# ipc-sim/IPC

Measured on AMD Instinct MI355X. Metric: newton_iterations_per_sec, higher is better.
Workload: dtype f64

## Files before the change

include/ipcgpu.h:

```cpp
#ifndef IPCGPU_H
#define IPCGPU_H

#ifdef __cplusplus
extern "C" {
#endif

#define IPCGPU_OK 0
#define IPCGPU_NOT_PD 1
#define IPCGPU_ERR_ARG -1
#define IPCGPU_ERR_HIP -2
#define IPCGPU_ERR_STATE -3
#define IPCGPU_ERR_UNSUPPORTED -4

typedef struct ipcgpu_ctx ipcgpu_ctx;

enum { IPCGPU_NOT_DBC = 0, IPCGPU_DBC_ZERO = 1, IPCGPU_DBC_NONZERO = 2 };

enum { IPCGPU_SOLVER_MULTIFRONTAL = 0, IPCGPU_SOLVER_ROCSOLVER_CSRRF = 1, IPCGPU_SOLVER_PCG = 2 };
enum { IPCGPU_PRECOND_BLOCK_JACOBI = 0, IPCGPU_PRECOND_LAGGED_CHOLESKY = 1, IPCGPU_PRECOND_TWO_LEVEL = 2 };

const char* ipcgpu_last_error(void);
int ipcgpu_version(void);

int ipcgpu_ctx_create(int device_id, ipcgpu_ctx** out);
int ipcgpu_ctx_destroy(ipcgpu_ctx*);
int ipcgpu_ctx_set_solver(ipcgpu_ctx*, int solver_type);
int ipcgpu_ctx_set_shard(ipcgpu_ctx*, int rank, int world_size);

typedef struct ipcgpu_tetmesh ipcgpu_tetmesh;
int ipcgpu_read_tet_mesh(const char* path, ipcgpu_tetmesh** mesh, int* nV, int* nT, int* nSF);
int ipcgpu_tet_mesh_get(const ipcgpu_tetmesh*, double* V_colmajor, int* T_colmajor, int* SF_colmajor);
void ipcgpu_tet_mesh_free(ipcgpu_tetmesh*);
int ipcgpu_save_tet_mesh(const char* path, int nV, int nT, const double* V_colmajor, const int* T_colmajor);

int ipcgpu_set_mesh(ipcgpu_ctx*, int nV, int nT, const double* V_rest_colmajor,
    const int* F_colmajor, double youngs_modulus, double poisson_ratio, double density);
int ipcgpu_set_dbc(ipcgpu_ctx*, int n, const int* vert_ids, int dbc_type);
int ipcgpu_clear_dbc(ipcgpu_ctx*);
int ipcgpu_set_component_material(ipcgpu_ctx*, int nodeBegin, int nodeEnd, int tetBegin, int tetEnd, double rho, double YM, double PR);
int ipcgpu_set_energy_type(ipcgpu_ctx*, int energy_type);
int ipcgpu_set_positions(ipcgpu_ctx*, const double* V_colmajor);
int ipcgpu_get_positions(ipcgpu_ctx*, double* V_colmajor);
int ipcgpu_set_xtilde(ipcgpu_ctx*, const double* xTilta_colmajor);
int ipcgpu_get_features(ipcgpu_ctx*, double* restTriInv_9nT, double* triArea_nT, double* mass_nV,
    double* mu_nT, double* lambda_nT);
int ipcgpu_get_mesh_dims(ipcgpu_ctx*, int* nV, int* nT);
int ipcgpu_set_mesh_features(ipcgpu_ctx*, const double* restTriInv_9nT, const double* triArea_nT, const double* mass_nV,
    const double* mu_nT, const double* lambda_nT);
int ipcgpu_check_inversion(ipcgpu_ctx*, int* ok);

int ipcgpu_elastic_energy(ipcgpu_ctx*, double coef, double* energy);
int ipcgpu_elastic_energy_per_elem(ipcgpu_ctx*, double* perElem_nT);
int ipcgpu_elastic_stress(ipcgpu_ctx*, double* perElem_nTx8, double* perNode_nVx8, int* n_invalid);
int ipcgpu_elastic_gradient(ipcgpu_ctx*, double coef, int projectDBC, double* grad_3nV);
int ipcgpu_elastic_hessian_add(ipcgpu_ctx*, double coef, int projectDBC);
int ipcgpu_filter_step_size(ipcgpu_ctx*, const double* searchDir_3nV, double* stepSize_inout);

int ipcgpu_linsys_set_pattern(ipcgpu_ctx*, int n_extra, const int* extra_pairs_2n);
int ipcgpu_linsys_set_pattern_csr(ipcgpu_ctx*, int n_rows, const int* ia, const int* ja);
int ipcgpu_linsys_get_dims(ipcgpu_ctx*, int* n_rows, int* nnz);
int ipcgpu_linsys_get_pattern(ipcgpu_ctx*, int* ia, int* ja);
int ipcgpu_linsys_set_zero(ipcgpu_ctx*);
int ipcgpu_linsys_get_values(ipcgpu_ctx*, double* a);
int ipcgpu_linsys_set_values(ipcgpu_ctx*, const double* a);
int ipcgpu_linsys_apply_host_updates(ipcgpu_ctx*, const double* delta_nnz, const unsigned char* isSet_nnz, const double* setVal_nnz);
int ipcgpu_linsys_add_coeff(ipcgpu_ctx*, int row, int col, double v);
int ipcgpu_linsys_set_coeff(ipcgpu_ctx*, int row, int col, double v);
int ipcgpu_linsys_multiply(ipcgpu_ctx*, const double* x, double* Ax);
int ipcgpu_linsys_analyze_pattern(ipcgpu_ctx*);
int ipcgpu_linsys_factorize(ipcgpu_ctx*);
int ipcgpu_linsys_solve(ipcgpu_ctx*, const double* rhs, double* result);
int ipcgpu_linsys_precondition_diag(ipcgpu_ctx*, const double* in, double* out);
int ipcgpu_linsys_set_iterative(ipcgpu_ctx*, double rel_tol, int max_iter, int precond, int max_factor_age);
int ipcgpu_linsys_iter_stats(ipcgpu_ctx*, double* out6);
int ipcgpu_linsys_coarse_stats(ipcgpu_ctx*, double* out5);
int ipcgpu_linsys_coarse_dims(ipcgpu_ctx*, int* n_aggregates, int* n_rows, int* nnz);
int ipcgpu_linsys_coarse_get(ipcgpu_ctx*, int* agg_of_node, int* coarse_ia, int* coarse_ja, double* coarse_a);
int ipcgpu_linsys_multiply_sym(ipcgpu_ctx*, const double* x, double* Ax);
int ipcgpu_linsys_set_shard(ipcgpu_ctx*, int rank, int world_size);
int ipcgpu_linsys_shard_stats(ipcgpu_ctx*, double* out2);
int ipcgpu_linsys_exchange_stats(ipcgpu_ctx*, double* out4);
int ipcgpu_linsys_critical_path(ipcgpu_ctx*, double* out5);
int ipcgpu_opt_comm_stats(ipcgpu_ctx*, double* out6);
int ipcgpu_opt_complete_matrix(ipcgpu_ctx*);
int ipcgpu_linsys_entry_destinations(ipcgpu_ctx*, long long* dst_nnz);
int ipcgpu_linsys_set_tuning(ipcgpu_ctx*, double bulk_min_mb, int bulk_block);
int ipcgpu_linsys_stats(ipcgpu_ctx*, double* stats4);

int ipcgpu_assemble_newton(ipcgpu_ctx*, double dtSq, int projectDBC, double* grad_3nV );
int ipcgpu_incremental_potential(ipcgpu_ctx*, double dtSq, double* energy);
int ipcgpu_gradient(ipcgpu_ctx*, double dtSq, int projectDBC, double* grad_3nV);

int ipcgpu_set_surface(ipcgpu_ctx*, int nSF, const int* SF_colmajor);
int ipcgpu_set_surface_codim(ipcgpu_ctx*, int nSF, const int* SF_colmajor, int nCE, const int* CE_pairs);
int ipcgpu_set_exact_predicates(ipcgpu_ctx*, int on);
int ipcgpu_get_surface(ipcgpu_ctx*, int* counts3 , int* SVI , int* SFEdges_2n );
int ipcgpu_set_obstacle_nodes(ipcgpu_ctx*, int n, const int* vert_ids, int obstacle_only);
int ipcgpu_set_codim_nodes(ipcgpu_ctx*, int n, const int* node_ids, const double* node_mass);
int ipcgpu_contact_build(ipcgpu_ctx*, double dHat, int* counts3);
int ipcgpu_contact_counts(ipcgpu_ctx*, int* counts3);
int ipcgpu_contact_get(ipcgpu_ctx*, int* active_4n, int* paraEE_4n, int* paraEEeIeJ_2n, int* csPTEE_2n );
int ipcgpu_contact_set(ipcgpu_ctx*, int nActive, const int* active_4n, int nParaEE, const int* paraEE_4n, const int* paraEEeIeJ_2n);
int ipcgpu_contact_energy(ipcgpu_ctx*, double dHat, double kappa, double* energy);
int ipcgpu_contact_evaluate(ipcgpu_ctx*, int n, const int* mmcvid_4n, double* val_n);
int ipcgpu_contact_jt_multiply(ipcgpu_ctx*, int n, const int* mmcvid_4n, const double* input_n, double coef, double* out_3nV_inout);
int ipcgpu_contact_gradient_add(ipcgpu_ctx*, double dHat, double kappa, int projectDBC, double* grad_3nV_inout);
int ipcgpu_contact_report(ipcgpu_ctx*, double dHat, double kappa, const double* Vt_colmajor , double eps2, double coef, int capacity, int* nRows,
    int* rowsI_8n, double* rowsD_20n);
int ipcgpu_contact_hessian_add(ipcgpu_ctx*, double dHat, double kappa, int projectDBC);
int ipcgpu_contact_connectivity(ipcgpu_ctx*, int capacity, int* pairs_2n, int* nPairs);
int ipcgpu_ccd_partial(ipcgpu_ctx*, const double* searchDir_3nV, double slackness, double* stepSize_inout, int* pair2);
int ipcgpu_ccd_full(ipcgpu_ctx*, const double* searchDir_3nV, double slackness, double* stepSize_inout, int* pair2, int* nCandidates);
int ipcgpu_ccd_full_reference(ipcgpu_ctx*, const double* searchDir_3nV, double slackness, double* stepSize_inout, double* alphaCapped, int* arg3,
    int* nCandidates);
int ipcgpu_set_ccd_mode(ipcgpu_ctx*, int mode);
int ipcgpu_is_intersected(ipcgpu_ctx*, int* flag);

int ipcgpu_opt_init(ipcgpu_ctx*, double dt, int withGravity);
int ipcgpu_opt_set_rel_tol(ipcgpu_ctx*, double relTol);
int ipcgpu_opt_set_twist(ipcgpu_ctx*, int nLeft, const int* left, int nRight, const int* right, double angVel);
int ipcgpu_opt_enable_self_collision(ipcgpu_ctx*, double dHatEps);
int ipcgpu_opt_set_pattern_lookahead(ipcgpu_ctx*, double pad);
int ipcgpu_opt_add_half_space(ipcgpu_ctx*, const double* origin3, const double* normal3, double dHatEps, int* id);
int ipcgpu_halfspace_build(ipcgpu_ctx*, int id, double dHat, int cap, int* verts, int* n);
int ipcgpu_halfspace_set(ipcgpu_ctx*, int id, int n, const int* verts);
int ipcgpu_halfspace_energy(ipcgpu_ctx*, int id, double dHat, double kappa, double* E);
int ipcgpu_halfspace_gradient_add(ipcgpu_ctx*, int id, double dHat, double kappa, double* grad_3nV_inout);
int ipcgpu_halfspace_hessian_add(ipcgpu_ctx*, int id, double dHat, double kappa, int projectDBC);
int ipcgpu_halfspace_move(ipcgpu_ctx*, int id, const double* delta3, double slackness, double* stepSizeLeft);
int ipcgpu_halfspace_step_bound(ipcgpu_ctx*, int id, const double* searchDir_3nV, double slackness, double* stepSize_inout);
int ipcgpu_opt_set_friction(ipcgpu_ctx*, double selfFric, int fricIterAmt, double epsV);
int ipcgpu_opt_set_friction_target(ipcgpu_ctx*, double eps_v_target);
int ipcgpu_opt_set_constructor_dt(ipcgpu_ctx*, double h);
int ipcgpu_opt_set_parameter_scaling(ipcgpu_ctx*, int useAbsParameters, double dTolRel, double kappaMinMultiplier);
int ipcgpu_opt_set_friction_scales(ipcgpu_ctx*, double scaleSelf, double scaleObstacle);
int ipcgpu_opt_force_friction_loop(ipcgpu_ctx*, int on);
int ipcgpu_opt_set_half_space_friction(ipcgpu_ctx*, int id, double mu);
int ipcgpu_opt_set_damping(ipcgpu_ctx*, double dampingStiff);
int ipcgpu_opt_set_kappa(ipcgpu_ctx*, double kappa);
int ipcgpu_opt_set_dhat_target(ipcgpu_ctx*, double dHatTargetEps);
int ipcgpu_opt_next_subproblem(ipcgpu_ctx*, int* more);
int ipcgpu_opt_get_friction_state(ipcgpu_ctx*, double* scalars4, double* lambda);
int ipcgpu_friction_update(ipcgpu_ctx*, double dHat, double kappa, int* nLagged);
int ipcgpu_friction_get(ipcgpu_ctx*, double* lambda_n, double* coord_2n, double* basis_6n);
int ipcgpu_friction_energy(ipcgpu_ctx*, const double* Vt_colmajor, double eps2, double coef, double* energy);
int ipcgpu_friction_gradient_add(ipcgpu_ctx*, const double* Vt_colmajor, double eps2, double coef, double* grad_3nV_inout);
int ipcgpu_friction_hessian_add(ipcgpu_ctx*, const double* Vt_colmajor, double eps2, double coef, int projectDBC);
int ipcgpu_opt_set_velocity(ipcgpu_ctx*, const double* vel_3nV);
int ipcgpu_opt_set_time_integration(ipcgpu_ctx*, int type, double beta, double gamma);
int ipcgpu_opt_set_warm_start(ipcgpu_ctx*, int option);
int ipcgpu_opt_get_warm_step(ipcgpu_ctx*, double* last_step);
int ipcgpu_opt_add_dirichlet(ipcgpu_ctx*, int n, const int* vert_ids, const double* lin_vel3, const double* ang_vel3, double t0, double t1);
int ipcgpu_opt_end_dirichlet(ipcgpu_ctx*, int group, double t_end);
int ipcgpu_opt_set_dirichlet_motion(ipcgpu_ctx*, int group, const double* lin_vel3, const double* ang_vel3, const double* center3 ,
    int force_nonzero);
int ipcgpu_opt_set_dirichlet_targets(ipcgpu_ctx*, int group, int n, const double* targets_3n);
int ipcgpu_opt_add_neumann(ipcgpu_ctx*, int n, const int* vert_ids, const double* accel3, double t0, double t1);
int ipcgpu_opt_get_dbc_state(ipcgpu_ctx*, double* out4);
int ipcgpu_opt_get_kinematics(ipcgpu_ctx*, double* vel_3nV, double* acc_3nV, double* dx_elastic_3nV);
int ipcgpu_opt_set_components(ipcgpu_ctx*, int nComp, const int* nodeEnd_nComp, const int* tetEnd_nComp);
int ipcgpu_opt_system_report(ipcgpu_ctx*, double* sysE_nComp, double* sysM_3nComp, double* sysL_3nComp);
int ipcgpu_opt_save_status(ipcgpu_ctx*, const char* path);
int ipcgpu_opt_load_status(ipcgpu_ctx*, const char* path);
int ipcgpu_opt_get_contact_state(ipcgpu_ctx*, int* counts6, int* pair2);
int ipcgpu_opt_precompute(ipcgpu_ctx*);
int ipcgpu_opt_begin_timestep(ipcgpu_ctx*);
int ipcgpu_opt_newton_iter(ipcgpu_ctx*, int* converged);
int ipcgpu_opt_end_timestep(ipcgpu_ctx*);
int ipcgpu_opt_solve_timestep(ipcgpu_ctx*, int maxIter, int* nIter);
int ipcgpu_opt_get_state(ipcgpu_ctx*, double* V_colmajor, double* searchDir_3nV, double* gradient_3nV, double* scalars8);
int ipcgpu_opt_get_timers(ipcgpu_ctx*, double* t16);
typedef int (*ipcgpu_allreduce_fn)(void* user, void* buf_dev, long long count, int op);
int ipcgpu_opt_set_allreduce(ipcgpu_ctx*, ipcgpu_allreduce_fn fn, void* user);
typedef int (*ipcgpu_allreduce_stream_fn)(void* user, void* buf_dev, long long count, int op, void* hip_stream);
int ipcgpu_opt_set_allreduce_stream(ipcgpu_ctx*, ipcgpu_allreduce_stream_fn fn, void* user);
typedef struct ipcgpu_p2p_op {
    void* buf_dev;
    long long count;
    int peer;
    int send;
} ipcgpu_p2p_op;
typedef int (*ipcgpu_exchange_fn)(void* user, int n_ops, const ipcgpu_p2p_op* ops);
typedef int (*ipcgpu_exchange_stream_fn)(void* user, int n_ops, const ipcgpu_p2p_op* ops, void* hip_stream);
int ipcgpu_opt_set_exchange(ipcgpu_ctx*, ipcgpu_exchange_fn fn, void* user);
int ipcgpu_opt_set_exchange_stream(ipcgpu_ctx*, ipcgpu_exchange_stream_fn fn, void* user);
int ipcgpu_ctx_get_stream(ipcgpu_ctx*, void** hip_stream);

int ipcgpu_bench_assembly(ipcgpu_ctx*, double dtSq, int reps, double* avg_ms, double* algorithmic_bytes);
int ipcgpu_bench_factor_solve(ipcgpu_ctx*, int reps, double* factor_ms, double* solve_ms);
int ipcgpu_bench_multiply_sym(ipcgpu_ctx*, int reps, double* avg_ms, double* algorithmic_bytes);
int ipcgpu_bench_stream(ipcgpu_ctx*, long long bytes, int reps, double* gbps);

#ifdef __cplusplus
}
#endif
#endif
```

ipc_amd/csrc/capi.cpp:

```cpp
#include "../../include/ipcgpu.h"
#include "hip_ipc.h"
#include "msh_io.h"
#include <cstdlib>
#include <cstring>
#include <mutex>

using namespace ipcgpu;

namespace {
thread_local std::string g_err;

template <class Fn>
int guarded(Fn&& fn)
{
    try {
        return fn();
    }
    catch (const ArgError& e) {
        g_err = e.what();
        return IPCGPU_ERR_ARG;
    }
    catch (const StateError& e) {
        g_err = e.what();
        return IPCGPU_ERR_STATE;
// ... 596 lines not shown
}
int ipcgpu_linsys_multiply_sym(ipcgpu_ctx* c, const double* x, double* y)
{
    return guarded([&] {
        bind(c);
        HipLinSysSolver& l = L(c);
        need(l.numRows > 0, "no pattern");
        needWholeMatrix(c);
        DevBuf<double> dx, dy;
        dx.upload(x, l.numRows, c->stream);
        dy.alloc(l.numRows);
        l.multiplySym(dx.p, dy.p);
        dy.download(y, l.numRows, c->stream);
        return IPCGPU_OK;
    });
}
int ipcgpu_linsys_set_iterative(ipcgpu_ctx* c, double rel_tol, int max_iter, int precond, int max_factor_age)
{
    specChanged(c);
    return guarded([&] {
        L(c).setIterative(rel_tol, max_iter, precond, max_factor_age);
        return IPCGPU_OK;
    });
}
int ipcgpu_linsys_iter_stats(ipcgpu_ctx* c, double* out6)
{
    return guarded([&] {
        needArg(c && out6, "null argument");
        L(c).iterStats(out6);
        return IPCGPU_OK;
    });
}
int ipcgpu_linsys_coarse_stats(ipcgpu_ctx* c, double* out5)
{
    return guarded([&] {
        needArg(c && out5, "null argument");
        L(c).coarseStats(out5);
        return IPCGPU_OK;
    });
}
int ipcgpu_linsys_coarse_dims(ipcgpu_ctx* c, int* n_agg, int* n_rows, int* nnz)
{
    return guarded([&] {
        L(c).coarseDims(n_agg, n_rows, nnz);
        return IPCGPU_OK;
    });
}
int ipcgpu_linsys_coarse_get(ipcgpu_ctx* c, int* agg_of_node, int* coarse_ia, int* coarse_ja, double* coarse_a)
{
    return guarded([&] {
        bind(c);
        L(c).coarseGet(agg_of_node, coarse_ia, coarse_ja, coarse_a);
        return IPCGPU_OK;
    });
}
int ipcgpu_linsys_analyze_pattern(ipcgpu_ctx* c)
{
    return guarded([&] {
        bind(c);
        L(c).analyze_pattern(c->mesh->nV ? c->mesh.get() : nullptr);
        return IPCGPU_OK;
    });
}
int ipcgpu_linsys_factorize(ipcgpu_ctx* c)
{
    return guarded([&] {
        bind(c);
        return L(c).factorize() ? IPCGPU_OK : IPCGPU_NOT_PD;
    });
}
int ipcgpu_linsys_solve(ipcgpu_ctx* c, const double* rhs, double* x)
{
    return guarded([&] {
        bind(c);
        HipLinSysSolver& l = L(c);
        DevBuf<double> db, dx;
        db.upload(rhs, l.numRows, c->stream);
        dx.alloc(l.numRows);
        const bool ok = l.solve(db.p, dx.p);
        dx.download(x, l.numRows, c->stream);
        return ok ? IPCGPU_OK : IPCGPU_NOT_PD;
    });
}
int ipcgpu_linsys_precondition_diag(ipcgpu_ctx* c, const double* in, double* out)
{
    return guarded([&] {
        bind(c);
        HipLinSysSolver& l = L(c);
        needWholeMatrix(c);
        DevBuf<double> di, dout;
        di.upload(in, l.numRows, c->stream);
        dout.alloc(l.numRows);
        l.precondition_diag(di.p, dout.p);
        dout.download(out, l.numRows, c->stream);
        return IPCGPU_OK;
    });
}
int ipcgpu_linsys_set_shard(ipcgpu_ctx* c, int rank, int world)
{
    specChanged(c);
    return guarded([&] {
        needArg(c && world >= 1 && rank >= 0 && rank < world, "bad shard");
        if (world > 1 && c->lin->solverType == IPCGPU_SOLVER_PCG) {
            g_err = "the iterative solver is not sharded";
            return IPCGPU_ERR_UNSUPPORTED;
        }
        need(world == 1 || c->opt->allreduce != nullptr || c->opt->allreduceStream != nullptr, "set the all-reduce hook first (ipcgpu_opt_set_allreduce)");
        need(world == 1 || c->lin->hasExchangeHook(), "set the exchange hook first (ipcgpu_opt_set_exchange / ipcgpu_opt_set_exchange_stream): the sharded solver sends point to point");
        c->lin->setShard(rank, world, c->opt->allreduce, c->opt->allreduceUser, c->opt->allreduceStream, c->opt->allreduceStreamUser);
        return IPCGPU_OK;
    });
}
int ipcgpu_opt_comm_stats(ipcgpu_ctx* c, double* out6)
{
    return guarded([&] {
        needArg(c && out6, "null argument");
        HipOptimizer& o = O(c);
        out6[0] = (double)o.commBytes;
        out6[1] = (double)o.commCalls;
        out6[2] = (double)L(c).exchangedBytes();
        out6[3] = (double)L(c).exchangeCalls();
        out6[4] = (double)(o.ownerMode() ? o.ownerNeededNodes : c->mesh->nV);
        out6[5] = (double)c->mesh->nV;
        return IPCGPU_OK;
    });
}
int ipcgpu_opt_complete_matrix(ipcgpu_ctx* c)
{
    return guarded([&] {
        bind(c);
        O(c).completeMatrix();
        return IPCGPU_OK;
    });
}
int ipcgpu_linsys_exchange_stats(ipcgpu_ctx* c, double* out4)
{
    return guarded([&] {
        needArg(c && out4, "null argument");
        out4[0] = (double)L(c).sentBytes();
        out4[1] = (double)L(c).receivedBytes();
        out4[2] = (double)L(c).exchangeCalls();
        out4[3] = L(c).exchangeWaitMs();
        return IPCGPU_OK;
    });
}
int ipcgpu_linsys_entry_destinations(ipcgpu_ctx* c, long long* dst_nnz)
{
    return guarded([&] {
        bind(c);
        needArg(c && dst_nnz, "null argument");
        need(L(c).solverType == IPCGPU_SOLVER_MULTIFRONTAL && L(c).analyzed(), "the multifrontal solver has not analysed a pattern yet");
        L(c).entryDestinations(dst_nnz);
        return IPCGPU_OK;
    });
}
int ipcgpu_linsys_shard_stats(ipcgpu_ctx* c, double* out2)
{
    return guarded([&] {
        out2[0] = L(c).solverWorld();
        out2[1] = L(c).sharedFlopFraction();
        return IPCGPU_OK;
    });
}
int ipcgpu_linsys_set_tuning(ipcgpu_ctx* c, double bulk_min_mb, int bulk_block)
{
    return guarded([&] {
// ... 891 lines not shown
            counts6[2] = o.selfCollision ? o.contact->nCand() : 0;
            counts6[3] = 0;
            for (const auto& h : o.planes) counts6[3] += (int)h->set.size();
            counts6[4] = o.nFullCCD;
            counts6[5] = o.nPatternChanges;
        }
        if (pair2) {
            pair2[0] = o.lastCCDPair[0];
            pair2[1] = o.lastCCDPair[1];
        }
        return IPCGPU_OK;
    });
}
int ipcgpu_opt_precompute(ipcgpu_ctx* c)
{
    return guarded([&] {
        bind(c);
        O(c).precompute();
        return IPCGPU_OK;
    });
}
int ipcgpu_opt_begin_timestep(ipcgpu_ctx* c)
{
    return guarded([&] {
        bind(c);
        O(c).beginTimestep();
        return IPCGPU_OK;
    });
}
int ipcgpu_opt_newton_iter(ipcgpu_ctx* c, int* converged)
{
    return guarded([&] {
        bind(c);
        const bool cv = O(c).newtonIter();
        if (converged) *converged = cv ? 1 : 0;
        return IPCGPU_OK;
    });
}
int ipcgpu_opt_end_timestep(ipcgpu_ctx* c)
{
    return guarded([&] {
        bind(c);
        O(c).endTimestep();
        return IPCGPU_OK;
    });
}
int ipcgpu_opt_solve_timestep(ipcgpu_ctx* c, int maxIter, int* nIter)
{
    return guarded([&] {
        bind(c);
        const int n = O(c).solveTimestep(maxIter);
        if (nIter) *nIter = n;
        return IPCGPU_OK;
    });
}
int ipcgpu_opt_get_state(ipcgpu_ctx* c, double* V, double* p, double* g, double* sc)
{
    return guarded([&] {
        HipOptimizer& o = O(c);
        bind(c);
        need(o.initialised, "call ipcgpu_opt_init first");
        const size_t n3 = 3 * (size_t)c->mesh->nV;
        if (V) downloadColMajor(c, c->mesh->d_x, V);
        if (p) o.d_searchDir.download(p, n3, c->stream);
        if (g) o.d_gradient.download(g, n3, c->stream);
        if (sc) {
            sc[0] = o.lastEnergyVal;
            sc[1] = o.lastStepSize;
            sc[2] = o.targetGRes;
            sc[3] = o.innerIterAmt;
            sc[4] = o.globalIterNum;
            sc[5] = o.lastAlphaFeasible;
            sc[6] = o.kappa;
            sc[7] = o.dHat;
        }
        return IPCGPU_OK;
    });
}
int ipcgpu_opt_get_timers(ipcgpu_ctx* c, double* t)
{
    return guarded([&] {
        O(c).resolveEventTimers();
        std::memcpy(t, O(c).timers, sizeof(double) * 16);
        return IPCGPU_OK;
    });
}
int ipcgpu_opt_set_allreduce(ipcgpu_ctx* c, ipcgpu_allreduce_fn fn, void* user)
{
    return guarded([&] {
        needArg(c != nullptr, "null context");
        c->opt->allreduce = fn;
        c->opt->allreduceUser = user;
        c->lin->setHooks(c->opt->allreduce, c->opt->allreduceUser, c->opt->allreduceStream, c->opt->allreduceStreamUser);
        return IPCGPU_OK;
    });
}

int ipcgpu_opt_set_allreduce_stream(ipcgpu_ctx* c, ipcgpu_allreduce_stream_fn fn, void* user)
{
    return guarded([&] {
        needArg(c != nullptr, "null context");
        c->opt->allreduceStream = fn;
        c->opt->allreduceStreamUser = user;
        c->lin->setHooks(c->opt->allreduce, c->opt->allreduceUser, c->opt->allreduceStream, c->opt->allreduceStreamUser);
        return IPCGPU_OK;
    });
}
static_assert(sizeof(ipcgpu_p2p_op) == sizeof(MfNumeric::P2POp), "ipcgpu_p2p_op and MfNumeric::P2POp must be one layout");
int ipcgpu_opt_set_exchange(ipcgpu_ctx* c, ipcgpu_exchange_fn fn, void* user)
{
    return guarded([&] {
        needArg(c != nullptr, "null context");
        c->exchange = reinterpret_cast<void*>(fn);
        c->exchangeUser = user;
        c->lin->setExchangeHooks(reinterpret_cast<MfNumeric::ExchangeFn>(c->exchange), c->exchangeUser, reinterpret_cast<MfNumeric::ExchangeStreamFn>(c->exchangeStream),
            c->exchangeStreamUser);
        return IPCGPU_OK;
    });
}
int ipcgpu_opt_set_exchange_stream(ipcgpu_ctx* c, ipcgpu_exchange_stream_fn fn, void* user)
{
    return guarded([&] {
        needArg(c != nullptr, "null context");
        c->exchangeStream = reinterpret_cast<void*>(fn);
        c->exchangeStreamUser = user;
        c->lin->setExchangeHooks(reinterpret_cast<MfNumeric::ExchangeFn>(c->exchange), c->exchangeUser, reinterpret_cast<MfNumeric::ExchangeStreamFn>(c->exchangeStream),
            c->exchangeStreamUser);
        return IPCGPU_OK;
    });
}
int ipcgpu_ctx_get_stream(ipcgpu_ctx* c, void** hipStream)
{
    return guarded([&] {
        needArg(c != nullptr && hipStream != nullptr, "null argument");
        *hipStream = (void*)c->stream;
        return IPCGPU_OK;
    });
}

int ipcgpu_bench_assembly(ipcgpu_ctx* c, double dtSq, int reps, double* avg_ms, double* bytes)
{
    return guarded([&] {
        HipOptimizer& o = O(c);
        bind(c);
        need(o.initialised && !c->lin->rowBase.empty(), "needs opt_init + a pattern");
        needArg(reps > 0, "reps must be positive");
        hipEvent_t e0, e1;
        HIP_CHECK(hipEventCreate(&e0));
        HIP_CHECK(hipEventCreate(&e1));
        const ElemView v = o.view();
        o.ensurePatchPlan();
        int pb, pe;
        o.patchShard(pb, pe);
        double total = 0.0;
        for (int r = 0; r < reps; ++r) {
            HIP_CHECK(hipEventRecord(e0, c->stream));
            launch_assemble_patches(v, o.patch, pb, pe, dtSq, 1, o.d_gradient.p, c->lin->d_a.p, c->stream);
            HIP_CHECK(hipEventRecord(e1, c->stream));
            HIP_CHECK(hipEventSynchronize(e1));
            float ms = 0;
            HIP_CHECK(hipEventElapsedTime(&ms, e0, e1));
            total += ms;
        }
        (void)hipEventDestroy(e0);
        (void)hipEventDestroy(e1);
        *avg_ms = total / reps;
// ... 92 lines not shown
```

ipc_amd/csrc/hip_ipc.h:

```cpp
#pragma once
#include "common.h"
#include "contact_pattern.h"
#include "mf_numeric.h"
#include "mf_symbolic.h"
#include "nh_kernels.h"
#include "patch_assembly.h"
#include "hip_contact.h"
#include "hip_halfspace.h"
#include "pcg.h"
#include "pcg_coarse.h"
#include "report_plan.h"
#include "stress_plan.h"
#include <map>
#include <memory>
#include <string>

struct ipcgpu_ctx;
typedef int (*ipcgpu_allreduce_fn_t)(void* user, void* buf_dev, long long count, int op);
typedef int (*ipcgpu_allreduce_stream_fn_t)(void* user, void* buf_dev, long long count, int op, void* hipStream);

namespace ipcgpu {

class HipMesh {
public:
    int nV = 0, nT = 0;
    int nElemNodes = 0;
    std::vector<double> V_rest;
    std::vector<int> F;
    std::vector<double> restTriInv;
    std::vector<double> triArea, mass, mu, lam;
    std::vector<int> dbcType;
    std::vector<int> nbPtr, nb;
    double avgEdgeLen = 0, bboxDiag2 = 0, bboxLo[3] = { 0, 0, 0 }, bboxHi[3] = { 0, 0, 0 };
    DevBuf<double> d_x, d_xTilde, d_mass, d_A, d_vol, d_mu, d_lam;
    DevBuf<int> d_dbc;
    DevBuf<int4> d_tet;

    unsigned featuresVersion = 0;
    void computeFeatures(int nV, int nT, const double* Vrest, const int* F, double YM, double PR, double density, hipStream_t s);
    std::vector<char> inMesh;
    void addSurfaceEdges(int nSF, const int* SF_colmajor, int nCE = 0, const int* CE_pairs = nullptr);
    void setCodimNodes(int n, const int* ids, const double* nodeMass, hipStream_t s);
    void meshBBox();
    void uploadDBC(hipStream_t s);
    int energyType = 0;
    double density = 0;
    void setComponentMaterial(int nodeBegin, int nodeEnd, int tetBegin, int tetEnd, double rho, double YM, double PR, hipStream_t s);
    bool isDBCVertex(int v) const { return dbcType[v] != 0; }
    bool isProjectDBCVertex(int v, bool projectDBC) const { return dbcType[v] == 1 || (dbcType[v] == 2 && projectDBC); }
};

class HipLinSysSolver {
public:
    explicit HipLinSysSolver(hipStream_t s);
    ~HipLinSysSolver();
    int numRows = 0;
    std::vector<int> ia, ja;
    DevBuf<int> d_ia, d_ja;
    DevBuf<double> d_a;
    DevBuf<double> hostDelta, hostSetVal;
    DevBuf<unsigned char> hostSetMask;
    std::vector<int> rowBase, rowLen;
    DevBuf<int> d_rowBase, d_rowLen, d_edgeP0;
    int solverType = 0;
    int patternVersion = 0;
    hipStream_t stream;

    void set_pattern(const HipMesh& mesh, int nExtra, const int* extraPairs);
    void set_pattern_csr(int nRows, const int* ia, const int* ja);
    void buildElementMap(const HipMesh& mesh);
    void setZero();
    int findEntry(int row, int col) const;
    void analyze_pattern(const HipMesh* meshForCoords);
    bool factorize();
    bool solve(const double* rhs_dev, double* x_dev);
    bool factorizeSolve(const double* rhs_dev, double* x_dev, bool wait = true);
    bool lastPivotsOk() const;
    bool lastSyncOk_ = true;
    void multiply(const double* x_dev, double* y_dev);
    void precondition_diag(const double* in_dev, double* out_dev);
    double pcgRelTol = 1e-5;
    int pcgMaxIter = 1000;
    int pcgPrecond = 0, pcgMaxFactorAge = 1;
    void setIterative(double relTol, int maxIter, int precond, int maxFactorAge);
    void iterStats(double* out6) const;
    void coarseStats(double* out5) const;
    bool coarseDims(int* nAgg, int* rows, int* nnz) const;
    void coarseGet(int* aggOfNode, int* cia, int* cja, double* ca);
    void multiplySym(const double* x_dev, double* y_dev);
    int getNumRows() const { return numRows; }
    int getNumNonzeros() const { return (int)ja.size(); }
    const MfSymbolic& symbolic() const { return sym_; }
    void setShard(int rank, int world, ipcgpu_allreduce_fn_t fn, void* user, ipcgpu_allreduce_stream_fn_t sfn = nullptr, void* streamUser = nullptr)
    {
        num_.setShard(rank, world, fn, user, sfn, streamUser);
        analyzed_ = false;
    }
    void setHooks(ipcgpu_allreduce_fn_t fn, void* user, ipcgpu_allreduce_stream_fn_t sfn, void* streamUser) { num_.setHooks(fn, user, sfn, streamUser); }
    void setExchangeHooks(MfNumeric::ExchangeFn fn, void* user, MfNumeric::ExchangeStreamFn sfn, void* streamUser) { num_.setExchangeHooks(fn, user, sfn, streamUser); }
    bool hasExchangeHook() const { return num_.hasExchangeHook(); }
    int solverWorld() const { return num_.world(); }
    void setBulkTuning(double minMB, int block) { num_.setBulkTuning(minMB, block); }
    void entryDestinations(long long* out) const { num_.entryDestinations(out, ja.size()); }
    void nodeOwners(std::vector<int>& o) const { num_.nodeOwners(o); }
    long long exchangedBytes() const { return num_.exchangedBytes(); }
    long long exchangeCalls() const { return num_.exchangeCalls(); }
    long long sentBytes() const { return num_.sentBytes(); }
    long long receivedBytes() const { return num_.receivedBytes(); }
    double exchangeWaitMs() { return num_.exchangeWaitMs(); }
    void criticalPath(double* out5) const { num_.criticalPath(out5); }
    int analysisVersion = 0;
    double sharedFlopFraction() const { return num_.sharedFlopFraction(); }
    bool analyzed() const { return analyzed_; }
    void invalidateAnalysis() { analyzed_ = false; }

private:
    MfSymbolic sym_;
    MfNumeric num_;
    bool analyzed_ = false;
    std::unique_ptr<struct RocsolverCsrrf> rs_;
    PcgPattern pcgPat_;
    PcgWork pcgWork_;
    int pcgPatVersion_ = -1;
    void ensurePcgPattern();
    int runPcg(const double* rhs_dev, double* x_dev, PcgState& out);
    bool haveFactor_ = false, lastConverged_ = true;
    int factorAge_ = 0;
    long long nFactorizations_ = 0;
    PcgCoarse coarseHost_;
    PcgCoarseDev coarseDev_;
    std::unique_ptr<HipLinSysSolver> coarse_;
    const HipMesh* coarseMesh_ = nullptr;
    int coarseVersion_ = -1;
    bool coarseBuilt_ = false, coarseOk_ = false;
    long long nCoarseFactorizations_ = 0, nCoarseFallbacks_ = 0;
    struct {
        int iterations = 0, syncs = 0, factorAge = 0;
        double residual = 0.0;
        bool converged = false;
    } pcgLast_;
    friend struct RocsolverCsrrf;
};

class HipOptimizer {
public:
    HipOptimizer(HipMesh& mesh, HipLinSysSolver& lin, hipStream_t s);
    void init(double dt, bool withGravity);
    void setRelGL2Tol(double relTol);
    void setParameterScaling(bool absolute, double dTolRel, double kappaMinMultiplier);
    void setTwist(int nL, const int* left, int nR, const int* right, double angVel);
    void precompute();
    void beginTimestep();
    bool newtonIter();
    void endTimestep();
    int solveTimestep(int maxIter);

    double computeEnergyVal();
    void computeGradient(bool projectDBC);
    void penaltyGradientAdd(bool projectDBC);
// ... 27 lines not shown
    double relGL2Tol = 1e-8, targetGRes = 0;
    int timeIntegration = 0;
    int warmStart = 0;
    double warmStepSize = 0.0;
    double betaNM = 0.25, gammaNM = 0.5;
    DevBuf<double> d_acc, d_dxElastic;
    double elasticCoef() const { return timeIntegration == 1 ? dtSq * betaNM : dtSq; }
    void setTimeIntegration(int type, double beta, double gamma);
    void getKinematics(double* vel, double* acc, double* dxElastic);
    void getDbcState(double* out4) const;
    std::vector<int> compNodeEnd, compTetEnd;
    DevBuf<double> d_xStepStart, d_reportRec;
    DevBuf<int> d_reportSlices, d_reportNodeStart, d_reportTetStart;
    PinnedBuf<double> h_report;
    bool reportPlanValid = false;
    int nReportNodeSlices = 0, nReportSlices = 0;
    void setComponents(int nComp, const int* nodeEnd, const int* tetEnd);
    void ensureReportPlan();
    void systemReport(double* sysE, double* sysM_3, double* sysL_3);
    void saveStatus(const std::string& path);
    void loadStatus(const std::string& path);
    DevBuf<double> d_vel, d_xPrev, d_searchDir, d_gradient, d_minusG, d_x0, d_partial, d_scalar;
    DevBuf<double> d_damp, d_xDamp, d_zeroMass, d_dampDx, d_dampAdx;
    unsigned long long dampPatternVersion = ~0ULL;
    DevBuf<int> d_flag, d_handleIds;
    DevBuf<double> d_handleAng;
    int nHandles = 0;
    struct DbcGroup {
        std::vector<int> ids;
        DevBuf<int> d_ids;
        DevBuf<double> d_pos;
        double lin[3], ang[3], t0, t1;
        bool forceNonzero = false, hasCenter = false;
        double center[3] = { 0, 0, 0 };
        bool hasTargets = false;
        DevBuf<double> d_targets;
        bool isZero() const { return !forceNonzero && lin[0] == 0 && lin[1] == 0 && lin[2] == 0 && ang[0] == 0 && ang[1] == 0 && ang[2] == 0; }
    };
    std::vector<std::unique_ptr<DbcGroup>> dbcGroups;
    struct NbcGroup {
        int n = 0;
        DevBuf<int> d_ids;
        double a[3], t0, t1;
    };
    std::vector<std::unique_ptr<NbcGroup>> nbcGroups;
    void addNeumannBC(int n, const int* ids, const double* accel3, double t0, double t1);
    void neumannGradientAdd(double* grad_dev);
    double neumannEnergy();
    std::vector<int> baseDbcType;
    double stepStartTime = 0, stepEndTime = 0;
    std::vector<int> tpIds, tpIdsOnDevice;
    DevBuf<int> d_tpIds;
    DevBuf<double> d_tpPos, d_tpLam, d_tpStage;
    double dist2Tol = 0, completedStep = 1.0, lastMove = 1.0, rhoDBC = 0.0, CN_MBC = 0.0;
    bool projDBC = true;
    MdbcView mdbc() const { return MdbcView{ (int)tpIds.size(), d_tpIds.p, d_tpPos.p, d_tpLam.p, mesh.d_mass.p }; }
    void buildTargetPositions(bool deferTolerance = false);
    void finishTolerance();
    PinnedBuf<double> h_tpStage;
    bool tolPending = false;
    void initSubProblem();
    double computeCompletedStepSize();
    void dirichletPenaltyUpdate();
    void addDirichletBC(int n, const int* ids, const double* lin3, const double* angRad3, double t0, double t1);
    void setDBCVertices();
    bool dbcGroupMotion();
    double rotCenter[3] = { 0, 0, 0 };
    PinnedBuf<double> h_scalar;
    PinnedBuf<int> h_flag;
    int innerIterAmt = 0, globalIterNum = 0, k = 0;
    double lastEnergyVal = 0, lastStepSize = 0, lastAlphaFeasible = 0;
    double timers[16] = { 0 };
    bool initialised = false;
    int rank = 0, worldSize = 1;
    int tetBegin = 0, tetEnd = 0;
    ipcgpu_allreduce_fn_t allreduce = nullptr;
    ipcgpu_allreduce_stream_fn_t allreduceStream = nullptr;
    void hookReduce(double* dev, long long n, int op);
    bool fastPath() const;
    bool cachedDistValid = false, cachedE0Valid = false;
    double cachedDist = 0, cachedE0 = 0, cachedFilter = 0;
    bool cachedTrialValid = false, cachedTrialInverted = false;
    double cachedTrialE = 0, cachedAlpha = 1.0;
    DevBuf<double> d_aSpec, d_gradSpec;
    bool specAsmValid = false;
    void speculativeAssembly();
    hipEvent_t evAsm0 = nullptr, evAsm1 = nullptr, evTail = nullptr;
    bool evAsmPending = false;
    int evAsmWeight = 1;
    unsigned asmLaunches = 0;
    void resolveEventTimers();
    DevBuf<double> d_contactG;
    void* allreduceUser = nullptr;
    void* allreduceStreamUser = nullptr;
    void reduceSum(double* dev, long long n);
    void reduceMin(double* dev, long long n);
    double readScalar(const double* dev);
    PatchPlan patch;
    int patchVersion = -1;
    void ensurePatchPlan();
    void patchShard(int& pb, int& pe) const;
    bool ownerMode() const;
    void ensureOwnerPlan();
    int ownerPlanPatch = -1, ownerPlanAnalysis = -1;
    int nOwnerPatches = 0;
    DevBuf<int> d_ownerPatches;
    DevBuf<unsigned char> d_need, d_mine;
    long long ownerNeededNodes = 0;
    bool matrixComplete = true;
    void maskAndReduceGradient(double* g);
    void ownerGradientTail(bool projectDBC);
    void completeMatrix();
    long long commBytes = 0, commCalls = 0;
    HipContact* contact = nullptr;
    bool selfCollision = false;
    double dHatEps = 1.0e-3, dHat = 0, kappa = 0, dTol = 0;
    bool absParameters = false;
    double dTolRel = 1.0e-9, kappaMinMultiplier = 1.0e11;
    double lenScale2() const { return absParameters ? 1.0 : mesh.bboxDiag2; }
    ContactPattern contactPattern;
    std::vector<std::array<int, 4>> closeID;
    std::vector<double> closeVal;
    int lastCCDPair[2] = { 0, 0 }, nFullCCD = 0, nPatternChanges = 0, dbcIncomplete = 0;
    unsigned long long coverSets = ~0ull;
    int coverPattern = -1;
    bool coverAnswer = false;
    double patternPad = -1.0;
    double lookahead() const { return patternPad >= 0.0 ? patternPad : (mesh.nV > 150000 ? 2.25 : 4.0); }
    std::vector<std::unique_ptr<HipHalfSpace>> planes;
    std::vector<std::pair<int, int>> closeHS;
    std::vector<double> closeHSVal;
    double selfFric = 0.0, epsV = 1.0e-3, fricDHat0 = 0, fricDHat = -1.0;
    double epsVTarget = -1.0, fricDHatTarget = 0;
    int fricIterAmt = 1, fricIterI = 0;
    bool fricLoopForced = false;
    bool solveFric() const;
    void updateFrictionLag();
    bool nextSubproblem();
    bool ipOn() const { return selfCollision || !planes.empty(); }
    size_t nConstraints() const;
    int addHalfSpace(HipContact* c, const double* origin3, const double* normal3, double dHatEps);
    bool anyIntersection();
    void elasticInertiaGradient(bool projectDBC, bool finish = true);
    void barrierGradientAdd(bool projectDBC, double kappa, bool activeOnly, double* grad_dev, int part = 0);
    void enableSelfCollision(HipContact* c, double dHatEps);
    void setVelocity(const double* vel3nV);
    void computeConstraintSets();
    double kappaFloor() const;
    void initKappa();
    void postLineSearch();
    bool isIntersected();
    void computeXTilta();
};

struct StressFields {
    bool planValid = false;
    DevBuf<int> d_ptr, d_elems, d_invalid;
    DevBuf<double> d_elem, d_node;
    PinnedBuf<int> h_invalid;
};

}

struct ipcgpu_ctx {
    int device = 0;
    hipStream_t stream = nullptr;
// ... 12 lines not shown
```

ipc_amd/csrc/hip_linsys.hip:

```cpp
#include "hip_ipc.h"
#include <rocsolver/rocsolver.h>
#include <algorithm>
#include <cmath>
#include <thread>
#include <cstdlib>

namespace ipcgpu {

struct RocsolverCsrrf {
    rocblas_handle handle = nullptr;
    rocsolver_rfinfo info = nullptr;
    int n = 0, nnzA = 0, nnzT = 0;
    DevBuf<int> ptrA, indA, ptrT, indT, pivQ, trans, flag;
    DevBuf<double> valA, valT, B;
    bool analyzed = false;
    ~RocsolverCsrrf()
    {
        if (info) rocsolver_destroy_rfinfo(info);
        if (handle) rocblas_destroy_handle(handle);
    }
};

namespace {
__global__ void k_gather(int n, const int* __restrict__ map, const double* __restrict__ src, double* __restrict__ dst)
// ... 224 lines not shown
        for (int r = 0; r < numRows; ++r) ptr[r + 1] += ptr[r];
        std::vector<int> pos(ptr.begin(), ptr.end() - 1);
        for (int r = 0; r < numRows; ++r)
            for (int k = ia[r]; k < ia[r + 1]; ++k) {
                const int c = ja[k];
                ind[pos[c]] = r;
                tr[pos[c]] = k;
                pos[c]++;
            }
        std::vector<int> pT, iT, q;
        mf_L_pattern_csr(sym_, pT, iT, q);
        R.nnzA = nnz;
        R.nnzT = (int)iT.size();
        R.ptrA.upload(ptr, stream);
        R.indA.upload(ind, stream);
        R.trans.upload(tr, stream);
        R.valA.alloc(nnz);
        R.ptrT.upload(pT, stream);
        R.indT.upload(iT, stream);
        R.pivQ.upload(q, stream);
        R.valT.alloc(iT.size());
        R.B.alloc(numRows);
        R.B.zero(stream);
        R.flag.alloc(1);
        hipLaunchKernelGGL(k_set_diag_one, dim3((numRows + 255) / 256), dim3(256), 0, stream, numRows, R.ptrT.p, R.indT.p, R.valT.p);
        hipLaunchKernelGGL(k_set_diag_one, dim3((numRows + 255) / 256), dim3(256), 0, stream, numRows, R.ptrA.p, R.indA.p, R.valA.p);
        const rocblas_status st = rocsolver_dcsrrf_analysis(R.handle, R.n, 1, R.nnzA, R.ptrA.p, R.indA.p, R.valA.p, R.nnzT, R.ptrT.p, R.indT.p, R.valT.p,
            nullptr, R.pivQ.p, R.B.p, R.n, R.info);
        if (st != rocblas_status_success) throw HipError("rocsolver_dcsrrf_analysis failed (rocblas_status " + std::to_string((int)st) + ")");
        HIP_CHECK(hipStreamSynchronize(stream));
        R.analyzed = true;
    }
    analyzed_ = true;
}

bool HipLinSysSolver::factorize()
{
    if (!analyzed_) throw StateError("factorize before analyze_pattern");
    if (solverType == 0) return num_.factorize(d_a.p);
    if (solverType == 2) {
        if (pcgPrecond == 0 || pcgPrecond == 2) {
            pcgWork_.ensure(numRows);
            pcgWork_.flag.zero(stream);
            launch_pcg_invert_blocks(pcgPat_, d_a.p, pcgWork_.flag.p, stream);
            int f = 0;
            pcgWork_.flag.download(&f, 1, stream);
            if (f || pcgPrecond == 0) return f == 0;
            if (!coarseMesh_->d_x.p || !coarseMesh_->d_dbc.p || 3 * coarseMesh_->nV != numRows) throw StateError("factorize: the mesh of the two-level preconditioner has no positions");
            launch_pcg_coarse_geometry(coarseDev_, coarseMesh_->d_x.p, coarseMesh_->d_dbc.p, stream);
            launch_pcg_galerkin(coarseDev_, d_rowLen.p, d_a.p, coarse_->d_a.p, stream);
            coarseBuilt_ = true;
            ++nCoarseFactorizations_;
            coarseOk_ = coarse_->factorize();
            if (!coarseOk_) ++nCoarseFallbacks_;
            return true;
        }
        if (haveFactor_ && lastConverged_ && factorAge_ + 1 < pcgMaxFactorAge) {
            ++factorAge_;
            return true;
        }
        ++nFactorizations_;
        haveFactor_ = num_.factorize(d_a.p);
        factorAge_ = 0;
        lastConverged_ = true;
        return haveFactor_;
    }
    RocsolverCsrrf& R = *rs_;
    hipLaunchKernelGGL(k_gather, dim3((R.nnzA + 255) / 256), dim3(256), 0, stream, R.nnzA, R.trans.p, d_a.p, R.valA.p);
    rocblas_status st = rocsolver_dcsrrf_refactchol(R.handle, R.n, R.nnzA, R.ptrA.p, R.indA.p, R.valA.p, R.nnzT, R.ptrT.p, R.indT.p,
        R.valT.p, R.pivQ.p, R.info);
    if (st != rocblas_status_success) {
        HIP_CHECK(hipStreamSynchronize(stream));
        return false;
    }
    R.flag.zero(stream);
    hipLaunchKernelGGL(k_check_diag, dim3((R.n + 255) / 256), dim3(256), 0, stream, R.n, R.ptrT.p, R.valT.p, R.pivQ.p, d_ia.p, d_a.p,
        R.flag.p);
    int f = 0;
    HIP_CHECK(hipMemcpyAsync(&f, R.flag.p, sizeof(int), hipMemcpyDeviceToHost, stream));
    HIP_CHECK(hipStreamSynchronize(stream));
    return f == 0;
}

bool HipLinSysSolver::factorizeSolve(const double* rhs_dev, double* x_dev, bool wait)
{
    if (!analyzed_) throw StateError("factorize before analyze_pattern");
    lastSyncOk_ = true;
    if (solverType == 0) return lastSyncOk_ = num_.factorizeSolve(d_a.p, rhs_dev, x_dev, wait);
    const bool ok = factorize();
    return lastSyncOk_ = ok && solve(rhs_dev, x_dev);
}
bool HipLinSysSolver::lastPivotsOk() const { return lastSyncOk_ && (solverType != 0 || num_.lastPivotsOk()); }

bool HipLinSysSolver::solve(const double* rhs_dev, double* x_dev)
{
    if (!analyzed_) throw StateError("solve before analyze_pattern");
    if (solverType == 0) {
        num_.solve(rhs_dev, x_dev);
        return true;
    }
    if (solverType == 2) {
        const bool lagged = pcgPrecond == 1;
        const bool jacobi = !lagged;
        if (lagged && !haveFactor_) throw StateError("solve before factorize");
        if (pcgPrecond == 2 && !coarseBuilt_) throw StateError("solve before factorize");
        pcgLast_ = {};
        pcgLast_.factorAge = jacobi ? 0 : factorAge_;
        PcgState st;
        int status = runPcg(rhs_dev, x_dev, st);
        pcgLast_.iterations = st.iter;
        if (status == PCG_MAXITER && !jacobi && factorAge_ > 0) {
            ++nFactorizations_;
            haveFactor_ = num_.factorize(d_a.p);
            factorAge_ = 0;
            if (!haveFactor_) return false;
            pcgLast_.factorAge = 0;
            status = runPcg(rhs_dev, x_dev, st);
            pcgLast_.iterations += st.iter;
        }
        pcgLast_.residual = st.bb > 0.0 ? std::sqrt(st.trueRes2 / st.bb) : 0.0;
        pcgLast_.converged = status == PCG_CONVERGED && st.trueRes2 <= st.tol2;
        lastConverged_ = pcgLast_.converged;
        return status != PCG_BREAKDOWN;
    }
    RocsolverCsrrf& R = *rs_;
    HIP_CHECK(hipMemcpyAsync(x_dev, rhs_dev, sizeof(double) * R.n, hipMemcpyDeviceToDevice, stream));
    if (rocsolver_dcsrrf_solve(R.handle, R.n, 1, R.nnzT, R.ptrT.p, R.indT.p, R.valT.p, nullptr, R.pivQ.p, x_dev, R.n, R.info)
        != rocblas_status_success)
        throw HipError("rocsolver_dcsrrf_solve failed");
    return true;
}

void HipLinSysSolver::setIterative(double relTol, int maxIter, int precond, int maxFactorAge)
{
    if (!(relTol > 0.0) || maxIter < 1 || precond < 0 || precond > 2 || maxFactorAge < 1)
        throw ArgError("set_iterative: rel_tol > 0, max_iter >= 1, precond 0 | 1 | 2, max_factor_age >= 1");
    if (precond != pcgPrecond && solverType == 2) analyzed_ = false;
    pcgRelTol = relTol;
    pcgMaxIter = maxIter;
    pcgPrecond = precond;
    pcgMaxFactorAge = maxFactorAge;
}

void HipLinSysSolver::iterStats(double* o) const
{
    o[0] = pcgLast_.iterations;
    o[1] = pcgLast_.residual;
    o[2] = pcgLast_.converged ? 1.0 : 0.0;
    o[3] = (double)nFactorizations_;
    o[4] = pcgLast_.factorAge;
    o[5] = pcgLast_.syncs;
}

void HipLinSysSolver::coarseStats(double* o) const
{
    const bool have = coarseVersion_ == patternVersion && coarse_;
    o[0] = have ? coarseHost_.nAgg : 0;
    o[1] = have ? 6.0 * coarseHost_.nAgg : 0;
    o[2] = have ? (double)coarseHost_.cja.size() : 0;
    o[3] = (double)nCoarseFactorizations_;
    o[4] = (double)nCoarseFallbacks_;
}
bool HipLinSysSolver::coarseDims(int* nAgg, int* rows, int* nnz) const
{
    const bool have = solverType == 2 && pcgPrecond == 2 && analyzed_ && coarse_ && coarseVersion_ == patternVersion;
    if (nAgg) *nAgg = have ? coarseHost_.nAgg : 0;
    if (rows) *rows = have ? 6 * coarseHost_.nAgg : 0;
    if (nnz) *nnz = have ? (int)coarseHost_.cja.size() : 0;
    return have;
}
void HipLinSysSolver::coarseGet(int* aggOfNode, int* cia, int* cja, double* ca)
{
    if (!coarseDims(nullptr, nullptr, nullptr)) throw StateError("no coarse level: set the two-level preconditioner and call analyze_pattern first");
    if (aggOfNode) std::copy(coarseHost_.aggOf.begin(), coarseHost_.aggOf.end(), aggOfNode);
// ... 89 lines not shown
```

ipc_amd/csrc/hip_optimizer.cpp:

```cpp
#include "hip_ipc.h"
#include <fstream>
#include <iomanip>
#include <limits>
#include <sstream>
#include <algorithm>
#include <chrono>
#include <thread>
#include <iterator>
#include <cmath>
#include <cstring>

#ifndef BEGIN_BATCHED
#define BEGIN_BATCHED 1
#endif

namespace ipcgpu {


namespace {
struct Tic {
    double& acc;
    hipStream_t s;
    std::chrono::high_resolution_clock::time_point t0;
    bool nosync = false;
    Tic(double& a, hipStream_t st) : acc(a), s(st), t0(std::chrono::high_resolution_clock::now()) {}
    ~Tic()
    {
        if (!nosync) (void)hipStreamSynchronize(s);
        acc += std::chrono::duration<double>(std::chrono::high_resolution_clock::now() - t0).count();
    }
};
}

HipOptimizer::HipOptimizer(HipMesh& m, HipLinSysSolver& l, hipStream_t s) : mesh(m), lin(l), stream(s) {}

ElemView HipOptimizer::view() const
{
    ElemView v;
    v.nV = mesh.nV;
    v.nT = mesh.nT;
    v.tetBegin = tetBegin;
    v.tetEnd = tetEnd;
    v.energyType = mesh.energyType;
    v.x = mesh.d_x.p;
    v.xTilde = mesh.d_xTilde.p;
    v.mass = mesh.d_mass.p;
    v.dbc = mesh.d_dbc.p;
    v.tet = mesh.d_tet.p;
    v.A = mesh.d_A.p;
    v.vol = mesh.d_vol.p;
    v.mu = mesh.d_mu.p;
    v.lam = mesh.d_lam.p;
    v.rowBase = lin.d_rowBase.p;
    v.rowLen = lin.d_rowLen.p;
    v.edgeP0 = lin.d_edgeP0.p;
    return v;
}

void HipOptimizer::init(double dt_, bool withGravity)
{
    dt = dt_;
    dtSq = dt * dt;
    gravity[0] = gravity[2] = 0.0;
    gravity[1] = withGravity ? -9.80665 : 0.0;
    const size_t n3 = 3 * (size_t)mesh.nV;
    d_vel.alloc(n3);
    d_vel.zero(stream);
    d_acc.alloc(n3);
    d_acc.zero(stream);
    d_dxElastic.alloc(n3);
    d_dxElastic.zero(stream);
    d_xPrev.alloc(n3);
    d_xStepStart.alloc(n3);
    d_searchDir.alloc(n3);
    d_searchDir.zero(stream);
    d_gradient.alloc(n3);
    d_gradient.zero(stream);
    d_minusG.alloc(n3);
    d_x0.alloc(n3);
    d_partial.alloc((size_t)std::max(mesh.nT, mesh.nV) / 256 + 2);
    d_scalar.alloc(8);
    d_flag.alloc(2);
    h_scalar.alloc(8);
    h_flag.alloc(2);
    HIP_CHECK(hipMemcpyAsync(d_xPrev.p, mesh.d_x.p, n3 * sizeof(double), hipMemcpyDeviceToDevice, stream));
    HIP_CHECK(hipMemcpyAsync(d_xStepStart.p, mesh.d_x.p, n3 * sizeof(double), hipMemcpyDeviceToDevice, stream));
    HIP_CHECK(hipMemcpyAsync(mesh.d_xTilde.p, mesh.d_x.p, n3 * sizeof(double), hipMemcpyDeviceToDevice, stream));
    for (int c = 0; c < 3; ++c) rotCenter[c] = 0.5 * (mesh.bboxLo[c] + mesh.bboxHi[c]);
    tetBegin = (int)((long long)mesh.nT * rank / worldSize);
    tetEnd = (int)((long long)mesh.nT * (rank + 1) / worldSize);
    setRelGL2Tol(1.0e-2);
    innerIterAmt = globalIterNum = k = 0;
    std::memset(timers, 0, sizeof(timers));
    initialised = true;
    HIP_CHECK(hipStreamSynchronize(stream));
    computeXTilta();
}

void HipOptimizer::setRelGL2Tol(double relTol)
{
    relGL2Tol = relTol * relTol;
    targetGRes = std::sqrt(relGL2Tol * (absParameters ? 1.0 : mesh.bboxDiag2 * dtSq));
    CN_MBC = std::sqrt(1.0e-4 * mesh.bboxDiag2 * (ctorDt * ctorDt));
}

void HipOptimizer::setParameterScaling(bool absolute, double dTolRel_, double kappaMinMultiplier_)
{
    if (!(dTolRel_ > 0.0) || !(kappaMinMultiplier_ > 0.0)) throw ArgError("set_parameter_scaling: dTolRel and kappaMinMultiplier must be positive");
    absParameters = absolute;
    dTolRel = dTolRel_;
    kappaMinMultiplier = kappaMinMultiplier_;
    targetGRes = std::sqrt(relGL2Tol * (absParameters ? 1.0 : mesh.bboxDiag2 * dtSq));
    if (ipOn()) {
        dHat = dHatEps * dHatEps * lenScale2();
        dTol = dTolRel * dTolRel * lenScale2();
    }
}

void HipOptimizer::setTwist(int nL, const int* left, int nR, const int* right, double angVel)
{
    std::vector<int> ids;
    std::vector<double> ang;
    for (int i = 0; i < nL; ++i) {
        mesh.dbcType[left[i]] = 2;
        ids.push_back(left[i]);
        ang.push_back(-angVel * dt);
    }
    for (int i = 0; i < nR; ++i) {
        mesh.dbcType[right[i]] = 2;
        ids.push_back(right[i]);
        ang.push_back(angVel * dt);
    }
    nHandles = (int)ids.size();
    if (nHandles) {
        d_handleIds.upload(ids, stream);
        d_handleAng.upload(ang, stream);
    }
    mesh.uploadDBC(stream);
    if (initialised) computeXTilta();
}

void HipOptimizer::addNeumannBC(int n, const int* ids, const double* accel3, double t0, double t1)
{
    std::unique_ptr<NbcGroup> g(new NbcGroup);
    g->n = n;
    g->d_ids.upload(ids, (size_t)n, stream);
    for (int c = 0; c < 3; ++c) g->a[c] = accel3[c];
    g->t0 = t0;
    g->t1 = t1;
    HIP_CHECK(hipStreamSynchronize(stream));
    nbcGroups.push_back(std::move(g));
}

void HipOptimizer::neumannGradientAdd(double* grad_dev)
{
    for (const auto& g : nbcGroups) {
        if (stepStartTime < g->t0 || stepStartTime >= g->t1) continue;
        const double c[3] = { dtSq * g->a[0], dtSq * g->a[1], dtSq * g->a[2] };
        launch_nbc_gradient(g->n, g->d_ids.p, mesh.d_dbc.p, mesh.d_mass.p, c, grad_dev, stream);
    }
}

double HipOptimizer::neumannEnergy()
// ... 730 lines not shown
    }
    lap("set_pattern");
    {
        int dev = 0;
        HIP_CHECK(hipGetDevice(&dev));
        std::exception_ptr planErr;
        std::thread planThread([&] {
            try {
                HIP_CHECK(hipSetDevice(dev));
                ensurePatchPlan();
            }
            catch (...) {
                planErr = std::current_exception();
            }
        });
        std::exception_ptr anaErr;
        try {
            Tic t(timers[2], stream);
            lin.analyze_pattern(&mesh);
        }
        catch (...) {
            anaErr = std::current_exception();
        }
        planThread.join();
        if (anaErr) std::rethrow_exception(anaErr);
        if (planErr) std::rethrow_exception(planErr);
    }
    lap("analyze_pattern + patch plan");
}

void HipOptimizer::assembleSystem(bool projectDBC, bool withGradient)
{
    const bool owner = ownerMode();
    int pb = 0, pe = 0;
    if (owner) {
        ensureOwnerPlan();
        pe = nOwnerPatches;
    }
    else patchShard(pb, pe);
    if (worldSize > 1) {
        lin.setZero();
        if (withGradient) d_gradient.zero(stream);
    }
    launch_assemble_patches(view(), patch, pb, pe, elasticCoef(), projectDBC, withGradient ? d_gradient.p : nullptr, lin.d_a.p, stream,
        owner ? d_ownerPatches.p : nullptr);
    matrixComplete = !owner;
    if (owner) {
        if (withGradient) ownerGradientTail(projectDBC);
    }
    else {
        if (worldSize > 1) {
            reduceSum(lin.d_a.p, (long long)lin.ja.size());
            if (withGradient) reduceSum(d_gradient.p, 3LL * mesh.nV);
        }
        if (withGradient) {
            neumannGradientAdd(d_gradient.p);
            if (ipOn()) barrierGradientAdd(projectDBC, kappa, false, d_gradient.p);
        }
    }
    if (ipOn()) {
        for (auto& h : planes)
            h->hessianAdd(mesh.d_x.p, mesh.d_dbc.p, lin.d_rowBase.p, lin.d_rowLen.p, dHat, kappa, projectDBC, lin.d_a.p);
        if (selfCollision)
            contact->hessianAdd(mesh.d_x.p, mesh.d_dbc.p, lin, dHat, kappa, projectDBC, lin.d_a.p, owner ? d_need.p : nullptr, true);
        if (fricDHat > 0.0) {
            for (auto& h : planes)
                if (h->friction > 0.0)
                    h->frictionHessianAdd(mesh.d_x.p, d_xPrev.p, mesh.d_dbc.p, lin.d_rowBase.p, lin.d_rowLen.p, fricDHat, projectDBC, lin.d_a.p);
            if (selfCollision && selfFric > 0.0)
                contact->frictionHessianAdd(mesh.d_x.p, d_xPrev.p, mesh.d_dbc.p, lin, fricDHat, selfFric, projectDBC, lin.d_a.p);
        }
    }
    if (dampingStiff > 0.0) {
        if (dampPatternVersion != lin.patternVersion) assembleDampingMtr();
        launch_axpy((long long)lin.ja.size(), 1.0, d_damp.p, lin.d_a.p, stream);
    }
    if (withGradient && !owner) penaltyGradientAdd(projectDBC);
    if (!projectDBC && rhoDBC && !tpIds.empty()) launch_mdbc_hessian(mdbc(), lin.d_ia.p, rhoDBC, lin.d_a.p, stream);
}

bool HipOptimizer::checkInversion()
{
    if (mesh.energyType == 1) return true;
    d_flag.zero(stream);
    launch_check_inversion(view(), d_flag.p, stream);
    launch_publish(d_flag.p, h_flag.dev, 1, stream);
    HIP_CHECK(hipStreamSynchronize(stream));
    int f = h_flag.p[0];
    if (worldSize > 1) {
        h_scalar.p[1] = (double)f;
        HIP_CHECK(hipMemcpyAsync(d_scalar.p + 1, h_scalar.p + 1, sizeof(double), hipMemcpyHostToDevice, stream));
        reduceSum(d_scalar.p + 1, 1);
        f = readScalar(d_scalar.p + 1) != 0.0;
    }
    return f == 0;
}

double HipOptimizer::fullCcd(double slackness, double stepSize)
{
    if (contact->ccdMode == 1) {
        int arg3[3];
        const double a = contact->ccdFullReference(mesh, mesh.d_x.p, d_searchDir.p, mesh.d_dbc.p, slackness, stepSize, nullptr, arg3, nullptr);
        lastCCDPair[0] = arg3[1];
        lastCCDPair[1] = arg3[2];
        return a;
    }
    return contact->ccdFull(mesh, mesh.d_x.p, d_searchDir.p, mesh.d_dbc.p, slackness, stepSize, lastCCDPair, nullptr);
}

double HipOptimizer::filterStepSize(const double* p_dev, double stepSize)
{
    if (mesh.energyType == 1) return stepSize;
    launch_fill(d_scalar.p + 2, 1, 1e20, stream);
    launch_inversion_step(view(), p_dev, 0.2, stepSize, d_scalar.p + 2, stream);
    reduceMin(d_scalar.p + 2, 1);
    const double t = readScalar(d_scalar.p + 2);
    if (t > 0.0 && t < stepSize) stepSize = t;
    return stepSize;
}

void HipOptimizer::stepForward(const double* x0_dev, double alpha)
{
    launch_step_forward(3 * mesh.nV, x0_dev, d_searchDir.p, alpha, mesh.d_x.p, stream);
}

#ifndef ASM_TIME_EVERY
#define ASM_TIME_EVERY 8
#endif
void HipOptimizer::speculativeAssembly()
{
    specAsmValid = false;
    if (!fastPath() || !projDBC || lin.rowBase.empty()) return;
    ensurePatchPlan();
    d_aSpec.alloc(lin.d_a.n);
    d_gradSpec.alloc(d_gradient.n);
    const bool timeIt = (asmLaunches++ % ASM_TIME_EVERY) == 0;
    if (timeIt) {
        resolveEventTimers();
        HIP_CHECK(hipEventRecord(evAsm0, stream));
    }
    launch_assemble_patches(view(), patch, 0, patch.nPatches, elasticCoef(), 1, d_gradSpec.p, d_aSpec.p, stream);
    if (timeIt) {
        HIP_CHECK(hipEventRecord(evAsm1, stream));
        evAsmPending = true;
        evAsmWeight = ASM_TIME_EVERY;
    }
    specAsmValid = true;
}

void HipOptimizer::enqueueDirNorm()
{
    launch_fill(d_scalar.p + 3, 1, 0.0, stream);
    launch_max_abs(3 * mesh.nV, d_searchDir.p, d_scalar.p + 3, stream);
}

void HipOptimizer::computeSearchDir()
{
    bool ok;
    launch_negate(3 * mesh.nV, d_gradient.p, d_minusG.p, stream);
    cachedTrialValid = false;
    cachedDistValid = false;
    if (fastPath()) {
        Tic t(timers[3], stream);
        const size_t bytes = 3 * (size_t)mesh.nV * sizeof(double);
        if (lin.factorizeSolve(d_minusG.p, d_searchDir.p, false)) {
            launch_iter_reset(d_scalar.p, d_flag.p, stream);
            launch_max_abs(3 * mesh.nV, d_searchDir.p, d_scalar.p + 3, stream);
            if (mesh.energyType != 1) launch_inversion_step(view(), d_searchDir.p, 0.2, 1.0, d_scalar.p + 2, stream);
            launch_energy(view(), elasticCoef(), true, true, d_partial.p, (int)d_partial.n, d_scalar.p, stream);
            launch_trial_step_fused(3 * mesh.nV, mesh.d_x.p, d_x0.p, d_searchDir.p, d_scalar.p + 2, mesh.energyType != 1, d_scalar.p + 6, stream);
            if (mesh.energyType != 1) launch_check_inversion(view(), d_flag.p, stream);
            launch_energy(view(), elasticCoef(), true, true, d_partial.p, (int)d_partial.n, d_scalar.p + 1, stream);
            launch_publish2(d_flag.p, h_flag.dev, 1, d_scalar.p, h_scalar.dev, 14, stream);
            if (!evTail) HIP_CHECK(hipEventCreateWithFlags(&evTail, hipEventDisableTiming));
            HIP_CHECK(hipEventRecord(evTail, stream));
            speculativeAssembly();
            HIP_CHECK(hipEventSynchronize(evTail));
            t.nosync = specAsmValid;
            if (lin.lastPivotsOk()) {
                cachedE0 = h_scalar.p[0];
                cachedTrialE = h_scalar.p[1];
                cachedFilter = h_scalar.p[2];
                cachedDist = h_scalar.p[3];
                cachedAlpha = h_scalar.p[6];
                cachedTrialInverted = mesh.energyType != 1 && h_flag.p[0] != 0;
                cachedDistValid = cachedE0Valid = cachedTrialValid = true;
                return;
            }
            HIP_CHECK(hipMemcpyAsync(mesh.d_x.p, d_x0.p, bytes, hipMemcpyDeviceToDevice, stream));
            specAsmValid = false;
            t.nosync = false;
        }
        ok = false;
    }
    else {
        Tic t(timers[3], stream);
        if (worldSize == 1) {
            ok = lin.factorizeSolve(d_minusG.p, d_searchDir.p, false);
            if (ok) {
                enqueueDirNorm();
                launch_publish(d_scalar.p + 3, h_scalar.dev + 3, 2, stream);
                HIP_CHECK(hipStreamSynchronize(stream));
                ok = lin.lastPivotsOk();
                if (ok) {
                    cachedDist = h_scalar.p[3];
                    cachedDistValid = true;
                }
            }
        }
        else ok = lin.factorizeSolve(d_minusG.p, d_searchDir.p);
    }
    Tic t(timers[4], stream);
    if (!ok) {
        completeMatrix();
        lin.precondition_diag(d_minusG.p, d_searchDir.p);
    }
    if (fastPath()) {
        enqueueDirNorm();
        launch_fill(d_scalar.p + 2, 1, 1e20, stream);
        if (mesh.energyType != 1) launch_inversion_step(view(), d_searchDir.p, 0.2, 1.0, d_scalar.p + 2, stream);
        launch_energy(view(), elasticCoef(), true, true, d_partial.p, (int)d_partial.n, d_scalar.p, stream);
        launch_publish(d_scalar.p, h_scalar.dev, 8, stream);
        HIP_CHECK(hipStreamSynchronize(stream));
        cachedE0 = h_scalar.p[0];
        cachedFilter = h_scalar.p[2];
        cachedDist = h_scalar.p[3];
        cachedDistValid = cachedE0Valid = true;
    }
    else {
        if (!cachedDistValid) {
            enqueueDirNorm();
            launch_publish(d_scalar.p + 3, h_scalar.dev + 3, 2, stream);
            HIP_CHECK(hipStreamSynchronize(stream));
            cachedDist = h_scalar.p[3];
            cachedDistValid = true;
        }
        if (selfCollision) contact->takeHessianError();
    }
}

bool HipOptimizer::fastPath() const
{
    return worldSize == 1 && !ipOn() && nbcGroups.empty() && !(dampingStiff > 0.0) && !(rhoDBC && !tpIds.empty()) && lin.solverType != 2;
}

void HipOptimizer::resolveEventTimers()
{
    if (!evAsmPending) return;
    HIP_CHECK(hipEventSynchronize(evAsm1));
    float ms = 0.0f;
    HIP_CHECK(hipEventElapsedTime(&ms, evAsm0, evAsm1));
    timers[0] += 1.0e-3 * (double)ms * evAsmWeight;
    evAsmPending = false;
}

void HipOptimizer::stepFeasible(double& stepSize)
{
    stepForward(d_x0.p, stepSize);
    while (!checkInversion()) {
        stepSize /= 2.0;
        stepForward(d_x0.p, stepSize);
    }
    if (ipOn())
        while (anyIntersection()) {
            stepSize /= 2.0;
            stepForward(d_x0.p, stepSize);
        }
}

void HipOptimizer::lineSearch(double& stepSize)
{
    const size_t bytes = 3 * (size_t)mesh.nV * sizeof(double);
    if (cachedTrialValid && fastPath()) {
        cachedTrialValid = cachedE0Valid = false;
        lastEnergyVal = cachedE0;
        if (!cachedTrialInverted && !(cachedTrialE > lastEnergyVal)) {
            lastEnergyVal = cachedTrialE;
            return;
        }
        HIP_CHECK(hipMemcpyAsync(mesh.d_x.p, d_x0.p, bytes, hipMemcpyDeviceToDevice, stream));
        specAsmValid = false;
    }
    else if (cachedE0Valid && fastPath()) {
        cachedE0Valid = false;
        lastEnergyVal = cachedE0;
        bool done = false;
        double testingE = 0.0;
        {
            Tic t(timers[5], stream);
            HIP_CHECK(hipMemcpyAsync(d_x0.p, mesh.d_x.p, bytes, hipMemcpyDeviceToDevice, stream));
            stepForward(d_x0.p, stepSize);
            int inverted = 0;
            if (mesh.energyType != 1) {
                d_flag.zero(stream);
                launch_check_inversion(view(), d_flag.p, stream);
                launch_publish(d_flag.p, h_flag.dev, 1, stream);
            }
            launch_energy(view(), elasticCoef(), true, true, d_partial.p, (int)d_partial.n, d_scalar.p, stream);
            launch_publish(d_scalar.p, h_scalar.dev, 2, stream);
            HIP_CHECK(hipStreamSynchronize(stream));
            if (mesh.energyType != 1) inverted = h_flag.p[0];
            testingE = h_scalar.p[0];
            done = !inverted && !(testingE > lastEnergyVal);
        }
        if (done) {
            lastEnergyVal = testingE;
            return;
        }
        HIP_CHECK(hipMemcpyAsync(mesh.d_x.p, d_x0.p, bytes, hipMemcpyDeviceToDevice, stream));
    }
    {
        Tic t(timers[9], stream);
        lastEnergyVal = computeEnergyVal();
    }
    {
        Tic t(timers[5], stream);
        HIP_CHECK(hipMemcpyAsync(d_x0.p, mesh.d_x.p, bytes, hipMemcpyDeviceToDevice, stream));
        stepForward(d_x0.p, stepSize);
        while (!checkInversion()) {
            stepSize /= 2.0;
            if (stepSize == 0.0) break;
            stepForward(d_x0.p, stepSize);
        }
        if (ipOn())
            while (anyIntersection()) {
                stepSize /= 2.0;
                stepForward(d_x0.p, stepSize);
            }
    }
    computeConstraintSets();
    double testingE;
    {
        Tic t(timers[9], stream);
        testingE = computeEnergyVal();
    }
    const double LFStepSize = stepSize;
    while (testingE > lastEnergyVal && stepSize > 0.0) {
        stepSize /= 2.0;
        if (stepSize == 0.0) break;
        {
            Tic t(timers[5], stream);
            stepForward(d_x0.p, stepSize);
        }
        computeConstraintSets();
        Tic t(timers[9], stream);
        testingE = computeEnergyVal();
    }
    if (stepSize < LFStepSize && ipOn()) {
        bool needRecomputeCS = false;
        while (anyIntersection()) {
            stepSize /= 2.0;
            stepForward(d_x0.p, stepSize);
            needRecomputeCS = true;
        }
        if (needRecomputeCS) computeConstraintSets();
    }
    lastEnergyVal = testingE;
}

void HipOptimizer::precompute()
{
    specAsmValid = false;
    if (!initialised) throw StateError("opt_precompute before opt_init");
    if (anyIntersection()) throw StateError("intersection detected in initial configuration");
    {
        Tic t(timers[1], stream);
        lin.set_pattern(mesh, 0, nullptr);
        contactPattern = ContactPattern();
    }
    computeConstraintSets();
    computeDampingMtr();
    {
        Tic t(timers[0], stream);
        computePrecondMtr(true, false);
    }
    if (!lin.analyzed()) {
        Tic t(timers[2], stream);
        lin.analyze_pattern(&mesh);
    }
    lastEnergyVal = computeEnergyVal();
}

void HipOptimizer::beginTimestep()
{
    specAsmValid = false;
    if (!initialised) throw StateError("opt_begin_timestep before opt_init");
    if (!lin.analyzed()) throw StateError("opt_begin_timestep before opt_precompute");
    Tic t(timers[11], stream);
    const bool batched = BEGIN_BATCHED && fastPath() && nHandles && dbcGroups.empty() && !selfCollision && planes.empty() && !(warmStart >= 1 && warmStart <= 5);
    if (batched) {
        const bool guard = mesh.energyType != 1;
        d_flag.zero(stream);
        if (guard) launch_check_inversion(view(), d_flag.p, stream);
        d_searchDir.zero(stream);
        stepStartTime = stepEndTime;
        stepEndTime += dt;
        setDBCVertices();
        launch_twist_dir(nHandles, d_handleIds.p, d_handleAng.p, rotCenter[1], rotCenter[2], mesh.d_x.p, d_searchDir.p, stream);
        buildTargetPositions(true);
        launch_fill(d_scalar.p + 2, 1, 1e20, stream);
        if (guard) launch_inversion_step(view(), d_searchDir.p, 0.2, 1.0, d_scalar.p + 2, stream);
        launch_trial_step_fused(3 * mesh.nV, mesh.d_x.p, d_x0.p, d_searchDir.p, d_scalar.p + 2, guard, d_scalar.p + 6, stream);
        if (guard) launch_check_inversion(view(), d_flag.p + 1, stream);
        launch_energy(view(), elasticCoef(), true, true, d_partial.p, (int)d_partial.n, d_scalar.p, stream);
        launch_publish2(d_flag.p, h_flag.dev, 2, d_scalar.p, h_scalar.dev, 14, stream);
        HIP_CHECK(hipStreamSynchronize(stream));
        if (h_flag.p[0]) throw StateError("element inversion before scripted motion (Optimizer.cpp:517-522)");
        finishTolerance();
        double stepSize = h_scalar.p[6];
        bool energyKnown = true;
        if (h_flag.p[1]) {
            energyKnown = false;
            stepSize /= 2.0;
            stepFeasible(stepSize);
        }
        if (stepSize < 1.0) dbcIncomplete++;
        completedStep = stepSize;
        d_searchDir.zero(stream);
        initSubProblem();
        lastEnergyVal = energyKnown ? h_scalar.p[0] : computeEnergyVal();
        k = 0;
        return;
    }
    if (!checkInversion()) throw StateError("element inversion before scripted motion (Optimizer.cpp:517-522)");
    d_searchDir.zero(stream);
    stepStartTime = stepEndTime;
    stepEndTime += dt;
    setDBCVertices();
    if (nHandles) launch_twist_dir(nHandles, d_handleIds.p, d_handleAng.p, rotCenter[1], rotCenter[2], mesh.d_x.p, d_searchDir.p, stream);
    const bool groupMotion = dbcGroupMotion();
    buildTargetPositions();
    completedStep = 1.0;
    if (nHandles || groupMotion) {
        double stepSize = filterStepSize(d_searchDir.p, 1.0);
        if (selfCollision)
            stepSize = fullCcd(0.5, stepSize);
        HIP_CHECK(hipMemcpyAsync(d_x0.p, mesh.d_x.p, 3 * (size_t)mesh.nV * sizeof(double), hipMemcpyDeviceToDevice, stream));
        stepFeasible(stepSize);
        if (stepSize < 1.0) dbcIncomplete++;
        completedStep = stepSize;
        d_searchDir.zero(stream);
    }
    if (warmStart >= 1 && warmStart <= 5) {
        if (warmStart == 5) {
            computeGradient(true);
            computePrecondMtr(false, false);
            launch_negate(3 * mesh.nV, d_gradient.p, d_minusG.p, stream);
            completeMatrix();
            lin.precondition_diag(d_minusG.p, d_searchDir.p);
            launch_clear_projected(mesh.nV, mesh.d_dbc.p, 1, d_searchDir.p, stream);
        }
        else {
        static const double CG[2][5] = { { 0, 0, 1, 1, 1 }, { 0, 0, 0.5, 0.5, 0.5 } }, CE[2][5] = { { 0, 0, 0, 1, 0.5 }, { 0, 0, 0, 2, 1 } };
        const double cg = CG[timeIntegration][warmStart], ce = CE[timeIntegration][warmStart];
        const double g3[3] = { cg * (dtSq * gravity[0]), cg * (dtSq * gravity[1]), cg * (dtSq * gravity[2]) };
        launch_warm_dir(mesh.nV, mesh.d_dbc.p, d_vel.p, d_dxElastic.p, dt, g3, ce, d_searchDir.p, stream);
        }
        double stepSize = filterStepSize(d_searchDir.p, 1.0);
        if (ipOn()) {
            for (auto& h : planes) stepSize = h->stepBound(contact->nSVI, contact->d_SVI.p, mesh.d_x.p, mesh.d_dbc.p, d_searchDir.p, 0.9, stepSize);
            if (selfCollision) stepSize = fullCcd(0.8, stepSize);
        }
        HIP_CHECK(hipMemcpyAsync(d_x0.p, mesh.d_x.p, 3 * (size_t)mesh.nV * sizeof(double), hipMemcpyDeviceToDevice, stream));
        stepFeasible(stepSize);
        warmStepSize = stepSize;
    }
    if (ipOn()) {
        dHat = dHatEps * dHatEps * lenScale2();
        computeConstraintSets();
        kappa = kappaConfig > 0.0 ? std::min(kappaConfig, 100 * kappaFloor()) : kappaFloor();
        initKappa();
        closeHS.clear();
        closeHSVal.clear();
        closeID.clear();
// ... 68 lines not shown
    if (projDBC) {
        if (completedStep < 1.0 - 1.0e-3) {
            projDBC = false;
            rhoDBC = 1.0e6;
        }
        return;
    }
    const double completed = computeCompletedStepSize();
    if (completed > 1.0 - 1.0e-3) projDBC = true;
    else if (completed < lastMove && rhoDBC < 1.0e8) rhoDBC *= 2.0;
    else {
        enqueueDirNorm();
        if (readScalar(d_scalar.p + 3) < CN_MBC) {
            if (completed < 0.99 && rhoDBC < 1.0e8) rhoDBC *= 2.0;
            else launch_mdbc_lambda(mdbc(), mesh.d_x.p, rhoDBC, stream);
        }
    }
}

bool HipOptimizer::newtonIter()
{
    double distToOpt_PN;
    if (k && cachedDistValid) distToOpt_PN = cachedDist;
    else if (k) {
        enqueueDirNorm();
        distToOpt_PN = readScalar(d_scalar.p + 3);
    }
    else distToOpt_PN = 0.0;
    cachedDistValid = false;
    if (k && distToOpt_PN < targetGRes && completedStep > 1.0 - 1.0e-3) {
        specAsmValid = false;
        Tic t(timers[12], stream);
        t.nosync = fastPath();
        computeGradient(projDBC);
        return true;
    }
    innerIterAmt++;
    if (fastPath()) {
        if (!evAsm0) {
            HIP_CHECK(hipEventCreate(&evAsm0));
            HIP_CHECK(hipEventCreate(&evAsm1));
        }
        if (specAsmValid && projDBC && d_aSpec.n == lin.d_a.n && d_gradSpec.n == d_gradient.n) {
            std::swap(lin.d_a.p, d_aSpec.p);
            std::swap(d_gradient.p, d_gradSpec.p);
            matrixComplete = true;
        }
        else {
            resolveEventTimers();
            HIP_CHECK(hipEventRecord(evAsm0, stream));
            computePrecondMtr(projDBC, true);
            HIP_CHECK(hipEventRecord(evAsm1, stream));
            evAsmPending = true;
            evAsmWeight = 1;
        }
        specAsmValid = false;
    }
    else {
        specAsmValid = false;
        Tic t(timers[0], stream);
        computePrecondMtr(projDBC, true);
    }
    cachedE0Valid = false;
    computeSearchDir();
    double alpha = 1.0;
    {
        Tic t(timers[13], stream);
        t.nosync = specAsmValid && cachedTrialValid;
        const bool batchedBounds = !cachedTrialValid && !cachedE0Valid && selfCollision && planes.empty() && worldSize == 1;
        if (cachedTrialValid) alpha = cachedAlpha;
        else if (cachedE0Valid) {
            if (mesh.energyType != 1 && cachedFilter > 0.0 && cachedFilter < alpha) alpha = cachedFilter;
        }
        else if (!batchedBounds)
        alpha = filterStepSize(d_searchDir.p, alpha);
        for (auto& h : planes)
            alpha = h->stepBound(contact->nSVI, contact->d_SVI.p, mesh.d_x.p, mesh.d_dbc.p, d_searchDir.p, 0.9, alpha);
        if (selfCollision) {
            const double slackness_m = 0.8;
            double pMax;
            if (batchedBounds) {
                const bool filter = mesh.energyType != 1;
                if (filter) {
                    launch_fill(d_scalar.p + 2, 1, 1e20, stream);
                    launch_inversion_step(view(), d_searchDir.p, 0.2, alpha, d_scalar.p + 2, stream);
                }
                contact->stepBounds(mesh.d_x.p, d_searchDir.p, slackness_m, alpha, filter ? d_scalar.p + 2 : nullptr, &alpha, lastCCDPair, &pMax);
            }
            else {
                alpha = contact->ccdPartial(mesh.d_x.p, d_searchDir.p, slackness_m, alpha, lastCCDPair);
                pMax = contact->maxSurfaceSpeed(d_searchDir.p);
            }
            const double alpha_CFL = std::sqrt(dHat) / (pMax * 2.0);
            if ((!k && alpha > alpha_CFL) || alpha > 2.0 * alpha_CFL) {
                alpha = fullCcd(slackness_m, alpha);
                nFullCCD++;
                if (alpha < alpha_CFL) alpha = alpha_CFL;
            }
            else alpha = std::min(alpha, alpha_CFL);
        }
    }
    lastAlphaFeasible = alpha;
    lineSearch(alpha);
    lastStepSize = alpha;
    postLineSearch();
    dirichletPenaltyUpdate();
    ++k;
    return false;
}

void HipOptimizer::endTimestep()
{
    specAsmValid = false;
    Tic t(timers[11], stream);
    t.nosync = fastPath();
    std::swap(d_xPrev.p, d_xStepStart.p);
    if (timeIntegration == 1)
        launch_nm_update(mesh.nV, mesh.d_dbc.p, mesh.d_x.p, d_xPrev.p, d_vel.p, d_acc.p, d_dxElastic.p, mesh.d_xTilde.p, dt, betaNM, gammaNM,
            gravity[0], gravity[1], gravity[2], stream);
    else
        launch_be_update(mesh.nV, mesh.d_dbc.p, mesh.d_x.p, d_xStepStart.p, d_xPrev.p, d_vel.p, d_acc.p, d_dxElastic.p, mesh.d_xTilde.p, dt, gravity[0],
            gravity[1], gravity[2], stream);
    computeDampingMtr();
    globalIterNum++;
}

void HipOptimizer::setComponents(int nComp, const int* nodeEnd, const int* tetEnd_)
{
    if (!reportEndsValid(nComp, nodeEnd, mesh.nV) || !reportEndsValid(nComp, tetEnd_, mesh.nT))
        throw ArgError("set_components: the accumulated ends must be non-decreasing and end at the node / element count");
    compNodeEnd.assign(nodeEnd, nodeEnd + nComp);
    compTetEnd.assign(tetEnd_, tetEnd_ + nComp);
    reportPlanValid = false;
}

void HipOptimizer::ensureReportPlan()
{
    if (reportPlanValid) return;
    if (compNodeEnd.empty() || compNodeEnd.back() != mesh.nV || compTetEnd.back() != mesh.nT) {
        compNodeEnd.assign(1, mesh.nV);
        compTetEnd.assign(1, mesh.nT);
    }
    const int nComp = (int)compNodeEnd.size();
    std::vector<ReportSlice> slices;
    std::vector<int> nodeStart, tetStart;
    buildReportSlices(nComp, compNodeEnd.data(), 256, slices, nodeStart);
    nReportNodeSlices = (int)slices.size();
    buildReportSlices(nComp, compTetEnd.data(), 256, slices, tetStart);
    nReportSlices = (int)slices.size();
    static_assert(sizeof(ReportSlice) == 3 * sizeof(int), "the kernel reads the list as int triples");
    std::vector<int> flat(3 * slices.size() + 1);
    std::memcpy(flat.data(), slices.data(), slices.size() * sizeof(ReportSlice));
    d_reportSlices.upload(flat, stream);
    d_reportNodeStart.upload(nodeStart, stream);
    d_reportTetStart.upload(tetStart, stream);
    d_reportRec.alloc(7 * slices.size() + 1);
    h_report.alloc(7 * (size_t)nComp);
    HIP_CHECK(hipStreamSynchronize(stream));
    reportPlanValid = true;
}

void HipOptimizer::systemReport(double* sysE, double* sysM, double* sysL)
{
    if (worldSize > 1) throw UnsupportedError("system report on a sharded context (multi-rank reports are not implemented)");
    ensureReportPlan();
    const int nComp = (int)compNodeEnd.size();
// ... 31 lines not shown
```

ipc_amd/csrc/mf_numeric.h:

```cpp
#pragma once
#include "common.h"
#include "mf_plan.h"
#include "mf_symbolic.h"

namespace ipcgpu {

class MfNumeric {
public:
    MfNumeric() = default;
    ~MfNumeric();
    MfNumeric(const MfNumeric&) = delete;
    MfNumeric& operator=(const MfNumeric&) = delete;

    void setup(const MfSymbolic& sym, hipStream_t stream, const int* ia_dev, const int* ja_dev, long long nnzPattern);
    typedef int (*AllreduceFn)(void* user, void* buf_dev, long long count, int op);
    typedef int (*AllreduceStreamFn)(void* user, void* buf_dev, long long count, int op, void* hipStream);
    struct P2POp {
        void* buf_dev;
        long long count;
        int peer;
        int send;
    };
    typedef int (*ExchangeFn)(void* user, int nOps, const P2POp* ops);
    typedef int (*ExchangeStreamFn)(void* user, int nOps, const P2POp* ops, void* hipStream);
    void setShard(int rank, int world, AllreduceFn fn, void* user, AllreduceStreamFn sfn = nullptr, void* streamUser = nullptr)
    {
        rank_ = rank;
        world_ = world;
        setHooks(fn, user, sfn, streamUser);
    }
    void setBulkTuning(double minMB, int block)
    {
        tune_.bulkMinMB = minMB;
        tune_.bulkBlock = block < 64 ? 64 : (block / 32) * 32;
    }
    void setExchangeHooks(ExchangeFn fn, void* user, ExchangeStreamFn sfn, void* streamUser)
    {
        exchange_ = fn;
        exchangeUser_ = user;
        exchangeStream_ = sfn;
        exchangeStreamUser_ = streamUser;
    }
    bool hasExchangeHook() const { return exchange_ || exchangeStream_; }
    void setHooks(AllreduceFn fn, void* user, AllreduceStreamFn sfn, void* streamUser)
    {
        allreduce_ = fn;
        allreduceUser_ = user;
        allreduceStream_ = sfn;
        allreduceStreamUser_ = streamUser;
    }
    int world() const { return world_; }
    void nodeOwners(std::vector<int>& ownerOfNode) const;
    long long exchangedBytes() const { return commBytes_; }
    long long exchangeCalls() const { return commCalls_; }
    long long sentBytes() const { return sentBytes_; }
    long long receivedBytes() const { return recvBytes_; }
    double exchangeWaitMs();
    void criticalPath(double* out5) const;
    double sharedFlopFraction() const { return mp_.sharedFlops; }
    bool factorize(const double* a_dev);
    void solve(const double* rhs_dev, double* x_dev);
    bool factorizeSolve(const double* a_dev, const double* rhs_dev, double* x_dev, bool wait = true);
    bool lastPivotsOk() const { return pivotsOk(); }
    bool pivotsOk() const;
    bool ready() const { return ns_ > 0; }
    void entryDestinations(long long* out, size_t nnz) const { entryDst_.download(out, nnz, stream_); }
    size_t front_bytes() const { return fronts_.n * sizeof(double); }

private:
    void enqueueFactor(const double* a_dev, bool overlapForward = false);
    void enqueueSolve(const double* rhs_dev, double* x_dev);
    typedef MfRange Range;
    typedef MfLevelPlan LevelPlan;
    typedef MfXinvLevel XinvLevel;
    int rank_ = 0, world_ = 1;
    MfPlanTuning tune_;
    MfPlan mp_;
    AllreduceFn allreduce_ = nullptr;
    AllreduceStreamFn allreduceStream_ = nullptr;
    void* allreduceUser_ = nullptr;
    void* allreduceStreamUser_ = nullptr;
    ExchangeFn exchange_ = nullptr;
    ExchangeStreamFn exchangeStream_ = nullptr;
    void* exchangeUser_ = nullptr;
    void* exchangeStreamUser_ = nullptr;
    long long commBytes_ = 0, commCalls_ = 0, sentBytes_ = 0, recvBytes_ = 0;
    double waitMs_ = 0.0;
    std::vector<std::pair<hipEvent_t, hipEvent_t>> waitPending_, waitFree_;
    struct Xchg {
        std::vector<P2POp> opsM, opsW, opsX;
    };
    std::vector<Xchg> xchg_;
    DevBuf<int4> xchgDesc_;
    DevBuf<double> xchgBuf_;
    DevBuf<int> nodeExec_;
    void allreduceSum(double* dev, long long count);
    void exchange(const std::vector<P2POp>& ops);
    void exchangeUpdateMatrices(int level);
    void exchangeUpdateVectors(int level);
    void reduceSolution();
    void allreduceFlag();
    void configureSweepKernels(size_t maxSolveLds, size_t maxBwdLds, size_t maxTriLds);
    void enqueuePermuteRhs(const double* rhs_dev, hipStream_t st);
    const MfSymbolic* sym_ = nullptr;
    hipStream_t stream_ = nullptr;
    int ns_ = 0, nLevels_ = 0;
    DevBuf<double> fronts_, w_, yperm_, bperm_, xsol_;
    DevBuf<double> xinvX_, xinvT_;
    DevBuf<long long> xinvOff_;
    DevBuf<int4> xinvDesc_;
    DevBuf<int> triList_;
    hipStream_t side_ = nullptr;
    int fwdStride_ = 4;
    bool fwdJoined_ = false;
    hipStream_t fwd_ = nullptr;
    hipEvent_t evRhs_ = nullptr, evFwdDone_ = nullptr;
    std::vector<hipEvent_t> evFactLevel_;
    void enqueueForwardLevel(int l, hipStream_t st);
    void enqueueBackward(double* x_dev);
    hipEvent_t evSide_ = nullptr;
    std::vector<hipEvent_t> evLevel_, evInvDone_;
    bool sidePending_ = false;
    void enqueueInverses(int level, hipStream_t st);
    DevBuf<double> dinv_;
    DevBuf<int> idx_, idxPtr_, firstNode_, childPtr_, child_, invPtr_, inv_, newOf_, flag_;
    DevBuf<long long> frontOff_, wOff_, dinvOff_;
    DevBuf<int> aSrc_, aLoc_;
    DevBuf<double> aPerm_;
    int nFusedA_ = 0;
    DevBuf<int> bigFd_;
    DevBuf<int> fdesc_;
    DevBuf<int> bigASrc_;
    DevBuf<long long> bigADst_;
    DevBuf<long long> entryDst_;
    DevBuf<int> entryBucket_, bucketHist_, bucketStart_, nodeFront_;
    DevBuf<int4> frontInfo_;
    DevBuf<int> eaAPtr_;
    DevBuf<int4> eaDesc_;
    DevBuf<int> smallList_, bigList_;
    DevBuf<int4> desc_;
    PinnedBuf<int> hflag_;
};

}
```

ipc_amd/csrc/mf_numeric.hip:

```cpp
#include <climits>
#include "mf_kernels.h"
#include <algorithm>
#include <chrono>
#include <cstdio>
#include <cstdlib>
#include <cstring>
#include <thread>

namespace ipcgpu {

namespace {

__global__ void k_publish_flag(const int* __restrict__ flag, int* __restrict__ mapped) { mapped[0] = flag[0]; }

__global__ void k_gather_a(int cnt, const int* __restrict__ src, const double* __restrict__ a, double* __restrict__ aP, int* __restrict__ flag)
{
    int k = blockIdx.x * blockDim.x + threadIdx.x;
    if (k == 0) flag[0] = 0;
    if (k < cnt) aP[k] = a[src[k]];
}


struct EntryView {
    const int *ia, *ja;
// ... 1424 lines not shown
            resolve(mp_.xchg[l].opsX, xsol_.p, xchg_[l].opsX);
        }
    }
    if (mp_.maxSmallLds > 48 * 1024) {
        HIP_CHECK(hipFuncSetAttribute((const void*)k_front_fused<256>, hipFuncAttributeMaxDynamicSharedMemorySize, (int)mp_.maxSmallLds));
        HIP_CHECK(hipFuncSetAttribute((const void*)k_front_fused<512>, hipFuncAttributeMaxDynamicSharedMemorySize, (int)mp_.maxSmallLds));
    }
    configureSweepKernels(mp_.maxSolveLds, mp_.maxBwdLds, mp_.maxTriLds);
    HIP_CHECK(hipStreamSynchronize(stream));
    lap("uploads + attributes");
}

void MfNumeric::nodeOwners(std::vector<int>& ownerOfNode) const
{
    if (!sym_) throw StateError("nodeOwners before analyze_pattern");
    const MfSymbolic& sym = *sym_;
    ownerOfNode.assign(sym.nn, -1);
    if (world_ <= 1) return;
    std::vector<int> perm(sym.nn, -1);
    for (int s = 0; s < ns_; ++s)
        for (int v = sym.firstNode[s]; v < sym.firstNode[s + 1]; ++v) perm[v] = mp_.owner[s];
    for (int v = 0; v < sym.nn; ++v) ownerOfNode[v] = perm[sym.newOf[v]];
}

MfNumeric::~MfNumeric()
{
    if (side_) (void)hipStreamSynchronize(side_);
    if (fwd_) (void)hipStreamSynchronize(fwd_);
    for (hipEvent_t e : evFactLevel_) (void)hipEventDestroy(e);
    if (evRhs_) (void)hipEventDestroy(evRhs_);
    if (evFwdDone_) (void)hipEventDestroy(evFwdDone_);
    if (fwd_) (void)hipStreamDestroy(fwd_);
    for (hipEvent_t e : evLevel_) (void)hipEventDestroy(e);
    for (hipEvent_t e : evInvDone_) (void)hipEventDestroy(e);
    if (evSide_) (void)hipEventDestroy(evSide_);
    if (side_) (void)hipStreamDestroy(side_);
}

bool MfNumeric::factorize(const double* a_dev)
{
    if (!sym_) throw StateError("factorize before analyze_pattern");
    enqueueFactor(a_dev);
    if (world_ > 1) {
        allreduceFlag();
    }
    hipLaunchKernelGGL(k_publish_flag, dim3(1), dim3(1), 0, stream_, flag_.p, hflag_.dev);
    HIP_CHECK(hipStreamSynchronize(stream_));
#ifdef MF_FUSED_PROBE
    {
        static int calls = 0;
        if (++calls == 3) {
            std::vector<unsigned long long> h(16 << 16);
            HIP_CHECK(hipMemcpyFromSymbol(h.data(), HIP_SYMBOL(g_probe), h.size() * sizeof(unsigned long long)));
            const char* names[7] = { "maps", "children", "A", "panels", "store", "schur", "total" };
            for (int l = 0; l < nLevels_; ++l) {
                const LevelPlan& P = mp_.level[l];
                if (!P.small.cnt) continue;
                double sum[16] = { 0 }, mx = 0;
                for (int b = 0; b < P.small.cnt; ++b) {
                    const unsigned long long* r = h.data() + 16 * (size_t)((P.small.off + b) & 0xffff);
                    for (int k = 0; k < 6; ++k) sum[k] += (double)(r[k + 1] - r[k]);
                    sum[6] += (double)(r[6] - r[0]);
                    mx = std::max(mx, (double)(r[6] - r[0]));
                    for (int k = 8; k < 16; ++k) sum[k] += (double)r[k];
                }
                const double c = 0.01 / P.small.cnt;
                std::fprintf(stderr, "[fused probe] level %d: %d fronts, %d threads, N %.0f nc %.0f kids %.1f |", l, P.small.cnt, P.smallThreads, sum[12] / P.small.cnt, sum[13] / P.small.cnt,
                    sum[14] / P.small.cnt);
                for (int k = 0; k < 7; ++k) std::fprintf(stderr, " %s %.2f", names[k], sum[k] * c);
                std::fprintf(stderr, " us (max %.2f) | inside panels: pivot %.2f rows %.2f trailing %.2f | inside schur (wave 0): gathers %.2f products + stores %.2f\n", mx * 0.01, sum[8] * c, sum[9] * c,
                    sum[10] * c, sum[11] * c, sum[15] * c);
            }
        }
    }
#endif
    return pivotsOk();
}

bool MfNumeric::pivotsOk() const
{
    return hflag_.p[0] == 0;
}

bool MfNumeric::factorizeSolve(const double* a_dev, const double* rhs_dev, double* x_dev, bool wait)
{
    if (!sym_) throw StateError("factorize before analyze_pattern");
    if (world_ > 1 || !fwd_) {
        const bool ok = factorize(a_dev);
        if (ok) solve(rhs_dev, x_dev);
        return ok;
    }
    HIP_CHECK(hipEventRecord(evRhs_, stream_));
    HIP_CHECK(hipStreamWaitEvent(fwd_, evRhs_, 0));
    enqueuePermuteRhs(rhs_dev, fwd_);
    fwdJoined_ = false;
    enqueueFactor(a_dev, true);
    if (!fwdJoined_) HIP_CHECK(hipEventRecord(evFwdDone_, fwd_));
    hipLaunchKernelGGL(k_publish_flag, dim3(1), dim3(1), 0, stream_, flag_.p, hflag_.dev);
    if (!fwdJoined_) HIP_CHECK(hipStreamWaitEvent(stream_, evFwdDone_, 0));
    enqueueBackward(x_dev);
    if (!wait) return true;
    HIP_CHECK(hipStreamSynchronize(stream_));
    return pivotsOk();
}

void MfNumeric::enqueueFactor(const double* a_dev, bool overlapForward)
{
    TreeView tv{ frontOff_.p, idxPtr_.p, firstNode_.p, childPtr_.p, child_.p, invPtr_.p, inv_.p, idx_.p, dinvOff_.p };
    XinvView xvF{ xinvOff_.p, xinvX_.p, xinvT_.p };
    if (sidePending_) HIP_CHECK(hipStreamWaitEvent(stream_, evSide_, 0));
    bool sideUsed = false;
    int fwdNext = 0;
#ifdef MF_FUSED_PROBE
    {
        const int* base = fdesc_.p;
        HIP_CHECK(hipMemcpyToSymbolAsync(HIP_SYMBOL(g_probeBase), &base, sizeof(base), 0, hipMemcpyHostToDevice, stream_));
    }
#endif
    if (nFusedA_) hipLaunchKernelGGL(k_gather_a, dim3((nFusedA_ + 255) / 256), dim3(256), 0, stream_, nFusedA_, aSrc_.p, a_dev, aPerm_.p, flag_.p);
    else flag_.zero(stream_);
    for (int l = 0; l < nLevels_; ++l) {
        const LevelPlan& P = mp_.level[l];
        if (P.small.cnt)
        {
            const int* fd = fdesc_.p + (size_t)P.small.off * FD_STRIDE;
            if (P.smallThreads == 512)
                hipLaunchKernelGGL(k_front_fused<512>, dim3(P.small.cnt), dim3(512), P.smallLds, stream_, fd, inv_.p, aLoc_.p, aPerm_.p, fronts_.p,
                    dinv_.p, flag_.p);
            else
                hipLaunchKernelGGL(k_front_fused<256>, dim3(P.small.cnt), dim3(256), P.smallLds, stream_, fd, inv_.p, aLoc_.p, aPerm_.p, fronts_.p,
                    dinv_.p, flag_.p);
        }
        if (P.ea.cnt) {
            hipLaunchKernelGGL(k_extend_add, dim3(P.ea.cnt), dim3(WG), 0, stream_, eaDesc_.p + P.ea.off, bigFd_.p, inv_.p, fronts_.p, P.fuseEA ? 1 : 0, eaAPtr_.p,
                bigASrc_.p, bigADst_.p, a_dev);
        }
        for (const Range& R : P.step) {
            if (!R.cnt) continue;
            if (P.stepTop) hipLaunchKernelGGL(k_big_step<true>, dim3(R.cnt), dim3(WGB), 0, stream_, desc_.p + R.off, tv, fronts_.p, dinv_.p, flag_.p, xvF);
            else hipLaunchKernelGGL(k_big_step<false>, dim3(R.cnt), dim3(WGB), 0, stream_, desc_.p + R.off, tv, fronts_.p, dinv_.p, flag_.p, xvF);
            const Range& U = P.bulk[&R - P.step.data()];
            if (U.cnt) hipLaunchKernelGGL(k_big_bulk, dim3(U.cnt), dim3(WG), 0, stream_, desc_.p + U.off, fronts_.p);
        }
        if (P.schur.cnt) {
            if (P.fuseEA) hipLaunchKernelGGL(k_big_schur64_ea, dim3(P.schur.cnt), dim3(WG), 0, stream_, desc_.p + P.schur.off, bigFd_.p, inv_.p, fronts_.p);
            else if (P.schur64) hipLaunchKernelGGL(k_big_schur64, dim3(P.schur.cnt), dim3(WG), 0, stream_, desc_.p + P.schur.off, fronts_.p);
            else hipLaunchKernelGGL(k_big_schur, dim3(P.schur.cnt), dim3(WG), 0, stream_, desc_.p + P.schur.off, fronts_.p);
        }
        if (world_ > 1) exchangeUpdateMatrices(l);
        if (mp_.xinvLevel[l].blocks.cnt) {
            if (side_) {
                HIP_CHECK(hipEventRecord(evLevel_[l], stream_));
                HIP_CHECK(hipStreamWaitEvent(side_, evLevel_[l], 0));
                enqueueInverses(l, side_);
                HIP_CHECK(hipEventRecord(evInvDone_[l], side_));
                sideUsed = true;
            }
            else enqueueInverses(l, stream_);
        }
        if (overlapForward) {
            if (l == nLevels_ - 1 && !sideUsed) {
                HIP_CHECK(hipEventRecord(evFwdDone_, fwd_));
                HIP_CHECK(hipStreamWaitEvent(stream_, evFwdDone_, 0));
                enqueueForwardLevel(l, stream_);
                fwdJoined_ = true;
            }
            else if (l >= nLevels_ - 2 || (l + 1) % fwdStride_ == 0) {
                HIP_CHECK(hipEventRecord(evFactLevel_[l], stream_));
                HIP_CHECK(hipStreamWaitEvent(fwd_, evFactLevel_[l], 0));
                for (; fwdNext <= l; ++fwdNext) {
                    if (mp_.level[fwdNext].xinvFwd.cnt && sideUsed) HIP_CHECK(hipStreamWaitEvent(fwd_, evInvDone_[fwdNext], 0));
                    enqueueForwardLevel(fwdNext, fwd_);
                }
            }
        }
    }
    if (sideUsed) HIP_CHECK(hipEventRecord(evSide_, side_));
    sidePending_ = sideUsed;
}

void MfNumeric::enqueueInverses(int l, hipStream_t st)
{
    const XinvLevel& XL = mp_.xinvLevel[l];
// ... 11 lines not shown
```

ipc_amd/csrc/mf_sweeps.hip:

```cpp
#include "mf_kernels.h"
#include <string>
#include <vector>
#include <algorithm>

#ifndef FWD_NARROW
#define FWD_NARROW 1
#endif
#ifndef BWD_NARROW_MAX_N
#define BWD_NARROW_MAX_N 160
#endif

namespace ipcgpu {

namespace {

__global__ void k_permute_rhs(int nn, const int* __restrict__ newOf, const double* __restrict__ b, double* __restrict__ bp)
{
    int i = blockIdx.x * blockDim.x + threadIdx.x;
    if (i < 3 * nn) {
        int v = i / 3, d = i - 3 * v;
        bp[3 * newOf[v] + d] = b[i];
    }
}
__global__ void k_unpermute_x(int nn, const int* __restrict__ newOf, const double* __restrict__ xp, double* __restrict__ x)
{
    int i = blockIdx.x * blockDim.x + threadIdx.x;
    if (i < 3 * nn) {
        int v = i / 3, d = i - 3 * v;
        x[i] = xp[3 * newOf[v] + d];
    }
}

__device__ __forceinline__ double gather_w(const TreeView& tv, const long long* __restrict__ wOff, const double* __restrict__ wbuf,
    const double* __restrict__ bperm, int s, int nc, int I)
{
    const int cb = tv.childPtr[s], ce = tv.childPtr[s + 1];
    double val = (I < nc) ? bperm[3 * tv.firstNode[s] + I] : 0.0;
    const int In = I / 3, Id = I - 3 * In;
    for (int c0 = cb; c0 < ce; c0 += 4) {
        int ip[4];
        long long base[4];
#pragma unroll
        for (int q = 0; q < 4; ++q) {
            const int c = tv.child[min(c0 + q, ce - 1)];
            ip[q] = tv.invPtr[c];
            base[q] = wOff[c] + frontNc(tv, c) + Id;
        }
        int ic[4];
#pragma unroll
        for (int q = 0; q < 4; ++q) ic[q] = tv.inv[ip[q] + In];
        double v[4];
#pragma unroll
        for (int q = 0; q < 4; ++q) v[q] = wbuf[base[q] + 3 * max(ic[q], 0)];
#pragma unroll
        for (int q = 0; q < 4; ++q)
            if (c0 + q < ce && ic[q] >= 0) val += v[q];
    }
    return val;
}

template <int NT>
__device__ __forceinline__ void fwd_triangle(const double* __restrict__ L, int N, int nc, int rowEnd, const double* __restrict__ dblk,
    double* w1, int tid)
{
    double dn[NB], ln[NB];
    auto fetch = [&](int kb, const double* blk) {
        const int wd = min(NB, nc - kb);
        if (tid < NB) {
#pragma unroll
            for (int c = 0; c < NB; ++c) dn[c] = blk[c * NB + tid];
        }
        const int i = kb + wd + tid;
        if (i < rowEnd) {
#pragma unroll
            for (int k = 0; k < NB; ++k) ln[k] = (k < wd) ? L[i + (long long)N * (kb + k)] : 0.0;
        }
    };
    if (nc > 0) fetch(0, dblk);
    for (int kb = 0; kb < nc; kb += NB, dblk += NB * NB) {
        const int wd = min(NB, nc - kb);
        double y = 0.0;
        if (tid < NB) {
            double p0 = 0.0, p1 = 0.0, p2 = 0.0, p3 = 0.0;
#pragma unroll
            for (int c = 0; c < NB; c += 4) {
                p0 += dn[c] * ((c < wd) ? w1[kb + c] : 0.0);
                p1 += dn[c + 1] * ((c + 1 < wd) ? w1[kb + c + 1] : 0.0);
                p2 += dn[c + 2] * ((c + 2 < wd) ? w1[kb + c + 2] : 0.0);
                p3 += dn[c + 3] * ((c + 3 < wd) ? w1[kb + c + 3] : 0.0);
            }
            y = (p0 + p1) + (p2 + p3);
        }
        __syncthreads();
        if (tid < wd) w1[kb + tid] = y;
        __syncthreads();
        const int i0 = kb + wd + tid;
        double acc0 = 0.0;
        if (i0 < rowEnd) {
            double p0 = 0.0, p1 = 0.0, p2 = 0.0, p3 = 0.0;
#pragma unroll
            for (int k = 0; k < NB; k += 4) {
                p0 += ln[k] * ((k < wd) ? w1[kb + k] : 0.0);
                p1 += ln[k + 1] * ((k + 1 < wd) ? w1[kb + k + 1] : 0.0);
                p2 += ln[k + 2] * ((k + 2 < wd) ? w1[kb + k + 2] : 0.0);
                p3 += ln[k + 3] * ((k + 3 < wd) ? w1[kb + k + 3] : 0.0);
            }
            acc0 = (p0 + p1) + (p2 + p3);
        }
        if (kb + NB < nc) fetch(kb + NB, dblk + NB * NB);
        if (i0 < rowEnd) w1[i0] -= acc0;
        for (int i = i0 + NT; i < rowEnd; i += NT) {
            double acc = 0.0;
#pragma unroll 8
// ... 287 lines not shown
        for (; c + 3 < ce; c += 4) {
            double x[4];
#pragma unroll
            for (int u = 0; u < 4; ++u) x[u] = Xr[(long long)nc * (c + u)];
#pragma unroll
            for (int u = 0; u < 4; u += 2) {
                acc0 += x[u] * w1[c + u];
                acc1 += x[u + 1] * w1[c + u + 1];
            }
        }
        for (; c < ce; ++c) acc0 += Xr[(long long)nc * c] * w1[c];
    }
    part[tid] = acc0 + acc1;
    __syncthreads();
    if (cg == 0 && r < nc) {
        double tot = 0.0;
#pragma unroll
        for (int g = 0; g < NCG; ++g) tot += part[g * MV_ROWS + lane];
        yperm[3 * tv.firstNode[s] + r] = tot;
    }
}

__global__ __launch_bounds__(WG) void k_xinv_bwd(const int4* __restrict__ desc, TreeView tv, XinvView xv, const double* __restrict__ yperm,
    double* __restrict__ xsol)
{
    extern __shared__ double tt[];
    const int4 d = desc[blockIdx.x];
    const int s = d.x, c0 = d.y;
    const int nc = frontNc(tv, s);
    const double* X = xv.X + xv.xOff[s];
    const int col0 = 3 * tv.firstNode[s];
    const int lane = threadIdx.x & 63, wave = threadIdx.x >> 6;
    for (int r = c0 + threadIdx.x; r < nc; r += WG) tt[r - c0] = yperm[col0 + r];
    __syncthreads();
    int cq[4];
    double acc[4] = { 0.0, 0.0, 0.0, 0.0 };
#pragma unroll
    for (int q = 0; q < 4; ++q) cq[q] = c0 + wave + 4 * q;
    for (int r0 = c0 + wave; r0 < nc; r0 += 128) {
        const int ra = r0 + lane, rb = r0 + 64 + lane;
        const double ta = (ra < nc) ? tt[min(ra, nc - 1) - c0] : 0.0, tb = (rb < nc) ? tt[min(rb, nc - 1) - c0] : 0.0;
        double va[4], vb[4];
#pragma unroll
        for (int q = 0; q < 4; ++q) {
            const double* Xc = X + (long long)nc * min(cq[q], nc - 1);
            va[q] = Xc[min(ra, nc - 1)];
            vb[q] = Xc[min(rb, nc - 1)];
        }
#pragma unroll
        for (int q = 0; q < 4; ++q) acc[q] += ((ra >= cq[q]) ? va[q] * ta : 0.0) + ((rb >= cq[q]) ? vb[q] * tb : 0.0);
    }
#pragma unroll
    for (int q = 0; q < 4; ++q) {
        double t = acc[q];
#pragma unroll
        for (int off = 32; off > 0; off >>= 1) t += __shfl_down(t, off, 64);
        if (lane == 0 && cq[q] < min(nc, c0 + 16)) xsol[col0 + cq[q]] = t;
    }
}

}

void MfNumeric::configureSweepKernels(size_t maxSolveLds, size_t maxBwdLds, size_t maxTriLds)
{
    if (mp_.xinvLds > 48 * 1024) {
        HIP_CHECK(hipFuncSetAttribute((const void*)k_xinv_fwd, hipFuncAttributeMaxDynamicSharedMemorySize, (int)mp_.xinvLds));
        HIP_CHECK(hipFuncSetAttribute((const void*)k_xinv_bwd, hipFuncAttributeMaxDynamicSharedMemorySize, (int)mp_.xinvLds));
    }
    if (maxSolveLds > 48 * 1024) {
        HIP_CHECK(hipFuncSetAttribute((const void*)k_fwd_level<256>, hipFuncAttributeMaxDynamicSharedMemorySize, (int)maxSolveLds));
        HIP_CHECK(hipFuncSetAttribute((const void*)k_fwd_level<128>, hipFuncAttributeMaxDynamicSharedMemorySize, (int)maxSolveLds));
        HIP_CHECK(hipFuncSetAttribute((const void*)k_bwd_level<256>, hipFuncAttributeMaxDynamicSharedMemorySize, (int)maxSolveLds));
        HIP_CHECK(hipFuncSetAttribute((const void*)k_bwd_level<128>, hipFuncAttributeMaxDynamicSharedMemorySize, (int)maxSolveLds));
    }
    if (maxBwdLds > 48 * 1024)
        HIP_CHECK(hipFuncSetAttribute((const void*)k_big_bwd_init, hipFuncAttributeMaxDynamicSharedMemorySize, (int)maxBwdLds));
    if (maxTriLds > 48 * 1024) {
        if (maxTriLds > 150 * 1024) throw StateError("a separator front is too wide for the single-workgroup triangular sweep");
        HIP_CHECK(hipFuncSetAttribute((const void*)k_big_fwd_tri, hipFuncAttributeMaxDynamicSharedMemorySize, (int)maxTriLds));
        HIP_CHECK(hipFuncSetAttribute((const void*)k_big_bwd_tri, hipFuncAttributeMaxDynamicSharedMemorySize, (int)maxTriLds));
    }
}

void MfNumeric::enqueuePermuteRhs(const double* rhs_dev, hipStream_t st)
{
    const int n3 = sym_->n;
    hipLaunchKernelGGL(k_permute_rhs, dim3((n3 + 255) / 256), dim3(256), 0, st, sym_->nn, newOf_.p, rhs_dev, bperm_.p);
}

void MfNumeric::solve(const double* rhs_dev, double* x_dev)
{
    if (!sym_) throw StateError("solve before analyze_pattern");
    enqueueSolve(rhs_dev, x_dev);
}

void MfNumeric::enqueueSolve(const double* rhs_dev, double* x_dev)
{
    enqueuePermuteRhs(rhs_dev, stream_);
    for (int l = 0; l < nLevels_; ++l) {
        const LevelPlan& P = mp_.level[l];
        if (P.xinvFwd.cnt && sidePending_) HIP_CHECK(hipStreamWaitEvent(stream_, evInvDone_[l], 0));
        enqueueForwardLevel(l, stream_);
        if (world_ > 1) exchangeUpdateVectors(l);
    }
    enqueueBackward(x_dev);
}

void MfNumeric::enqueueForwardLevel(int l, hipStream_t st)
{
    TreeView tv{ frontOff_.p, idxPtr_.p, firstNode_.p, childPtr_.p, child_.p, invPtr_.p, inv_.p, idx_.p, dinvOff_.p };
    XinvView xv{ xinvOff_.p, xinvX_.p, xinvT_.p };
    const LevelPlan& P = mp_.level[l];
    if (P.small.cnt)
    {
        if (FWD_NARROW && P.solveLds <= BWD_NARROW_MAX_N * sizeof(double))
            hipLaunchKernelGGL(k_fwd_level<128>, dim3(P.small.cnt), dim3(128), P.solveLds, st, smallList_.p + P.small.off, tv, wOff_.p, fronts_.p, dinv_.p, w_.p,
                bperm_.p, yperm_.p);
        else
            hipLaunchKernelGGL(k_fwd_level<256>, dim3(P.small.cnt), dim3(WG), P.solveLds, st, smallList_.p + P.small.off, tv, wOff_.p, fronts_.p, dinv_.p, w_.p,
                bperm_.p, yperm_.p);
    }
    if (P.bigTri.cnt)
        hipLaunchKernelGGL(k_big_fwd_tri, dim3(P.bigTri.cnt), dim3(WGT), P.triLds, st, triList_.p + P.bigTri.off, tv, wOff_.p, fronts_.p, dinv_.p, w_.p,
            bperm_.p, yperm_.p);
    if (P.xinvFwd.cnt)
        hipLaunchKernelGGL(k_xinv_fwd, dim3(P.xinvFwd.cnt), dim3(WG), mp_.xinvLds, st, xinvDesc_.p + P.xinvFwd.off, tv, xv, wOff_.p, w_.p, bperm_.p, yperm_.p);
    if (P.fwdRect.cnt)
        hipLaunchKernelGGL(k_big_fwd_rect, dim3(P.fwdRect.cnt), dim3(WG), 0, st, desc_.p + P.fwdRect.off, tv, wOff_.p, fronts_.p, w_.p, yperm_.p);
}

void MfNumeric::enqueueBackward(double* x_dev)
{
    const MfSymbolic& sym = *sym_;
    TreeView tv{ frontOff_.p, idxPtr_.p, firstNode_.p, childPtr_.p, child_.p, invPtr_.p, inv_.p, idx_.p, dinvOff_.p };
    XinvView xv{ xinvOff_.p, xinvX_.p, xinvT_.p };
    const int n3 = sym.n;
#ifdef MF_BWD_PROBE
    static int probeCall = 0;
    const bool probe = ++probeCall == 40;
    std::vector<hipEvent_t> pe;
    std::vector<std::string> pn;
    auto mark = [&](const char* what, int l) {
        if (!probe) return;
        hipEvent_t e;
        HIP_CHECK(hipEventCreate(&e));
        HIP_CHECK(hipEventRecord(e, stream_));
        pe.push_back(e);
        pn.push_back(std::string(what) + " L" + std::to_string(l));
    };
    mark("start", nLevels_);
#else
    auto mark = [](const char*, int) {};
#endif
    for (int l = nLevels_ - 1; l >= 0; --l) {
        const LevelPlan& P = mp_.level[l];
        if (P.bwdInit.cnt)
            hipLaunchKernelGGL(k_big_bwd_init, dim3(P.bwdInit.cnt), dim3(WG), P.bwdLds, stream_, desc_.p + P.bwdInit.off, tv, fronts_.p, yperm_.p,
                xsol_.p);
        if (P.bwdInit.cnt) mark("bwd_init", l);
        if (P.bigTri.cnt)
            hipLaunchKernelGGL(k_big_bwd_tri, dim3(P.bigTri.cnt), dim3(WGT), P.triLds, stream_, triList_.p + P.bigTri.off, tv, fronts_.p,
                dinv_.p, yperm_.p, xsol_.p);
        if (P.bigTri.cnt) mark("bwd_tri", l);
        if (P.xinvBwd.cnt)
            hipLaunchKernelGGL(k_xinv_bwd, dim3(P.xinvBwd.cnt), dim3(WG), mp_.xinvLds, stream_, xinvDesc_.p + P.xinvBwd.off, tv, xv, yperm_.p,
                xsol_.p);
        if (P.small.cnt) {
            if (P.solveLds <= BWD_NARROW_MAX_N * sizeof(double))
                hipLaunchKernelGGL(k_bwd_level<128>, dim3(P.small.cnt), dim3(128), P.solveLds, stream_, smallList_.p + P.small.off, tv, fronts_.p, dinv_.p,
                    yperm_.p, xsol_.p);
            else
                hipLaunchKernelGGL(k_bwd_level<256>, dim3(P.small.cnt), dim3(WG), P.solveLds, stream_, smallList_.p + P.small.off, tv, fronts_.p, dinv_.p,
                    yperm_.p, xsol_.p);
        }
        if (P.xinvBwd.cnt || P.small.cnt) mark("xinv/small", l);
        if (world_ > 1) exchange(xchg_[l].opsX);
    }
#ifdef MF_BWD_PROBE
    if (probe) {
        HIP_CHECK(hipStreamSynchronize(stream_));
        for (size_t i = 1; i < pe.size(); ++i) {
            float ms = 0;
            HIP_CHECK(hipEventElapsedTime(&ms, pe[i - 1], pe[i]));
            fprintf(stderr, "bwd probe: %-16s %7.1f us\n", pn[i].c_str(), 1e3 * ms);
        }
    }
#endif
    if (world_ > 1) reduceSolution();
    hipLaunchKernelGGL(k_unpermute_x, dim3((n3 + 255) / 256), dim3(256), 0, stream_, sym.nn, newOf_.p, xsol_.p, x_dev);
}

}
```

ipc_amd/csrc/nh_kernels.h:

```cpp
#pragma once
#include <hip/hip_runtime.h>

namespace ipcgpu {

struct ElemView {
    int nV, nT;
    int tetBegin, tetEnd;
    int energyType;
    const double* x;
    const double* xTilde;
    const double* mass;
    const int* dbc;
    const int4* tet;
    const double* A;
    const double* vol;
    const double* mu;
    const double* lam;
    const int* rowBase;
    const int* rowLen;
    const int* edgeP0;
};

void launch_node_init(const ElemView& v, int projectDBC, bool ownerRank, double* a, double* grad, hipStream_t s);

void launch_assemble(const ElemView& v, double coef, int projectDBC, double* grad ,
    double* a , hipStream_t s);
const char* assemble_kernel_name();

void launch_energy(const ElemView& v, double coef, bool withInertia, bool ownerRank, double* partial, int partialCap,
    double* out, hipStream_t s);
void launch_energy_per_elem(const ElemView& v, double* perElem, hipStream_t s);
void launch_stress_elements(const ElemView& v, double* rec, int* nInvalid, hipStream_t s);
void launch_stress_nodes(int nV, int nT, const int* ptr, const int* elems, const double* vol, const double* rec, double* out, hipStream_t s);
void launch_system_report(const ElemView& v, const double* xStart, const int* slices, int nNodeSlices, int nSlices, const int* nodeStart,
    const int* tetStart, int nComp, double dt, const double* g3, double* rec, double* out, hipStream_t s);

void launch_check_inversion(const ElemView& v, int* flag, hipStream_t s);
void launch_inversion_step(const ElemView& v, const double* p, double slackness, double tMax, double* outMin, hipStream_t s);

void launch_step_forward(int n3, const double* x0, const double* p, double alpha, double* x, hipStream_t s);
void launch_trial_step(int n3, const double* x0, const double* p, const double* filterMin, bool useFilter, double* alphaOut, double* x, hipStream_t s);
void launch_max_abs(int n, const double* v, double* out , hipStream_t s);
void launch_trial_step_fused(int n3, double* x, double* x0, const double* p, const double* filterMin, bool useFilter, double* alphaOut, hipStream_t s);
void launch_iter_reset(double* scalar, int* flag, hipStream_t s);
void launch_publish2(const void* a, void* da, int na, const void* b, void* db, int nb, hipStream_t s);
void launch_fill(double* p, size_t n, double v, hipStream_t s);
void launch_negate(int n, const double* in, double* out, hipStream_t s);
void launch_publish(const void* src_dev, void* dst_mapped, int nWords, hipStream_t s);
void launch_colmajor_to_aos(int nV, const double* src, double* dst, hipStream_t s);
void launch_aos_to_colmajor(int nV, const double* src, double* dst, hipStream_t s);
void launch_csr_symv(int nRows, const int* ia, const int* ja, const double* a, const double* x, double* y, hipStream_t s);
void launch_apply_host_updates(long long nnz, const double* delta, const unsigned char* mask, const double* setVal, double* a, hipStream_t s);
void launch_precond_diag(int nRows, const int* ia, const double* a, const double* in, double* out, hipStream_t s);
void launch_be_update(int nV, const int* dbc, const double* x, const double* xPrev, double* xPrevOut, double* vel, double* acc, double* dxElastic, double* xTilde,
    double dt, double gx, double gy, double gz, hipStream_t s);
void launch_nm_update(int nV, const int* dbc, const double* x, double* xPrevOut, double* vel, double* acc, double* dxElastic, double* xTilde,
    double dt, double beta, double gamma, double gx, double gy, double gz, hipStream_t s);
struct DbcMotion {
    double R[9];
    double c[3];
    double linDt[3];
};
void launch_gather3(int n, const int* ids, const double* x, double* out, hipStream_t s);
void launch_target_positions(int n, const int* ids, const double* x, const double* p, double* pos, double* pOut, hipStream_t s);
void launch_dbc_motion(int n, const int* ids, const DbcMotion& m, const double* x, double* p, hipStream_t s);
void launch_dbc_targets(int n, const int* ids, const double* target_3n, const double* x, double* p, hipStream_t s);
void launch_nbc_gradient(int n, const int* ids, const int* dbc, const double* mass, const double* dtSqA3, double* g, hipStream_t s);
void launch_nbc_energy(int n, const int* ids, const int* dbc, const double* mass, const double* x, const double* dtSqA3, double* out, hipStream_t s);
struct MdbcView {
    int n;
    const int* ids;
    const double* pos;
    double* lam;
    const double* mass;
};
void launch_clear_projected(int nV, const int* dbc, int projectDBC, double* g, hipStream_t s);
void launch_keep_mine3(int nV, const unsigned char* mine, double* g, hipStream_t s);
void launch_keep_mine_rows(int nRows, const unsigned char* mine, const int* ia, double* a, hipStream_t s);
void launch_damp_dx(int nV, const int* dbc, int mode, int projectDBC, const double* x, const double* xPrev, double* dx, hipStream_t s);
void launch_damp_clear_diag(int nV, const int* dbc, const int* ia, double* d, hipStream_t s);
void launch_axpy(long long n, double alpha, const double* x, double* y, hipStream_t s);
void launch_dot_scaled(int n, const double* x, const double* y, double scale, double* out, hipStream_t s);
void launch_dot2(int n, const double* g, const double* e, double* partial, int partialCap, double* out2, hipStream_t s);
void launch_mdbc_reduce(const MdbcView& m, const double* x, double rho, int mode , double* out, hipStream_t s);
void launch_mdbc_gradient(const MdbcView& m, const double* x, double rho, double* g, hipStream_t s);
void launch_mdbc_hessian(const MdbcView& m, const int* ia, double rho, double* a, hipStream_t s);
void launch_mdbc_lambda(const MdbcView& m, const double* x, double rho, hipStream_t s);
void launch_warm_dir(int nV, const int* dbc, const double* vel, const double* dx, double dt, const double* cgDtSqG3, double ce, double* p,
    hipStream_t s);
void launch_twist_dir(int nH, const int* ids, const double* ang, double cy, double cz, const double* x, double* p, hipStream_t s);

}
```

ipc_amd/csrc/nh_kernels.hip:

```cpp
#include "nh_device.h"
#include <algorithm>
#include <cfloat>
#include <cstdlib>

namespace ipcgpu {

namespace {

constexpr int BLOCK = 256;

using namespace dev;

struct GlobalAtomicSink {
    const ElemView& v;
    int t;
    int vid[4];
    double* gptr;
    double* a;
    __device__ __forceinline__ void grad(int k, int i, double g) { atomicAdd(&gptr[3 * (size_t)vid[k] + i], g); }
    __device__ __forceinline__ bool wantPair(int, int, int) const { return true; }
    __device__ __forceinline__ void diagBlock(int ka, const double H[3][3])
    {
        const int base = v.rowBase[vid[ka]], Lr = v.rowLen[vid[ka]];
        atomicAdd(&a[base + 0], H[0][0]);
// ... 6 lines not shown
    __device__ __forceinline__ void offBlock(int e, int ka, int kc, bool aFirst, const double H[3][3])
    {
        const int p0 = v.edgeP0[(size_t)e * v.nT + t];
        const int Lr = v.rowLen[vid[aFirst ? ka : kc]];
#pragma unroll
        for (int r = 0; r < 3; ++r) {
            const int rowOff = (r == 0) ? 0 : (r == 1 ? (Lr - 1) : (2 * Lr - 3));
#pragma unroll
            for (int c = 0; c < 3; ++c) atomicAdd(&a[p0 + rowOff + c], aFirst ? H[r][c] : H[c][r]);
        }
    }
};

template <bool HESS>
__global__ __launch_bounds__(BLOCK) void k_assemble(ElemView v, double coef, int projectDBC, double* __restrict__ grad,
    double* __restrict__ a)
{
    const int t = v.tetBegin + blockIdx.x * BLOCK + threadIdx.x;
    if (t >= v.tetEnd) return;
    const int4 tv = v.tet[t];
    GlobalAtomicSink sink{ v, t, { tv.x, tv.y, tv.z, tv.w }, grad, a };
    assemble_element<HESS>(v, t, coef, projectDBC, grad != nullptr, sink);
}

__global__ __launch_bounds__(BLOCK) void k_node_init(ElemView v, int projectDBC, int owner, double* __restrict__ a,
    double* __restrict__ grad)
{
    const int n = blockIdx.x * BLOCK + threadIdx.x;
    if (n >= v.nV) return;
    const int type = v.dbc[n];
    const bool proj = projected_dbc(type, projectDBC);
    if (grad) {
        double g[3] = { 0, 0, 0 };
        if (!proj && owner) {
            const double m = v.mass[n];
#pragma unroll
            for (int i = 0; i < 3; ++i) g[i] = m * (v.x[3 * (size_t)n + i] - v.xTilde[3 * (size_t)n + i]);
        }
#pragma unroll
        for (int i = 0; i < 3; ++i) grad[3 * (size_t)n + i] = g[i];
    }
    if (a && owner) {
        const int base = v.rowBase[n], Lr = v.rowLen[n];
        const double d = proj ? 1.0 : v.mass[n];
        a[base] = d;
        a[base + Lr] = d;
        a[base + 2 * Lr - 1] = d;
    }
}

__device__ __forceinline__ double block_sum(double x, double* sm)
{
#pragma unroll
    for (int off = 32; off > 0; off >>= 1) x += __shfl_down(x, off, 64);
    const int lane = threadIdx.x & 63, wv = threadIdx.x >> 6;
    if (lane == 0) sm[wv] = x;
    __syncthreads();
    double r = 0.0;
    if (threadIdx.x == 0) {
        for (int i = 0; i < BLOCK / 64; ++i) r += sm[i];
    }
    return r;
}

__device__ __forceinline__ double nh_psi(const double F[9], double mu, double lam)
{
    if (mu == 0.0 && lam == 0.0) return 0.0;
    double I1 = 0.0;
#pragma unroll
    for (int i = 0; i < 9; ++i) I1 += F[i] * F[i];
    const double lJ = log(det3(F));
    return mu / 2.0 * (I1 - 3.0) - (mu - lam / 2.0 * lJ) * lJ;
}

__device__ __forceinline__ double elem_psi(const ElemView& v, const double F[9], double mu, double lam)
{
    if (v.energyType != 1) return nh_psi(F, mu, lam);
    if (mu == 0.0 && lam == 0.0) return 0.0;
    double U[9], s[3], V[9];
    svd3(F, U, s, V);
    return fcr_psi(s, mu, lam);
}

__global__ __launch_bounds__(BLOCK) void k_energy(ElemView v, double coef, int withInertia, int owner, double* __restrict__ partial)
{
    __shared__ double sm[BLOCK / 64];
    const int gid = blockIdx.x * BLOCK + threadIdx.x;
    double e = 0.0;
    const int t = v.tetBegin + gid;
    if (t < v.tetEnd) {
        const int4 tv = v.tet[t];
        double A[9], F[9];
        load_A(v, t, A);
        deformation_gradient(ld3(v.x, tv.x), ld3(v.x, tv.y), ld3(v.x, tv.z), ld3(v.x, tv.w), A, F);
        e = coef * v.vol[t] * elem_psi(v, F, v.mu[t], v.lam[t]);
    }
    if (withInertia && owner && gid < v.nV) {
        double d2 = 0.0;
#pragma unroll
        for (int i = 0; i < 3; ++i) {
            double d = v.x[3 * (size_t)gid + i] - v.xTilde[3 * (size_t)gid + i];
            d2 += d * d;
        }
        e += d2 * v.mass[gid] / 2.0;
    }
    double r = block_sum(e, sm);
    if (threadIdx.x == 0) partial[blockIdx.x] = r;
}

__global__ __launch_bounds__(BLOCK) void k_reduce_partials(const double* __restrict__ partial, int n, double* __restrict__ out)
{
    __shared__ double sm[BLOCK / 64];
    double x = 0.0;
    for (int i = threadIdx.x; i < n; i += BLOCK) x += partial[i];
    double r = block_sum(x, sm);
    if (threadIdx.x == 0) out[0] = r;
}

__global__ __launch_bounds__(BLOCK) void k_energy_per_elem(ElemView v, double* __restrict__ out)
{
    const int t = blockIdx.x * BLOCK + threadIdx.x;
    if (t >= v.nT) return;
    const int4 tv = v.tet[t];
    double A[9], F[9];
    load_A(v, t, A);
    deformation_gradient(ld3(v.x, tv.x), ld3(v.x, tv.y), ld3(v.x, tv.z), ld3(v.x, tv.w), A, F);
    out[t] = v.vol[t] * elem_psi(v, F, v.mu[t], v.lam[t]);
}

constexpr int STRESS_Q = 8;

__device__ __forceinline__ double von_mises(double sxx, double syy, double szz, double sxy, double syz, double sxz)
{
    const double a = sxx - syy, b = syy - szz, c = szz - sxx;
    return sqrt(0.5 * (a * a + b * b + c * c) + 3.0 * (sxy * sxy + syz * syz + sxz * sxz));
}

template <bool FCR>
__global__ __launch_bounds__(BLOCK) void k_stress_elements(ElemView v, double* __restrict__ out, int* __restrict__ nInvalid)
{
    const int t = blockIdx.x * BLOCK + threadIdx.x;
    bool invalid = false;
    if (t < v.nT) {
        const int4 tv = v.tet[t];
        double A[9], F[9];
        load_A(v, t, A);
        deformation_gradient(ld3(v.x, tv.x), ld3(v.x, tv.y), ld3(v.x, tv.z), ld3(v.x, tv.w), A, F);
        const double mu = v.mu[t], lam = v.lam[t];
        const double J = det3(F);
        double s[6] = { 0.0, 0.0, 0.0, 0.0, 0.0, 0.0 }, vm = 0.0, Jout = J;
        if (!(mu == 0.0 && lam == 0.0)) {
            if (!FCR && !(J > 0.0)) {
                invalid = true;
                const double nan = __longlong_as_double(0x7ff8000000000000LL);
#pragma unroll
                for (int k = 0; k < 6; ++k) s[k] = nan;
                vm = Jout = nan;
            }
            else {
                double G[9];
                double isoJ, iso;
                if (FCR) {
                    double U[9], sv[3], V[9];
                    svd3(F, U, sv, V);
#pragma unroll
                    for (int j = 0; j < 3; ++j)
#pragma unroll
                        for (int i = 0; i < 3; ++i) G[i + 3 * j] = 2.0 * (F[i + 3 * j] - (U[i] * V[j] + U[i + 3] * V[j + 3] + U[i + 6] * V[j + 6]));
                    isoJ = 0.0;
                    iso = lam * (J - 1.0);
                }
                else {
#pragma unroll
                    for (int i = 0; i < 9; ++i) G[i] = F[i];
                    isoJ = lam * log(J) - mu;
                    iso = 0.0;
                }
                auto gft = [&](int i, int j) { return G[i] * F[j] + G[i + 3] * F[j + 3] + G[i + 6] * F[j + 6]; };
                s[0] = (mu * gft(0, 0) + isoJ) / J + iso;
                s[1] = (mu * gft(1, 1) + isoJ) / J + iso;
                s[2] = (mu * gft(2, 2) + isoJ) / J + iso;
                s[3] = mu * (0.5 * (gft(0, 1) + gft(1, 0))) / J;
                s[4] = mu * (0.5 * (gft(1, 2) + gft(2, 1))) / J;
                s[5] = mu * (0.5 * (gft(0, 2) + gft(2, 0))) / J;
                vm = von_mises(s[0], s[1], s[2], s[3], s[4], s[5]);
            }
        }
#pragma unroll
// ... 18 lines not shown
        w += ve;
#pragma unroll
        for (int c = 0; c < 6; ++c) s[c] += ve * rec[(size_t)c * nT + e];
    }
    if (k1 > ptr[n]) {
#pragma unroll
        for (int c = 0; c < 6; ++c) s[c] /= w;
    }
#pragma unroll
    for (int c = 0; c < 6; ++c) out[(size_t)c * nV + n] = s[c];
    out[(size_t)(STRESS_Q - 2) * nV + n] = von_mises(s[0], s[1], s[2], s[3], s[4], s[5]);
    out[(size_t)(STRESS_Q - 1) * nV + n] = w;
}

constexpr int REPORT_Q = 7;

__device__ __forceinline__ double wave_sum(double x)
{
#pragma unroll
    for (int off = 32; off > 0; off >>= 1) x += __shfl_down(x, off, 64);
    return x;
}

__global__ __launch_bounds__(BLOCK) void k_report_slices(ElemView v, const double* __restrict__ xStart, const int* __restrict__ slices, int nNodeSlices,
    double dt, double gx, double gy, double gz, double* __restrict__ rec)
{
    __shared__ double sm[REPORT_Q][BLOCK / 64];
    const int b = blockIdx.x, lane = threadIdx.x & 63, wv = threadIdx.x >> 6;
    const int i = slices[3 * b + 1] + threadIdx.x;
    const bool live = i < slices[3 * b + 2];
    const int nq = b < nNodeSlices ? REPORT_Q : 1;
    double q[REPORT_Q] = { 0.0, 0.0, 0.0, 0.0, 0.0, 0.0, 0.0 };
    if (live && b < nNodeSlices) {
        const d3 x = ld3(v.x, i), x0 = ld3(xStart, i);
        const double m = v.mass[i];
        const double dx = x.x - x0.x, dy = x.y - x0.y, dz = x.z - x0.z;
        q[0] = m * ((dx * dx + dy * dy + dz * dz) / (dt * dt) / 2.0 - (gx * x.x + gy * x.y + gz * x.z));
        const double mdt = m / dt;
        q[1] = mdt * dx;
        q[2] = mdt * dy;
        q[3] = mdt * dz;
        q[4] = x.y * q[3] - x.z * q[2];
        q[5] = x.z * q[1] - x.x * q[3];
        q[6] = x.x * q[2] - x.y * q[1];
    }
    else if (live) {
        const int4 tv = v.tet[i];
        double A[9], F[9];
        load_A(v, i, A);
        deformation_gradient(ld3(v.x, tv.x), ld3(v.x, tv.y), ld3(v.x, tv.z), ld3(v.x, tv.w), A, F);
        q[0] = v.vol[i] * elem_psi(v, F, v.mu[i], v.lam[i]);
    }
#pragma unroll
    for (int k = 0; k < REPORT_Q; ++k)
        if (k < nq) {
            const double r = wave_sum(q[k]);
            if (lane == 0) sm[k][wv] = r;
        }
    __syncthreads();
    if (threadIdx.x < nq) {
        double r = 0.0;
#pragma unroll
        for (int w = 0; w < BLOCK / 64; ++w) r += sm[threadIdx.x][w];
        rec[REPORT_Q * (size_t)b + threadIdx.x] = r;
    }
}

__global__ __launch_bounds__(64) void k_report_components(const double* __restrict__ rec, const int* __restrict__ nodeStart,
    const int* __restrict__ tetStart, double* __restrict__ out)
{
    const int c = blockIdx.x, lane = threadIdx.x;
    const int n0 = nodeStart[c], n1 = nodeStart[c + 1], t0 = tetStart[c], t1 = tetStart[c + 1];
#pragma unroll
    for (int k = 0; k < REPORT_Q; ++k) {
        double a = 0.0;
        for (int j = n0 + lane; j < n1; j += 64) a += rec[REPORT_Q * (size_t)j + k];
        if (k == 0)
            for (int j = t0 + lane; j < t1; j += 64) a += rec[REPORT_Q * (size_t)j];
        a = wave_sum(a);
        if (lane == 0) out[REPORT_Q * (size_t)c + k] = a;
    }
}

__global__ __launch_bounds__(BLOCK) void k_check_inversion(ElemView v, int* flag)
{
    const int t = v.tetBegin + blockIdx.x * BLOCK + threadIdx.x;
    if (t >= v.tetEnd) return;
    if (!(v.mu[t] != 0.0 && v.lam[t] != 0.0)) return;
    const int4 tv = v.tet[t];
    const d3 x0 = ld3(v.x, tv.x), x1 = ld3(v.x, tv.y), x2 = ld3(v.x, tv.z), x3 = ld3(v.x, tv.w);
    const double e[9] = { x1.x - x0.x, x1.y - x0.y, x1.z - x0.z, x2.x - x0.x, x2.y - x0.y, x2.z - x0.z, x3.x - x0.x,
        x3.y - x0.y, x3.z - x0.z };
    if (det3(e) < 0.0) atomicOr(flag, 1);
}

struct cplx {
    double re, im;
};
__device__ __forceinline__ cplx cmul(cplx a, cplx b) { return { a.re * b.re - a.im * b.im, a.re * b.im + a.im * b.re }; }
__device__ __forceinline__ cplx cadd(cplx a, cplx b) { return { a.re + b.re, a.im + b.im }; }
__device__ __forceinline__ cplx csub(cplx a, cplx b) { return { a.re - b.re, a.im - b.im }; }
__device__ __forceinline__ cplx cscale(cplx a, double s) { return { a.re * s, a.im * s }; }
__device__ __forceinline__ cplx cdiv(cplx a, cplx b)
{
    double d = b.re * b.re + b.im * b.im;
    return { (a.re * b.re + a.im * b.im) / d, (a.im * b.re - a.re * b.im) / d };
}
__device__ __forceinline__ double cabs_(cplx a) { return hypot(a.re, a.im); }
__device__ __forceinline__ cplx csqrt_(cplx z)
{
    if (z.re == 0.0 && z.im == 0.0) return { 0.0, 0.0 };
    double m = cabs_(z);
    double t = sqrt(0.5 * (m + fabs(z.re)));
    if (z.re >= 0.0) return { t, z.im / (2.0 * t) };
    return { fabs(z.im) / (2.0 * t), copysign(t, z.im) };
}
__device__ __forceinline__ cplx cpow_third(cplx z)
{
    if (z.re == 0.0 && z.im == 0.0) return { 0.0, 0.0 };
    if (z.im == 0.0 && z.re > 0.0) return { cbrt(z.re), 0.0 };
    double r = cbrt(cabs_(z)), th = atan2(z.im, z.re) / 3.0;
    return { r * cos(th), r * sin(th) };
}
__device__ double quad_root(double a, double b, double c, double tol)
{
    double t;
    if (fabs(a) <= tol) t = -c / b;
    else {
        double desc = b * b - 4 * a * c;
        if (desc > 0) {
            t = (-b - sqrt(desc)) / (2 * a);
            if (t < 0) t = (-b + sqrt(desc)) / (2 * a);
        }
        else t = -1;
    }
    return t;
}
__device__ double cubic_root(double a, double b, double c, double d, double tol)
{
    double t = -1;
    if (fabs(a) <= tol) return quad_root(b, c, d, tol);
    cplx delta0 = { b * b - 3 * a * c, 0 };
    cplx delta1 = { 2 * b * b * b - 9 * a * b * c + 27 * a * a * d, 0 };
    cplx disc = csqrt_(csub(cmul(delta1, delta1), cscale(cmul(cmul(delta0, delta0), delta0), 4.0)));
    cplx C = cpow_third(cscale(cadd(delta1, disc), 0.5));
    if (cabs_(C) == 0.0) C = cpow_third(cscale(csub(delta1, disc), 0.5));
    const double h = sqrt(3.0) / 2.0;
    cplx u2 = { -0.5, h }, u3 = { -0.5, -h };
    cplx bb = { b, 0 };
    double m3a = -3.0 * a;
    cplx t1 = cscale(cadd(cadd(bb, C), cdiv(delta0, C)), 1.0 / m3a);
    cplx u2C = cmul(u2, C), u3C = cmul(u3, C);
    cplx t2 = cscale(cadd(cadd(bb, u2C), cdiv(delta0, u2C)), 1.0 / m3a);
    cplx t3 = cscale(cadd(cadd(bb, u3C), cdiv(delta0, u3C)), 1.0 / m3a);
    if ((fabs(t1.im) < tol) && (t1.re > 0)) t = t1.re;
    if ((fabs(t2.im) < tol) && (t2.re > 0) && ((t2.re < t) || (t < 0))) t = t2.re;
    if ((fabs(t3.im) < tol) && (t3.re > 0) && ((t3.re < t) || (t < 0))) t = t3.re;
    return t;
}

__global__ __launch_bounds__(BLOCK) void k_inversion_step(ElemView v, const double* __restrict__ p, double slackness, double tMax,
    unsigned long long* __restrict__ outMin)
{
    const int t = v.tetBegin + blockIdx.x * BLOCK + threadIdx.x;
    double res = 1e20;
    if (t < v.tetEnd) {
        const int4 tv = v.tet[t];
        const d3 x0 = ld3(v.x, tv.x), x1 = ld3(v.x, tv.y), x2 = ld3(v.x, tv.z), x3 = ld3(v.x, tv.w);
        const d3 p0 = ld3(p, tv.x), p1 = ld3(p, tv.y), p2 = ld3(p, tv.z), p3 = ld3(p, tv.w);
        const double v0[3] = { x1.x - x0.x, x1.y - x0.y, x1.z - x0.z }, v1[3] = { x2.x - x0.x, x2.y - x0.y, x2.z - x0.z },
                     v2[3] = { x3.x - x0.x, x3.y - x0.y, x3.z - x0.z };
        const double q0[3] = { p1.x - p0.x, p1.y - p0.y, p1.z - p0.z }, q1[3] = { p2.x - p0.x, p2.y - p0.y, p2.z - p0.z },
                     q2[3] = { p3.x - p0.x, p3.y - p0.y, p3.z - p0.z };
        auto cross = [](const double* x, const double* y, double* z) {
            z[0] = x[1] * y[2] - x[2] * y[1];
            z[1] = x[2] * y[0] - x[0] * y[2];
            z[2] = x[0] * y[1] - x[1] * y[0];
        };
        auto dot = [](const double* x, const double* y) { return x[0] * y[0] + x[1] * y[1] + x[2] * y[2]; };
        double pxp[3], vxp[3], pxv[3], vxv[3], mix[3];
        cross(q0, q1, pxp);
        cross(v0, q1, vxp);
        cross(q0, v1, pxv);
        cross(v0, v1, vxv);
        for (int c = 0; c < 3; ++c) mix[c] = vxp[c] + pxv[c];
        const double a = dot(q2, pxp);
        const double b = dot(v2, pxp) + dot(q2, mix);
        const double c = dot(q2, vxv) + dot(v2, mix);
        const double d = (1.0 - slackness) * dot(v2, vxv);
        const double lower = d + tMax * (fmin(c, 0.0) + tMax * (fmin(b, 0.0) + tMax * fmin(a, 0.0)));
        if (!(lower > 0.01 * d)) {
            const double r = cubic_root(a, b, c, d, 1.0e-6);
            res = (r >= 0) ? r : 1e20;
        }
    }
#pragma unroll
    for (int off = 32; off > 0; off >>= 1) res = fmin(res, __shfl_down(res, off, 64));
    if ((threadIdx.x & 63) == 0 && res < 1e20) atomicMin(outMin, (unsigned long long)__double_as_longlong(res));
}

__global__ void k_step_forward(int n, const double* __restrict__ x0, const double* __restrict__ p, double alpha, double* __restrict__ x)
{
    int i = blockIdx.x * blockDim.x + threadIdx.x;
    if (i < n) x[i] = x0[i] + alpha * p[i];
}
__global__ void k_trial_alpha(const double* __restrict__ filterMin, int useFilter, double* __restrict__ alphaOut)
{
    double alpha = 1.0;
    const double t = filterMin[0];
    if (useFilter && t > 0.0 && t < alpha) alpha = t;
    alphaOut[0] = alpha;
}
__global__ void k_step_forward_dev(int n, const double* __restrict__ x0, const double* __restrict__ p, const double* __restrict__ alphaPtr,
    double* __restrict__ x)
{
    const double alpha = alphaPtr[0];
    int i = blockIdx.x * blockDim.x + threadIdx.x;
    if (i < n) x[i] = x0[i] + alpha * p[i];
}
__global__ void k_trial_step_fused(int n, double* __restrict__ x, double* __restrict__ x0, const double* __restrict__ p, const double* __restrict__ filterMin,
    int useFilter, double* __restrict__ alphaOut)
{
    double alpha = 1.0;
    const double t = filterMin[0];
    if (useFilter && t > 0.0 && t < alpha) alpha = t;
    const int i = blockIdx.x * blockDim.x + threadIdx.x;
    if (i == 0) alphaOut[0] = alpha;
    if (i < n) {
        const double xi = x[i];
        x0[i] = xi;
        x[i] = xi + alpha * p[i];
    }
}
__global__ void k_iter_reset(double* __restrict__ scalar, int* __restrict__ flag)
{
    scalar[3] = 0.0;
    scalar[2] = 1e20;
    flag[0] = 0;
}
__global__ void k_publish2(const unsigned* __restrict__ a, unsigned* __restrict__ da, int na, const unsigned* __restrict__ b, unsigned* __restrict__ db, int nb)
{
    const int i = threadIdx.x;
    if (i < na) da[i] = a[i];
    if (i < nb) db[i] = b[i];
}
__global__ __launch_bounds__(BLOCK) void k_max_abs(int n, const double* __restrict__ v, unsigned long long* __restrict__ out)
{
    __shared__ double sm[BLOCK / 64];
    double m = 0.0;
    for (int i = blockIdx.x * BLOCK + threadIdx.x; i < n; i += gridDim.x * BLOCK) m = fmax(m, fabs(v[i]));
#pragma unroll
    for (int off = 32; off > 0; off >>= 1) m = fmax(m, __shfl_down(m, off, 64));
    if ((threadIdx.x & 63) == 0) sm[threadIdx.x >> 6] = m;
    __syncthreads();
    if (threadIdx.x == 0) {
        for (int w = 1; w < BLOCK / 64; ++w) m = fmax(m, sm[w]);
        atomicMax(out, (unsigned long long)__double_as_longlong(m));
    }
}
__global__ void k_fill(double* p, size_t n, double v)
{
    size_t i = (size_t)blockIdx.x * blockDim.x + threadIdx.x;
    if (i < n) p[i] = v;
}
__global__ void k_negate(int n, const double* __restrict__ in, double* __restrict__ out)
{
    int i = blockIdx.x * blockDim.x + threadIdx.x;
    if (i < n) out[i] = -in[i];
}
__global__ void k_colmajor_to_aos(int nV, const double* __restrict__ src, double* __restrict__ dst)
{
    int i = blockIdx.x * blockDim.x + threadIdx.x;
    if (i < 3 * nV) {
        int v = i / 3, c = i % 3;
        dst[i] = src[v + (size_t)nV * c];
    }
}
__global__ void k_aos_to_colmajor(int nV, const double* __restrict__ src, double* __restrict__ dst)
{
    int i = blockIdx.x * blockDim.x + threadIdx.x;
    if (i < 3 * nV) {
// ... 257 lines not shown
}
__global__ void k_mdbc_lambda(int n, const int* __restrict__ ids, const double* __restrict__ pos, double* __restrict__ lam,
    const double* __restrict__ mass, const double* __restrict__ x, double rho)
{
    int i = blockIdx.x * blockDim.x + threadIdx.x;
    if (i >= 3 * n) return;
    const int t = i / 3, c = i - 3 * t;
    const size_t v = (size_t)ids[t];
    lam[i] -= rho * sqrt(mass[v]) * (x[3 * v + c] - pos[i]);
}

inline int nblk(long long n, int b = BLOCK) { return (int)((n + b - 1) / b); }

}

void launch_node_init(const ElemView& v, int projectDBC, bool ownerRank, double* a, double* grad, hipStream_t s)
{
    if (v.nV) hipLaunchKernelGGL(k_node_init, dim3(nblk(v.nV)), dim3(BLOCK), 0, s, v, projectDBC, ownerRank ? 1 : 0, a, grad);
}

void launch_assemble(const ElemView& v, double coef, int projectDBC, double* grad, double* a, hipStream_t s)
{
    const int n = v.tetEnd - v.tetBegin;
    if (n <= 0) return;
    if (a) hipLaunchKernelGGL(k_assemble<true>, dim3(nblk(n)), dim3(BLOCK), 0, s, v, coef, projectDBC, grad, a);
    else hipLaunchKernelGGL(k_assemble<false>, dim3(nblk(n)), dim3(BLOCK), 0, s, v, coef, projectDBC, grad, a);
}
const char* assemble_kernel_name() { return "k_assemble"; }

void launch_energy(const ElemView& v, double coef, bool withInertia, bool ownerRank, double* partial, int partialCap, double* out,
    hipStream_t s)
{
    const int n = std::max(v.tetEnd - v.tetBegin, withInertia ? v.nV : 0);
    const int nb = std::max(1, nblk(n));
    (void)partialCap;
    hipLaunchKernelGGL(k_energy, dim3(nb), dim3(BLOCK), 0, s, v, coef, withInertia ? 1 : 0, ownerRank ? 1 : 0, partial);
    hipLaunchKernelGGL(k_reduce_partials, dim3(1), dim3(BLOCK), 0, s, partial, nb, out);
}
void launch_energy_per_elem(const ElemView& v, double* perElem, hipStream_t s)
{
    if (v.nT) hipLaunchKernelGGL(k_energy_per_elem, dim3(nblk(v.nT)), dim3(BLOCK), 0, s, v, perElem);
}
void launch_stress_elements(const ElemView& v, double* rec, int* nInvalid, hipStream_t s)
{
    if (!v.nT) return;
    if (v.energyType == 1) hipLaunchKernelGGL(k_stress_elements<true>, dim3(nblk(v.nT)), dim3(BLOCK), 0, s, v, rec, nInvalid);
    else hipLaunchKernelGGL(k_stress_elements<false>, dim3(nblk(v.nT)), dim3(BLOCK), 0, s, v, rec, nInvalid);
}
void launch_stress_nodes(int nV, int nT, const int* ptr, const int* elems, const double* vol, const double* rec, double* out, hipStream_t s)
{
    if (nV) hipLaunchKernelGGL(k_stress_nodes, dim3(nblk(nV)), dim3(BLOCK), 0, s, nV, nT, ptr, elems, vol, rec, out);
}
void launch_system_report(const ElemView& v, const double* xStart, const int* slices, int nNodeSlices, int nSlices, const int* nodeStart,
    const int* tetStart, int nComp, double dt, const double* g3, double* rec, double* out, hipStream_t s)
{
    if (nSlices)
        hipLaunchKernelGGL(k_report_slices, dim3(nSlices), dim3(BLOCK), 0, s, v, xStart, slices, nNodeSlices, dt, g3[0], g3[1], g3[2], rec);
    hipLaunchKernelGGL(k_report_components, dim3(nComp), dim3(64), 0, s, rec, nodeStart, tetStart, out);
}
void launch_check_inversion(const ElemView& v, int* flag, hipStream_t s)
{
    const int n = v.tetEnd - v.tetBegin;
    if (n > 0) hipLaunchKernelGGL(k_check_inversion, dim3(nblk(n)), dim3(BLOCK), 0, s, v, flag);
}
void launch_inversion_step(const ElemView& v, const double* p, double slackness, double tMax, double* outMin, hipStream_t s)
{
    const int n = v.tetEnd - v.tetBegin;
    if (n > 0)
        hipLaunchKernelGGL(k_inversion_step, dim3(nblk(n)), dim3(BLOCK), 0, s, v, p, slackness, tMax, (unsigned long long*)outMin);
}
void launch_step_forward(int n3, const double* x0, const double* p, double alpha, double* x, hipStream_t s)
{
    if (n3) hipLaunchKernelGGL(k_step_forward, dim3(nblk(n3)), dim3(BLOCK), 0, s, n3, x0, p, alpha, x);
}
void launch_trial_step(int n3, const double* x0, const double* p, const double* filterMin, bool useFilter, double* alphaOut, double* x, hipStream_t s)
{
    hipLaunchKernelGGL(k_trial_alpha, dim3(1), dim3(1), 0, s, filterMin, useFilter ? 1 : 0, alphaOut);
    if (n3) hipLaunchKernelGGL(k_step_forward_dev, dim3(nblk(n3)), dim3(BLOCK), 0, s, n3, x0, p, (const double*)alphaOut, x);
}
void launch_trial_step_fused(int n3, double* x, double* x0, const double* p, const double* filterMin, bool useFilter, double* alphaOut, hipStream_t s)
{
    hipLaunchKernelGGL(k_trial_step_fused, dim3(std::max(nblk(n3), 1)), dim3(BLOCK), 0, s, n3, x, x0, p, filterMin, useFilter ? 1 : 0, alphaOut);
}
void launch_iter_reset(double* scalar, int* flag, hipStream_t s) { hipLaunchKernelGGL(k_iter_reset, dim3(1), dim3(1), 0, s, scalar, flag); }
void launch_publish2(const void* a, void* da, int na, const void* b, void* db, int nb, hipStream_t s)
{
    hipLaunchKernelGGL(k_publish2, dim3(1), dim3(64), 0, s, (const unsigned*)a, (unsigned*)da, na, (const unsigned*)b, (unsigned*)db, nb);
}
void launch_max_abs(int n, const double* v, double* out, hipStream_t s)
{
    if (n) hipLaunchKernelGGL(k_max_abs, dim3(std::min(nblk(n), 256)), dim3(BLOCK), 0, s, n, v, (unsigned long long*)out);
}
void launch_fill(double* p, size_t n, double v, hipStream_t s)
{
    if (n) hipLaunchKernelGGL(k_fill, dim3(nblk((long long)n)), dim3(BLOCK), 0, s, p, n, v);
}
void launch_negate(int n, const double* in, double* out, hipStream_t s)
{
    if (n) hipLaunchKernelGGL(k_negate, dim3(nblk(n)), dim3(BLOCK), 0, s, n, in, out);
}
void launch_colmajor_to_aos(int nV, const double* src, double* dst, hipStream_t s)
{
    if (nV) hipLaunchKernelGGL(k_colmajor_to_aos, dim3(nblk(3LL * nV)), dim3(BLOCK), 0, s, nV, src, dst);
}
void launch_aos_to_colmajor(int nV, const double* src, double* dst, hipStream_t s)
{
    if (nV) hipLaunchKernelGGL(k_aos_to_colmajor, dim3(nblk(3LL * nV)), dim3(BLOCK), 0, s, nV, src, dst);
}
void launch_csr_symv(int nRows, const int* ia, const int* ja, const double* a, const double* x, double* y, hipStream_t s)
{
    if (!nRows) return;
    hipLaunchKernelGGL(k_csr_symv_zero, dim3(nblk(nRows)), dim3(BLOCK), 0, s, nRows, y);
    hipLaunchKernelGGL(k_csr_symv, dim3(nblk(nRows)), dim3(BLOCK), 0, s, nRows, ia, ja, a, x, y);
}
__global__ void k_apply_host_updates(long long nnz, const double* __restrict__ delta, const unsigned char* __restrict__ mask,
    const double* __restrict__ setVal, double* __restrict__ a)
{
    const long long k = (long long)blockIdx.x * blockDim.x + threadIdx.x;
    if (k < nnz) a[k] = (mask && mask[k]) ? setVal[k] + delta[k] : a[k] + delta[k];
}
void launch_apply_host_updates(long long nnz, const double* delta, const unsigned char* mask, const double* setVal, double* a, hipStream_t s)
{
    if (nnz) hipLaunchKernelGGL(k_apply_host_updates, dim3(nblk(nnz)), dim3(BLOCK), 0, s, nnz, delta, mask, setVal, a);
}
void launch_precond_diag(int nRows, const int* ia, const double* a, const double* in, double* out, hipStream_t s)
{
    if (nRows) hipLaunchKernelGGL(k_precond_diag, dim3(nblk(nRows)), dim3(BLOCK), 0, s, nRows, ia, a, in, out);
}
void launch_nm_update(int nV, const int* dbc, const double* x, double* xPrevOut, double* vel, double* acc, double* dxElastic, double* xTilde,
    double dt, double beta, double gamma, double gx, double gy, double gz, hipStream_t s)
{
    hipLaunchKernelGGL(k_nm_update, dim3((3 * nV + 255) / 256), dim3(256), 0, s, nV, dbc, x, xPrevOut, vel, acc, dxElastic, xTilde, dt, beta, gamma,
        gx, gy, gz);
}
void launch_be_update(int nV, const int* dbc, const double* x, const double* xPrev, double* xPrevOut, double* vel, double* acc, double* dxElastic, double* xTilde,
    double dt, double gx, double gy, double gz, hipStream_t s)
{
    if (nV)
        hipLaunchKernelGGL(k_be_update, dim3(nblk(3LL * nV)), dim3(BLOCK), 0, s, nV, dbc, x, xPrev, xPrevOut, vel, acc, dxElastic, xTilde, dt, gx, gy,
            gz);
}
void launch_warm_dir(int nV, const int* dbc, const double* vel, const double* dx, double dt, const double* cgDtSqG3, double ce, double* p,
    hipStream_t s)
{
    if (nV) hipLaunchKernelGGL(k_warm_dir, dim3(nblk(3LL * nV)), dim3(BLOCK), 0, s, nV, dbc, vel, dx, dt, cgDtSqG3[0], cgDtSqG3[1], cgDtSqG3[2], ce, p);
}
void launch_twist_dir(int nH, const int* ids, const double* ang, double cy, double cz, const double* x, double* p, hipStream_t s)
{
    if (nH) hipLaunchKernelGGL(k_twist_dir, dim3(nblk(nH)), dim3(BLOCK), 0, s, nH, ids, ang, cy, cz, x, p);
}

void launch_nbc_gradient(int n, const int* ids, const int* dbc, const double* mass, const double* dtSqA3, double* g, hipStream_t s)
{
    if (n) hipLaunchKernelGGL(k_nbc_gradient, dim3(nblk(n)), dim3(BLOCK), 0, s, n, ids, dbc, mass, dtSqA3[0], dtSqA3[1], dtSqA3[2], g);
}
void launch_nbc_energy(int n, const int* ids, const int* dbc, const double* mass, const double* x, const double* dtSqA3, double* out, hipStream_t s)
{
    hipLaunchKernelGGL(k_nbc_energy, dim3(1), dim3(BLOCK), 0, s, n, ids, dbc, mass, x, dtSqA3[0], dtSqA3[1], dtSqA3[2], out);
}
void launch_damp_dx(int nV, const int* dbc, int mode, int projectDBC, const double* x, const double* xPrev, double* dx, hipStream_t s)
{
    if (nV) hipLaunchKernelGGL(k_damp_dx, dim3(nblk(3LL * nV)), dim3(BLOCK), 0, s, nV, dbc, mode, projectDBC, x, xPrev, dx);
}
void launch_damp_clear_diag(int nV, const int* dbc, const int* ia, double* d, hipStream_t s)
{
    if (nV) hipLaunchKernelGGL(k_damp_clear_diag, dim3(nblk(3LL * nV)), dim3(BLOCK), 0, s, nV, dbc, ia, d);
// ... 72 lines not shown
```

ipc_amd/lib.py:

```python
from __future__ import annotations

import ctypes as C
import os
import re

import numpy as np

_HERE = os.path.dirname(os.path.abspath(__file__))
_LIB_PATH = os.path.join(_HERE, "libipcgpu_%s.so" % os.environ["IPCGPU_LIB_VARIANT"] if os.environ.get("IPCGPU_LIB_VARIANT") else "libipcgpu.so")
_HEADER = os.path.join(_HERE, "..", "include", "ipcgpu.h")

c_dp = C.POINTER(C.c_double)
c_ip = C.POINTER(C.c_int)

IPCGPU_OK = 0
IPCGPU_NOT_PD = 1
SOLVER_MULTIFRONTAL = 0
SOLVER_ROCSOLVER_CSRRF = 1
SOLVER_PCG = 2
PRECOND_BLOCK_JACOBI = 0
PRECOND_LAGGED_CHOLESKY = 1
PRECOND_TWO_LEVEL = 2

ALLREDUCE_FN = C.CFUNCTYPE(C.c_int, C.c_void_p, C.c_void_p, C.c_longlong, C.c_int)
# ... 243 lines not shown
        self._chk(self._L.ipcgpu_set_mesh(self.h, C.c_int(self.nV), C.c_int(self.nT), _dp(V), _ip(F),
                                          C.c_double(YM), C.c_double(PR), C.c_double(density)))

    def set_dbc(self, ids, typ):
        ids = _i32(ids)
        self._chk(self._L.ipcgpu_set_dbc(self.h, C.c_int(len(ids)), _ip(ids), C.c_int(typ)))

    def set_component_material(self, node_range, tet_range, density, YM, PR):
        self._chk(self._L.ipcgpu_set_component_material(self.h, C.c_int(node_range[0]), C.c_int(node_range[1]), C.c_int(tet_range[0]),
                                                        C.c_int(tet_range[1]), C.c_double(density), C.c_double(YM), C.c_double(PR)))

    def set_components(self, node_end, tet_end):
        node_end, tet_end = _i32(node_end).ravel(), _i32(tet_end).ravel()
        if len(node_end) != len(tet_end):
            raise ValueError("set_components: one node end and one element end per component")
        self._chk(self._L.ipcgpu_opt_set_components(self.h, C.c_int(len(node_end)), _ip(node_end), _ip(tet_end)))
        self._ncomp = len(node_end)

    def system_report(self):
        n = getattr(self, "_ncomp", 1)
        E, M, L = np.zeros(n), np.zeros((n, 3)), np.zeros((n, 3))
        self._chk(self._L.ipcgpu_opt_system_report(self.h, _dp(E), _dp(M), _dp(L)))
        return E, M, L

    def set_energy_type(self, name):
        self._chk(self._L.ipcgpu_set_energy_type(self.h, C.c_int({"NH": 0, "FCR": 1}[name])))

    def clear_dbc(self):
        self._chk(self._L.ipcgpu_clear_dbc(self.h))

    def set_positions(self, V):
        V = np.asfortranarray(V, dtype=np.float64)
        assert V.shape == (self.nV, 3)
        self._chk(self._L.ipcgpu_set_positions(self.h, _dp(V)))

    def get_positions(self):
        V = np.zeros((self.nV, 3), order="F")
        self._chk(self._L.ipcgpu_get_positions(self.h, _dp(V)))
        return V

    def set_xtilde(self, V):
        V = np.asfortranarray(V, dtype=np.float64)
        self._chk(self._L.ipcgpu_set_xtilde(self.h, _dp(V)))

    def features(self):
        A = np.zeros((self.nT, 9))
        vol = np.zeros(self.nT)
        mass = np.zeros(self.nV)
        mu = np.zeros(self.nT)
        lam = np.zeros(self.nT)
        self._chk(self._L.ipcgpu_get_features(self.h, _dp(A), _dp(vol), _dp(mass), _dp(mu), _dp(lam)))
        return dict(restTriInv=A, triArea=vol, mass=mass, mu=mu, lam=lam)

    def check_inversion(self):
        ok = C.c_int()
        self._chk(self._L.ipcgpu_check_inversion(self.h, C.byref(ok)))
        return bool(ok.value)

    def elastic_energy(self, coef=1.0):
        E = C.c_double()
        self._chk(self._L.ipcgpu_elastic_energy(self.h, C.c_double(coef), C.byref(E)))
        return E.value

    def elastic_energy_per_elem(self):
        out = np.zeros(self.nT)
        self._chk(self._L.ipcgpu_elastic_energy_per_elem(self.h, _dp(out)))
        return out

    def elastic_stress(self, nodal=True):
        elem = np.zeros((self.nT, 8), order="F")
        node = np.zeros((self.nV, 8), order="F") if nodal else None
        n = C.c_int()
        self._chk(self._L.ipcgpu_elastic_stress(self.h, _dp(elem), _dp(node), C.byref(n)))
        return elem, node, n.value

    def elastic_gradient(self, coef=1.0, projectDBC=True):
        g = np.zeros(3 * self.nV)
        self._chk(self._L.ipcgpu_elastic_gradient(self.h, C.c_double(coef), C.c_int(int(projectDBC)), _dp(g)))
        return g

    def elastic_hessian_add(self, coef=1.0, projectDBC=True):
        self._chk(self._L.ipcgpu_elastic_hessian_add(self.h, C.c_double(coef), C.c_int(int(projectDBC))))

    def filter_step_size(self, p, step=1.0):
        p = _f64(p)
        s = C.c_double(step)
        self._chk(self._L.ipcgpu_filter_step_size(self.h, _dp(p), C.byref(s)))
        return s.value

    def set_pattern(self, extra_pairs=None):
        if extra_pairs is None or len(extra_pairs) == 0:
            self._chk(self._L.ipcgpu_linsys_set_pattern(self.h, C.c_int(0), None))
        else:
            e = _i32(extra_pairs)
            self._chk(self._L.ipcgpu_linsys_set_pattern(self.h, C.c_int(e.shape[0]), _ip(e)))

    def set_pattern_csr(self, ia, ja):
        ia, ja = _i32(ia), _i32(ja)
        self._chk(self._L.ipcgpu_linsys_set_pattern_csr(self.h, C.c_int(len(ia) - 1), _ip(ia), _ip(ja)))

    def get_dims(self):
        n, nnz = C.c_int(), C.c_int()
        self._chk(self._L.ipcgpu_linsys_get_dims(self.h, C.byref(n), C.byref(nnz)))
        return n.value, nnz.value

    def get_pattern(self):
        n, nnz = self.get_dims()
        ia = np.zeros(n + 1, dtype=np.int32)
        ja = np.zeros(nnz, dtype=np.int32)
        self._chk(self._L.ipcgpu_linsys_get_pattern(self.h, _ip(ia), _ip(ja)))
        return ia, ja

    def set_zero(self):
        self._chk(self._L.ipcgpu_linsys_set_zero(self.h))

    def get_a(self):
        _, nnz = self.get_dims()
        a = np.zeros(nnz)
        self._chk(self._L.ipcgpu_linsys_get_values(self.h, _dp(a)))
        return a

    def set_a(self, a):
        a = _f64(a)
        self._chk(self._L.ipcgpu_linsys_set_values(self.h, _dp(a)))

    def add_coeff(self, r, c, v):
        self._chk(self._L.ipcgpu_linsys_add_coeff(self.h, C.c_int(r), C.c_int(c), C.c_double(v)))

    def set_coeff(self, r, c, v):
        self._chk(self._L.ipcgpu_linsys_set_coeff(self.h, C.c_int(r), C.c_int(c), C.c_double(v)))

    def multiply(self, x):
        x = _f64(x)
        y = np.zeros_like(x)
        self._chk(self._L.ipcgpu_linsys_multiply(self.h, _dp(x), _dp(y)))
        return y

    def multiply_sym(self, x):
        x = _f64(x)
        y = np.zeros_like(x)
        self._chk(self._L.ipcgpu_linsys_multiply_sym(self.h, _dp(x), _dp(y)))
        return y

    def set_iterative(self, rel_tol=1e-5, max_iter=1000, precond=PRECOND_BLOCK_JACOBI, max_factor_age=1):
        self._chk(self._L.ipcgpu_linsys_set_iterative(self.h, C.c_double(rel_tol), C.c_int(max_iter), C.c_int(precond), C.c_int(max_factor_age)))

    def iter_stats(self):
        o = np.zeros(6)
        self._chk(self._L.ipcgpu_linsys_iter_stats(self.h, _dp(o)))
        return dict(iterations=int(o[0]), residual=float(o[1]), converged=int(o[2]), factorizations=int(o[3]), factor_age=int(o[4]), syncs=int(o[5]))

    def coarse_stats(self):
        o = np.zeros(5)
        self._chk(self._L.ipcgpu_linsys_coarse_stats(self.h, _dp(o)))
        return dict(aggregates=int(o[0]), coarse_rows=int(o[1]), coarse_nnz=int(o[2]), coarse_factorizations=int(o[3]), jacobi_fallbacks=int(o[4]))

    def coarse_dims(self):
        a, r, z = C.c_int(), C.c_int(), C.c_int()
        self._chk(self._L.ipcgpu_linsys_coarse_dims(self.h, C.byref(a), C.byref(r), C.byref(z)))
        return a.value, r.value, z.value

    def coarse_get(self, values=True):
        _, rows, nnz = self.coarse_dims()
        n, _ = self.get_dims()
        agg = np.zeros(n // 3, dtype=np.int32)
        cia, cja = np.zeros(rows + 1, dtype=np.int32), np.zeros(nnz, dtype=np.int32)
        ca = np.zeros(nnz) if values else None
        self._chk(self._L.ipcgpu_linsys_coarse_get(self.h, _ip(agg), _ip(cia), _ip(cja), _dp(ca)))
        return agg, cia, cja, ca

    def analyze_pattern(self):
        self._chk(self._L.ipcgpu_linsys_analyze_pattern(self.h))

    def factorize(self):
        return self._chk(self._L.ipcgpu_linsys_factorize(self.h), allow_not_pd=True) == IPCGPU_OK

    def solve(self, rhs):
        rhs = _f64(rhs)
        x = np.zeros_like(rhs)
        self._chk(self._L.ipcgpu_linsys_solve(self.h, _dp(rhs), _dp(x)))
        return x

    def precondition_diag(self, v):
        v = _f64(v)
        out = np.zeros_like(v)
        self._chk(self._L.ipcgpu_linsys_precondition_diag(self.h, _dp(v), _dp(out)))
        return out

    def set_solver_tuning(self, bulk_min_mb=48.0, bulk_block=256):
        self._chk(self._L.ipcgpu_linsys_set_tuning(self.h, C.c_double(bulk_min_mb), C.c_int(bulk_block)))

    def linsys_stats(self):
        st = np.zeros(4)
        self._chk(self._L.ipcgpu_linsys_stats(self.h, _dp(st)))
        return dict(nnzL=st[0], flops=st[1], fronts=int(st[2]), levels=int(st[3]))

    def set_surface(self, SF, codim_edges=None):
        SF = np.asfortranarray(np.asarray(SF, dtype=np.int32).reshape(-1, 3))
        if codim_edges is None or len(codim_edges) == 0:
            self._chk(self._L.ipcgpu_set_surface(self.h, C.c_int(SF.shape[0]), _ip(SF)))
            return
        CE = np.ascontiguousarray(codim_edges, dtype=np.int32).reshape(-1, 2)
        self._chk(self._L.ipcgpu_set_surface_codim(self.h, C.c_int(SF.shape[0]), _ip(SF), C.c_int(CE.shape[0]), _ip(CE)))

    def set_exact_predicates(self, on=True):
        self._chk(self._L.ipcgpu_set_exact_predicates(self.h, C.c_int(int(on))))

    def set_codim_nodes(self, ids, mass):
        ids = _i32(ids)
        m = _f64(np.asarray(mass, dtype=np.float64))
        self._chk(self._L.ipcgpu_set_codim_nodes(self.h, C.c_int(len(ids)), _ip(ids), _dp(m)))

    def set_obstacle(self, ids, obstacle_only=False):
        ids = _i32(ids)
        self._chk(self._L.ipcgpu_set_obstacle_nodes(self.h, C.c_int(len(ids)), _ip(ids), C.c_int(int(obstacle_only))))

    def get_surface(self):
        n = np.zeros(3, dtype=np.int32)
        self._chk(self._L.ipcgpu_get_surface(self.h, _ip(n), None, None))
        svi = np.zeros(n[0], dtype=np.int32)
        sfe = np.zeros((n[2], 2), dtype=np.int32)
        self._chk(self._L.ipcgpu_get_surface(self.h, _ip(n), _ip(svi), _ip(sfe)))
        return svi, sfe

    def contact_build(self, dHat):
        n = np.zeros(3, dtype=np.int32)
        self._chk(self._L.ipcgpu_contact_build(self.h, C.c_double(dHat), _ip(n)))
        a = np.zeros((n[0], 4), dtype=np.int32)
        p = np.zeros((n[1], 4), dtype=np.int32)
        q = np.zeros((n[1], 2), dtype=np.int32)
        cs = np.zeros((n[2], 2), dtype=np.int32)
        self._chk(self._L.ipcgpu_contact_get(self.h, _ip(a), _ip(p), _ip(q), _ip(cs)))
        return dict(active=a, para=p, para_eiej=q, cs_ptee=cs)

    def contact_set(self, active, para=None, para_eiej=None):
        a = np.ascontiguousarray(active, dtype=np.int32).reshape(-1, 4)
        p = np.ascontiguousarray(para if para is not None else np.zeros((0, 4)), dtype=np.int32).reshape(-1, 4)
        q = np.ascontiguousarray(para_eiej if para_eiej is not None else np.zeros((0, 2)), dtype=np.int32).reshape(-1, 2)
        self._chk(self._L.ipcgpu_contact_set(self.h, C.c_int(a.shape[0]), _ip(a), C.c_int(p.shape[0]), _ip(p), _ip(q)))

    def contact_energy(self, dHat, kappa):
        E = C.c_double()
        self._chk(self._L.ipcgpu_contact_energy(self.h, C.c_double(dHat), C.c_double(kappa), C.byref(E)))
        return E.value

    def contact_gradient_add(self, dHat, kappa, projectDBC=True, grad=None):
        g = np.zeros(3 * self.nV) if grad is None else _f64(grad).copy()
        self._chk(self._L.ipcgpu_contact_gradient_add(self.h, C.c_double(dHat), C.c_double(kappa), C.c_int(int(projectDBC)), _dp(g)))
        return g

    def contact_held(self):
        n = np.zeros(3, dtype=np.int32)
        self._chk(self._L.ipcgpu_contact_counts(self.h, _ip(n)))
        a, p, q = np.zeros((n[0], 4), dtype=np.int32), np.zeros((n[1], 4), dtype=np.int32), np.zeros((n[1], 2), dtype=np.int32)
        self._chk(self._L.ipcgpu_contact_get(self.h, _ip(a), _ip(p), _ip(q), None))
        return dict(active=a, para=p, para_eiej=q)

    def contact_evaluate(self, tuples):
        t = np.ascontiguousarray(tuples, dtype=np.int32).reshape(-1, 4)
        val = np.zeros(t.shape[0])
        self._chk(self._L.ipcgpu_contact_evaluate(self.h, C.c_int(t.shape[0]), _ip(t), _dp(val)))
        return val

    def contact_report(self, dHat=None, kappa=None, x_prev=None, eps2=None, coef=None):
# ... 225 lines not shown
    def friction_energy(self, Vt, eps2, coef):
        Vt = np.asfortranarray(Vt, dtype=np.float64)
        E = C.c_double()
        self._chk(self._L.ipcgpu_friction_energy(self.h, _dp(Vt), C.c_double(eps2), C.c_double(coef), C.byref(E)))
        return E.value

    def friction_gradient_add(self, Vt, eps2, coef, grad=None):
        Vt = np.asfortranarray(Vt, dtype=np.float64)
        g = np.zeros(3 * self.nV) if grad is None else _f64(grad).copy()
        self._chk(self._L.ipcgpu_friction_gradient_add(self.h, _dp(Vt), C.c_double(eps2), C.c_double(coef), _dp(g)))
        return g

    def friction_hessian_add(self, Vt, eps2, coef, projectDBC=True):
        Vt = np.asfortranarray(Vt, dtype=np.float64)
        self._chk(self._L.ipcgpu_friction_hessian_add(self.h, _dp(Vt), C.c_double(eps2), C.c_double(coef), C.c_int(int(projectDBC))))

    def set_time_integration(self, name, beta=0.25, gamma=0.5):
        self._chk(self._L.ipcgpu_opt_set_time_integration(self.h, C.c_int({"BE": 0, "NM": 1}[name]), C.c_double(beta), C.c_double(gamma)))

    def set_warm_start(self, option):
        self._chk(self._L.ipcgpu_opt_set_warm_start(self.h, C.c_int(int(option))))

    def warm_step(self):
        v = C.c_double()
        self._chk(self._L.ipcgpu_opt_get_warm_step(self.h, C.byref(v)))
        return v.value

    def add_dirichlet(self, ids, lin_vel=(0, 0, 0), ang_vel_deg=(0, 0, 0), t0=0.0, t1=float("inf")):
        ids = _i32(ids)
        lin = _f64(np.asarray(lin_vel, dtype=np.float64))
        ang = _f64(np.asarray(ang_vel_deg, dtype=np.float64) * np.pi / 180)
        self._chk(self._L.ipcgpu_opt_add_dirichlet(self.h, C.c_int(len(ids)), _ip(ids), _dp(lin), _dp(ang), C.c_double(t0), C.c_double(t1)))

    def set_dirichlet_targets(self, group, targets):
        if targets is None:
            self._chk(self._L.ipcgpu_opt_set_dirichlet_targets(self.h, C.c_int(group), C.c_int(0), None))
            return
        t = _f64(np.ascontiguousarray(np.asarray(targets, dtype=np.float64).reshape(-1, 3)))
        self._chk(self._L.ipcgpu_opt_set_dirichlet_targets(self.h, C.c_int(group), C.c_int(t.shape[0]), _dp(t)))

    def set_dirichlet_motion(self, group, lin_vel=(0, 0, 0), ang_vel_deg=(0, 0, 0), center=None, force_nonzero=True):
        lin = _f64(np.asarray(lin_vel, dtype=np.float64))
        ang = _f64(np.asarray(ang_vel_deg, dtype=np.float64) * np.pi / 180)
        ctr = None if center is None else _f64(np.asarray(center, dtype=np.float64))
        self._chk(self._L.ipcgpu_opt_set_dirichlet_motion(self.h, C.c_int(group), _dp(lin), _dp(ang), None if ctr is None else _dp(ctr),
                                                          C.c_int(int(force_nonzero))))

    def end_dirichlet(self, group, t_end):
        self._chk(self._L.ipcgpu_opt_end_dirichlet(self.h, C.c_int(group), C.c_double(t_end)))

    def add_neumann(self, ids, accel, t0=0.0, t1=float("inf")):
        ids = _i32(ids)
        a = _f64(np.asarray(accel, dtype=np.float64))
        self._chk(self._L.ipcgpu_opt_add_neumann(self.h, C.c_int(len(ids)), _ip(ids), _dp(a), C.c_double(t0), C.c_double(t1)))

    def dbc_state(self):
        out = np.zeros(4)
        self._chk(self._L.ipcgpu_opt_get_dbc_state(self.h, _dp(out)))
        return dict(completed=out[0], rho=out[1], projectDBC=bool(out[2]), n_targets=int(out[3]))

    def kinematics(self):
        vel, acc, dx = np.zeros(3 * self.nV), np.zeros(3 * self.nV), np.zeros(3 * self.nV)
        self._chk(self._L.ipcgpu_opt_get_kinematics(self.h, _dp(vel), _dp(acc), _dp(dx)))
        return dict(velocity=vel, acceleration=acc, dx_Elastic=dx)

    def save_status(self, path):
        self._chk(self._L.ipcgpu_opt_save_status(self.h, str(path).encode()))

    def load_status(self, path):
        self._chk(self._L.ipcgpu_opt_load_status(self.h, str(path).encode()))

    def set_velocity(self, vel):
        vel = _f64(np.asarray(vel).reshape(-1))
        assert vel.size == 3 * self.nV
        self._chk(self._L.ipcgpu_opt_set_velocity(self.h, _dp(vel)))

    def contact_state(self):
        cnt = np.zeros(6, dtype=np.int32)
        pr = np.zeros(2, dtype=np.int32)
        self._chk(self._L.ipcgpu_opt_get_contact_state(self.h, _ip(cnt), _ip(pr)))
        return dict(nActive=int(cnt[0]), nPara=int(cnt[1]), nCand=int(cnt[2]), nHalfSpace=int(cnt[3]), nFullCCD=int(cnt[4]),
                    nPatternChanges=int(cnt[5]), ccdPair=(int(pr[0]), int(pr[1])))

    def timers(self):
        t = np.zeros(16)
        self._chk(self._L.ipcgpu_opt_get_timers(self.h, _dp(t)))
        return t

    def bench_assembly(self, dtSq, reps=20):
        ms, by = C.c_double(), C.c_double()
        self._chk(self._L.ipcgpu_bench_assembly(self.h, C.c_double(dtSq), C.c_int(reps), C.byref(ms), C.byref(by)))
        return ms.value, by.value

    def bench_factor_solve(self, reps=3):
        f, s = C.c_double(), C.c_double()
        self._chk(self._L.ipcgpu_bench_factor_solve(self.h, C.c_int(reps), C.byref(f), C.byref(s)))
        return f.value, s.value

    def bench_multiply_sym(self, reps=50):
        ms, by = C.c_double(), C.c_double()
        self._chk(self._L.ipcgpu_bench_multiply_sym(self.h, C.c_int(reps), C.byref(ms), C.byref(by)))
        return ms.value, by.value

    def bench_stream(self, nbytes=1 << 30, reps=10):
        g = C.c_double()
        self._chk(self._L.ipcgpu_bench_stream(self.h, C.c_longlong(nbytes), C.c_int(reps), C.byref(g)))
        return g.value
```

Measured before the change: 448.7.

## Fuse solve tail: negate, max-abs, filter+energy, trial check into fewer kernels

Adds a fused Newton search-direction tail for the single-rank multifrontal path. The right-hand-side negation is folded into the permute kernel and the direction inf-norm is folded into the unpermute kernel. The inversion filter and current energy are computed in one pass, the trial energy and inversion check in another, and all scalars are published to the host in one kernel. It also skips the per-iteration scalar reset when slots are known clean. The aim is fewer kernel launches and fewer passes over the mesh per iteration, at the cost of dirty-slot bookkeeping that must stay correct, plus new stats counters.

```diff
diff --git a/include/ipcgpu.h b/include/ipcgpu.h
--- a/include/ipcgpu.h
+++ b/include/ipcgpu.h
@@ -71,6 +71,7 @@
 int ipcgpu_linsys_factorize(ipcgpu_ctx*);
 int ipcgpu_linsys_solve(ipcgpu_ctx*, const double* rhs, double* result);
 int ipcgpu_linsys_precondition_diag(ipcgpu_ctx*, const double* in, double* out);
+int ipcgpu_linsys_factorize_solve(ipcgpu_ctx*, const double* rhs, double* result, int negate, double* xInf);
 int ipcgpu_linsys_set_iterative(ipcgpu_ctx*, double rel_tol, int max_iter, int precond, int max_factor_age);
 int ipcgpu_linsys_iter_stats(ipcgpu_ctx*, double* out6);
 int ipcgpu_linsys_coarse_stats(ipcgpu_ctx*, double* out5);
@@ -170,6 +171,7 @@
 int ipcgpu_opt_solve_timestep(ipcgpu_ctx*, int maxIter, int* nIter);
 int ipcgpu_opt_get_state(ipcgpu_ctx*, double* V_colmajor, double* searchDir_3nV, double* gradient_3nV, double* scalars8);
 int ipcgpu_opt_get_timers(ipcgpu_ctx*, double* t16);
+int ipcgpu_opt_tail_stats(ipcgpu_ctx*, long long* out7, double* dirNorm);
 typedef int (*ipcgpu_allreduce_fn)(void* user, void* buf_dev, long long count, int op);
 int ipcgpu_opt_set_allreduce(ipcgpu_ctx*, ipcgpu_allreduce_fn fn, void* user);
 typedef int (*ipcgpu_allreduce_stream_fn)(void* user, void* buf_dev, long long count, int op, void* hip_stream);
diff --git a/ipc_amd/csrc/capi.cpp b/ipc_amd/csrc/capi.cpp
--- a/ipc_amd/csrc/capi.cpp
+++ b/ipc_amd/csrc/capi.cpp
@@ -702,6 +702,23 @@
         return ok ? IPCGPU_OK : IPCGPU_NOT_PD;
     });
 }
+int ipcgpu_linsys_factorize_solve(ipcgpu_ctx* c, const double* rhs, double* x, int negate, double* xInf)
+{
+    return guarded([&] {
+        bind(c);
+        HipLinSysSolver& l = L(c);
+        need(l.fusedSolveTail(), "ipcgpu_linsys_factorize_solve: the multifrontal solver on one rank, after analyze_pattern");
+        DevBuf<double> db, dx, dm;
+        db.upload(rhs, l.numRows, c->stream);
+        dx.alloc(l.numRows);
+        dm.alloc(1);
+        dm.zero(c->stream);
+        const bool ok = l.factorizeSolve(db.p, dx.p, true, negate != 0, xInf ? dm.p : nullptr);
+        dx.download(x, l.numRows, c->stream);
+        if (xInf) dm.download(xInf, 1, c->stream);
+        return ok ? IPCGPU_OK : IPCGPU_NOT_PD;
+    });
+}
 int ipcgpu_linsys_precondition_diag(ipcgpu_ctx* c, const double* in, double* out)
 {
     return guarded([&] {
@@ -1759,6 +1776,16 @@
     return guarded([&] {
         O(c).resolveEventTimers();
         std::memcpy(t, O(c).timers, sizeof(double) * 16);
+        return IPCGPU_OK;
+    });
+}
+int ipcgpu_opt_tail_stats(ipcgpu_ctx* c, long long* out7, double* dirNorm)
+{
+    return guarded([&] {
+        HipOptimizer& o = O(c);
+        for (int i = 0; i < 6; ++i) out7[i] = o.tailStats[i];
+        out7[6] = o.tailSlotsClean ? 1 : 0;
+        if (dirNorm) *dirNorm = o.cachedDist;
         return IPCGPU_OK;
     });
 }
diff --git a/ipc_amd/csrc/hip_ipc.h b/ipc_amd/csrc/hip_ipc.h
--- a/ipc_amd/csrc/hip_ipc.h
+++ b/ipc_amd/csrc/hip_ipc.h
@@ -74,7 +74,8 @@
     void analyze_pattern(const HipMesh* meshForCoords);
     bool factorize();
     bool solve(const double* rhs_dev, double* x_dev);
-    bool factorizeSolve(const double* rhs_dev, double* x_dev, bool wait = true);
+    bool factorizeSolve(const double* rhs_dev, double* x_dev, bool wait = true, bool negateRhs = false, double* maxAbsOut = nullptr);
+    bool fusedSolveTail() const;
     bool lastPivotsOk() const;
     bool lastSyncOk_ = true;
     void multiply(const double* x_dev, double* y_dev);
@@ -268,6 +269,10 @@
     double cachedDist = 0, cachedE0 = 0, cachedFilter = 0;
     bool cachedTrialValid = false, cachedTrialInverted = false;
     double cachedTrialE = 0, cachedAlpha = 1.0;
+    DevBuf<double> d_partialTrial;
+    bool tailSlotsClean = false;
+    void dirtyTailSlots() { tailSlotsClean = false; }
+    long long tailStats[6] = { 0, 0, 0, 0, 0, 0 };
     DevBuf<double> d_aSpec, d_gradSpec;
     bool specAsmValid = false;
     void speculativeAssembly();
diff --git a/ipc_amd/csrc/hip_linsys.hip b/ipc_amd/csrc/hip_linsys.hip
--- a/ipc_amd/csrc/hip_linsys.hip
+++ b/ipc_amd/csrc/hip_linsys.hip
@@ -330,14 +330,16 @@
     return f == 0;
 }
 
-bool HipLinSysSolver::factorizeSolve(const double* rhs_dev, double* x_dev, bool wait)
+bool HipLinSysSolver::factorizeSolve(const double* rhs_dev, double* x_dev, bool wait, bool negateRhs, double* maxAbsOut)
 {
     if (!analyzed_) throw StateError("factorize before analyze_pattern");
     lastSyncOk_ = true;
-    if (solverType == 0) return lastSyncOk_ = num_.factorizeSolve(d_a.p, rhs_dev, x_dev, wait);
+    if (solverType == 0) return lastSyncOk_ = num_.factorizeSolve(d_a.p, rhs_dev, x_dev, wait, negateRhs, maxAbsOut);
+    if (negateRhs || maxAbsOut) throw StateError("factorizeSolve: a negated right-hand side and |x|_inf come with the multifrontal solver only (fusedSolveTail())");
     const bool ok = factorize();
     return lastSyncOk_ = ok && solve(rhs_dev, x_dev);
 }
+bool HipLinSysSolver::fusedSolveTail() const { return solverType == 0 && analyzed_ && num_.overlapsForward(); }
 bool HipLinSysSolver::lastPivotsOk() const { return lastSyncOk_ && (solverType != 0 || num_.lastPivotsOk()); }
 
 bool HipLinSysSolver::solve(const double* rhs_dev, double* x_dev)
diff --git a/ipc_amd/csrc/hip_optimizer.cpp b/ipc_amd/csrc/hip_optimizer.cpp
--- a/ipc_amd/csrc/hip_optimizer.cpp
+++ b/ipc_amd/csrc/hip_optimizer.cpp
@@ -79,6 +79,8 @@
     d_minusG.alloc(n3);
     d_x0.alloc(n3);
     d_partial.alloc((size_t)std::max(mesh.nT, mesh.nV) / 256 + 2);
+    d_partialTrial.alloc(d_partial.n);
+    dirtyTailSlots();
     d_scalar.alloc(8);
     d_flag.alloc(2);
     h_scalar.alloc(8);
@@ -975,6 +977,7 @@
 bool HipOptimizer::checkInversion()
 {
     if (mesh.energyType == 1) return true;
+    dirtyTailSlots();
     d_flag.zero(stream);
     launch_check_inversion(view(), d_flag.p, stream);
     launch_publish(d_flag.p, h_flag.dev, 1, stream);
@@ -1004,6 +1007,7 @@
 double HipOptimizer::filterStepSize(const double* p_dev, double stepSize)
 {
     if (mesh.energyType == 1) return stepSize;
+    dirtyTailSlots();
     launch_fill(d_scalar.p + 2, 1, 1e20, stream);
     launch_inversion_step(view(), p_dev, 0.2, stepSize, d_scalar.p + 2, stream);
     reduceMin(d_scalar.p + 2, 1);
@@ -1043,6 +1047,7 @@
 
 void HipOptimizer::enqueueDirNorm()
 {
+    dirtyTailSlots();
     launch_fill(d_scalar.p + 3, 1, 0.0, stream);
     launch_max_abs(3 * mesh.nV, d_searchDir.p, d_scalar.p + 3, stream);
 }
@@ -1050,10 +1055,50 @@
 void HipOptimizer::computeSearchDir()
 {
     bool ok;
-    launch_negate(3 * mesh.nV, d_gradient.p, d_minusG.p, stream);
+    const bool fusedTail = fastPath() && lin.fusedSolveTail();
+    if (!fusedTail) launch_negate(3 * mesh.nV, d_gradient.p, d_minusG.p, stream);
     cachedTrialValid = false;
     cachedDistValid = false;
-    if (fastPath()) {
+    if (fusedTail) {
+        Tic t(timers[3], stream);
+        const size_t bytes = 3 * (size_t)mesh.nV * sizeof(double);
+        const bool guard = mesh.energyType != 1;
+        tailStats[0]++;
+        if (!tailSlotsClean) {
+            launch_iter_reset(d_scalar.p, d_flag.p, stream);
+            tailStats[1]++;
+        }
+        if (!lin.factorizeSolve(d_gradient.p, d_searchDir.p, false, true, d_scalar.p + 3))
+            throw StateError("computeSearchDir: the solver left the enqueued sequence it announced");
+        launch_filter_energy(view(), d_searchDir.p, 0.2, 1.0, guard, d_scalar.p + 2, elasticCoef(), d_partial.p, stream);
+        launch_trial_step_fused(3 * mesh.nV, mesh.d_x.p, d_x0.p, d_searchDir.p, d_scalar.p + 2, guard, d_scalar.p + 6, stream);
+        launch_check_energy(view(), guard, d_flag.p, elasticCoef(), d_partialTrial.p, stream);
+        launch_tail_publish(view(), d_partial.p, d_partialTrial.p, d_scalar.p, d_flag.p, h_flag.dev, h_scalar.dev, stream);
+        tailSlotsClean = true;
+        if (!evTail) HIP_CHECK(hipEventCreateWithFlags(&evTail, hipEventDisableTiming));
+        HIP_CHECK(hipEventRecord(evTail, stream));
+        speculativeAssembly();
+        HIP_CHECK(hipEventSynchronize(evTail));
+        t.nosync = specAsmValid;
+        if (lin.lastPivotsOk()) {
+            cachedE0 = h_scalar.p[0];
+            cachedTrialE = h_scalar.p[1];
+            cachedFilter = h_scalar.p[2];
+            cachedDist = h_scalar.p[3];
+            cachedAlpha = h_scalar.p[6];
+            cachedTrialInverted = guard && h_flag.p[0] != 0;
+            cachedDistValid = cachedE0Valid = cachedTrialValid = true;
+            return;
+        }
+        tailStats[5]++;
+        HIP_CHECK(hipMemcpyAsync(mesh.d_x.p, d_x0.p, bytes, hipMemcpyDeviceToDevice, stream));
+        specAsmValid = false;
+        t.nosync = false;
+        dirtyTailSlots();
+        launch_negate(3 * mesh.nV, d_gradient.p, d_minusG.p, stream);
+        ok = false;
+    }
+    else if (fastPath()) {
         Tic t(timers[3], stream);
         const size_t bytes = 3 * (size_t)mesh.nV * sizeof(double);
         if (lin.factorizeSolve(d_minusG.p, d_searchDir.p, false)) {
@@ -1110,6 +1155,7 @@
     }
     if (fastPath()) {
         enqueueDirNorm();
+        dirtyTailSlots();
         launch_fill(d_scalar.p + 2, 1, 1e20, stream);
         if (mesh.energyType != 1) launch_inversion_step(view(), d_searchDir.p, 0.2, 1.0, d_scalar.p + 2, stream);
         launch_energy(view(), elasticCoef(), true, true, d_partial.p, (int)d_partial.n, d_scalar.p, stream);
@@ -1169,10 +1215,13 @@
         lastEnergyVal = cachedE0;
         if (!cachedTrialInverted && !(cachedTrialE > lastEnergyVal)) {
             lastEnergyVal = cachedTrialE;
+            tailStats[2]++;
             return;
         }
+        tailStats[cachedTrialInverted ? 3 : 4]++;
         HIP_CHECK(hipMemcpyAsync(mesh.d_x.p, d_x0.p, bytes, hipMemcpyDeviceToDevice, stream));
         specAsmValid = false;
+        dirtyTailSlots();
     }
     else if (cachedE0Valid && fastPath()) {
         cachedE0Valid = false;
@@ -1185,6 +1234,7 @@
             stepForward(d_x0.p, stepSize);
             int inverted = 0;
             if (mesh.energyType != 1) {
+                dirtyTailSlots();
                 d_flag.zero(stream);
                 launch_check_inversion(view(), d_flag.p, stream);
                 launch_publish(d_flag.p, h_flag.dev, 1, stream);
@@ -1283,6 +1333,7 @@
     const bool batched = BEGIN_BATCHED && fastPath() && nHandles && dbcGroups.empty() && !selfCollision && planes.empty() && !(warmStart >= 1 && warmStart <= 5);
     if (batched) {
         const bool guard = mesh.energyType != 1;
+        dirtyTailSlots();
         d_flag.zero(stream);
         if (guard) launch_check_inversion(view(), d_flag.p, stream);
         d_searchDir.zero(stream);
@@ -1517,6 +1568,7 @@
             if (batchedBounds) {
                 const bool filter = mesh.energyType != 1;
                 if (filter) {
+                    dirtyTailSlots();
                     launch_fill(d_scalar.p + 2, 1, 1e20, stream);
                     launch_inversion_step(view(), d_searchDir.p, 0.2, alpha, d_scalar.p + 2, stream);
                 }
diff --git a/ipc_amd/csrc/mf_numeric.h b/ipc_amd/csrc/mf_numeric.h
--- a/ipc_amd/csrc/mf_numeric.h
+++ b/ipc_amd/csrc/mf_numeric.h
@@ -60,7 +60,8 @@
     double sharedFlopFraction() const { return mp_.sharedFlops; }
     bool factorize(const double* a_dev);
     void solve(const double* rhs_dev, double* x_dev);
-    bool factorizeSolve(const double* a_dev, const double* rhs_dev, double* x_dev, bool wait = true);
+    bool factorizeSolve(const double* a_dev, const double* rhs_dev, double* x_dev, bool wait = true, bool negateRhs = false, double* maxAbsOut = nullptr);
+    bool overlapsForward() const { return world_ <= 1 && fwd_; }
     bool lastPivotsOk() const { return pivotsOk(); }
     bool pivotsOk() const;
     bool ready() const { return ns_ > 0; }
@@ -101,7 +102,7 @@
     void reduceSolution();
     void allreduceFlag();
     void configureSweepKernels(size_t maxSolveLds, size_t maxBwdLds, size_t maxTriLds);
-    void enqueuePermuteRhs(const double* rhs_dev, hipStream_t st);
+    void enqueuePermuteRhs(const double* rhs_dev, hipStream_t st, bool negate = false);
     const MfSymbolic* sym_ = nullptr;
     hipStream_t stream_ = nullptr;
     int ns_ = 0, nLevels_ = 0;
@@ -117,7 +118,7 @@
     hipEvent_t evRhs_ = nullptr, evFwdDone_ = nullptr;
     std::vector<hipEvent_t> evFactLevel_;
     void enqueueForwardLevel(int l, hipStream_t st);
-    void enqueueBackward(double* x_dev);
+    void enqueueBackward(double* x_dev, bool tail = false, double* maxAbsOut = nullptr);
     hipEvent_t evSide_ = nullptr;
     std::vector<hipEvent_t> evLevel_, evInvDone_;
     bool sidePending_ = false;
diff --git a/ipc_amd/csrc/mf_numeric.hip b/ipc_amd/csrc/mf_numeric.hip
--- a/ipc_amd/csrc/mf_numeric.hip
+++ b/ipc_amd/csrc/mf_numeric.hip
@@ -1530,23 +1530,23 @@
     return hflag_.p[0] == 0;
 }
 
-bool MfNumeric::factorizeSolve(const double* a_dev, const double* rhs_dev, double* x_dev, bool wait)
+bool MfNumeric::factorizeSolve(const double* a_dev, const double* rhs_dev, double* x_dev, bool wait, bool negateRhs, double* maxAbsOut)
 {
     if (!sym_) throw StateError("factorize before analyze_pattern");
-    if (world_ > 1 || !fwd_) {
+    if (!overlapsForward()) {
+        if (negateRhs || maxAbsOut) throw StateError("factorizeSolve: a negated right-hand side and |x|_inf need the overlapped sequence (one rank)");
         const bool ok = factorize(a_dev);
         if (ok) solve(rhs_dev, x_dev);
         return ok;
     }
     HIP_CHECK(hipEventRecord(evRhs_, stream_));
     HIP_CHECK(hipStreamWaitEvent(fwd_, evRhs_, 0));
-    enqueuePermuteRhs(rhs_dev, fwd_);
+    enqueuePermuteRhs(rhs_dev, fwd_, negateRhs);
     fwdJoined_ = false;
     enqueueFactor(a_dev, true);
     if (!fwdJoined_) HIP_CHECK(hipEventRecord(evFwdDone_, fwd_));
-    hipLaunchKernelGGL(k_publish_flag, dim3(1), dim3(1), 0, stream_, flag_.p, hflag_.dev);
     if (!fwdJoined_) HIP_CHECK(hipStreamWaitEvent(stream_, evFwdDone_, 0));
-    enqueueBackward(x_dev);
+    enqueueBackward(x_dev, true, maxAbsOut);
     if (!wait) return true;
     HIP_CHECK(hipStreamSynchronize(stream_));
     return pivotsOk();
diff --git a/ipc_amd/csrc/mf_sweeps.hip b/ipc_amd/csrc/mf_sweeps.hip
--- a/ipc_amd/csrc/mf_sweeps.hip
+++ b/ipc_amd/csrc/mf_sweeps.hip
@@ -14,21 +14,40 @@
 
 namespace {
 
-__global__ void k_permute_rhs(int nn, const int* __restrict__ newOf, const double* __restrict__ b, double* __restrict__ bp)
+__global__ void k_permute_rhs(int nn, const int* __restrict__ newOf, const double* __restrict__ b, int negate, double* __restrict__ bp)
 {
     int i = blockIdx.x * blockDim.x + threadIdx.x;
     if (i < 3 * nn) {
         int v = i / 3, d = i - 3 * v;
-        bp[3 * newOf[v] + d] = b[i];
-    }
-}
-__global__ void k_unpermute_x(int nn, const int* __restrict__ newOf, const double* __restrict__ xp, double* __restrict__ x)
+        const double val = b[i];
+        bp[3 * newOf[v] + d] = negate ? -val : val;
+    }
+}
+template <bool TAIL>
+__global__ __launch_bounds__(256) void k_unpermute_x(int nn, const int* __restrict__ newOf, const double* __restrict__ xp, double* __restrict__ x,
+    unsigned long long* __restrict__ maxAbs, const int* __restrict__ flag, int* __restrict__ mapped)
 {
     int i = blockIdx.x * blockDim.x + threadIdx.x;
+    double m = 0.0;
     if (i < 3 * nn) {
         int v = i / 3, d = i - 3 * v;
-        x[i] = xp[3 * newOf[v] + d];
-    }
+        const double val = xp[3 * newOf[v] + d];
+        x[i] = val;
+        m = fmax(m, fabs(val));
+    }
+    if (!TAIL) return;
+    if (maxAbs) {
+        __shared__ double sm[256 / 64];
+#pragma unroll
+        for (int off = 32; off > 0; off >>= 1) m = fmax(m, __shfl_down(m, off, 64));
+        if ((threadIdx.x & 63) == 0) sm[threadIdx.x >> 6] = m;
+        __syncthreads();
+        if (threadIdx.x == 0) {
+            for (int w = 1; w < 256 / 64; ++w) m = fmax(m, sm[w]);
+            atomicMax(maxAbs, (unsigned long long)__double_as_longlong(m));
+        }
+    }
+    if (blockIdx.x == 0 && threadIdx.x == 0) mapped[0] = flag[0];
 }
 
 __device__ __forceinline__ double gather_w(const TreeView& tv, const long long* __restrict__ wOff, const double* __restrict__ wbuf,
@@ -482,10 +501,10 @@
     }
 }
 
-void MfNumeric::enqueuePermuteRhs(const double* rhs_dev, hipStream_t st)
+void MfNumeric::enqueuePermuteRhs(const double* rhs_dev, hipStream_t st, bool negate)
 {
     const int n3 = sym_->n;
-    hipLaunchKernelGGL(k_permute_rhs, dim3((n3 + 255) / 256), dim3(256), 0, st, sym_->nn, newOf_.p, rhs_dev, bperm_.p);
+    hipLaunchKernelGGL(k_permute_rhs, dim3((n3 + 255) / 256), dim3(256), 0, st, sym_->nn, newOf_.p, rhs_dev, negate ? 1 : 0, bperm_.p);
 }
 
 void MfNumeric::solve(const double* rhs_dev, double* x_dev)
@@ -529,7 +548,7 @@
         hipLaunchKernelGGL(k_big_fwd_rect, dim3(P.fwdRect.cnt), dim3(WG), 0, st, desc_.p + P.fwdRect.off, tv, wOff_.p, fronts_.p, w_.p, yperm_.p);
 }
 
-void MfNumeric::enqueueBackward(double* x_dev)
+void MfNumeric::enqueueBackward(double* x_dev, bool tail, double* maxAbsOut)
 {
     const MfSymbolic& sym = *sym_;
     TreeView tv{ frontOff_.p, idxPtr_.p, firstNode_.p, childPtr_.p, child_.p, invPtr_.p, inv_.p, idx_.p, dinvOff_.p };
@@ -587,7 +606,12 @@
     }
 #endif
     if (world_ > 1) reduceSolution();
-    hipLaunchKernelGGL(k_unpermute_x, dim3((n3 + 255) / 256), dim3(256), 0, stream_, sym.nn, newOf_.p, xsol_.p, x_dev);
-}
-
-}
+    if (tail)
+        hipLaunchKernelGGL(k_unpermute_x<true>, dim3((n3 + 255) / 256), dim3(256), 0, stream_, sym.nn, newOf_.p, xsol_.p, x_dev, (unsigned long long*)maxAbsOut,
+            flag_.p, hflag_.dev);
+    else
+        hipLaunchKernelGGL(k_unpermute_x<false>, dim3((n3 + 255) / 256), dim3(256), 0, stream_, sym.nn, newOf_.p, xsol_.p, x_dev, (unsigned long long*)nullptr,
+            (const int*)nullptr, (int*)nullptr);
+}
+
+}
diff --git a/ipc_amd/csrc/nh_kernels.h b/ipc_amd/csrc/nh_kernels.h
--- a/ipc_amd/csrc/nh_kernels.h
+++ b/ipc_amd/csrc/nh_kernels.h
@@ -43,6 +43,9 @@
 void launch_max_abs(int n, const double* v, double* out , hipStream_t s);
 void launch_trial_step_fused(int n3, double* x, double* x0, const double* p, const double* filterMin, bool useFilter, double* alphaOut, hipStream_t s);
 void launch_iter_reset(double* scalar, int* flag, hipStream_t s);
+void launch_filter_energy(const ElemView& v, const double* p, double slackness, double tMax, bool filter, double* outMin, double coef, double* partial, hipStream_t s);
+void launch_check_energy(const ElemView& v, bool check, int* flag, double coef, double* partial, hipStream_t s);
+void launch_tail_publish(const ElemView& v, const double* partial0, const double* partial1, double* scalar, int* flag, void* hflag, void* hscalar, hipStream_t s);
 void launch_publish2(const void* a, void* da, int na, const void* b, void* db, int nb, hipStream_t s);
 void launch_fill(double* p, size_t n, double v, hipStream_t s);
 void launch_negate(int n, const double* in, double* out, hipStream_t s);
diff --git a/ipc_amd/csrc/nh_kernels.hip b/ipc_amd/csrc/nh_kernels.hip
--- a/ipc_amd/csrc/nh_kernels.hip
+++ b/ipc_amd/csrc/nh_kernels.hip
@@ -112,6 +112,24 @@
     return fcr_psi(s, mu, lam);
 }
 
+__device__ __forceinline__ double elem_energy(const ElemView& v, int t, const d3& x0, const d3& x1, const d3& x2, const d3& x3, double coef)
+{
+    double A[9], F[9];
+    load_A(v, t, A);
+    deformation_gradient(x0, x1, x2, x3, A, F);
+    return coef * v.vol[t] * elem_psi(v, F, v.mu[t], v.lam[t]);
+}
+__device__ __forceinline__ double node_inertia(const ElemView& v, int n)
+{
+    double d2 = 0.0;
+#pragma unroll
+    for (int i = 0; i < 3; ++i) {
+        double d = v.x[3 * (size_t)n + i] - v.xTilde[3 * (size_t)n + i];
+        d2 += d * d;
+    }
+    return d2 * v.mass[n] / 2.0;
+}
+
 __global__ __launch_bounds__(BLOCK) void k_energy(ElemView v, double coef, int withInertia, int owner, double* __restrict__ partial)
 {
     __shared__ double sm[BLOCK / 64];
@@ -120,20 +138,9 @@
     const int t = v.tetBegin + gid;
     if (t < v.tetEnd) {
         const int4 tv = v.tet[t];
-        double A[9], F[9];
-        load_A(v, t, A);
-        deformation_gradient(ld3(v.x, tv.x), ld3(v.x, tv.y), ld3(v.x, tv.z), ld3(v.x, tv.w), A, F);
-        e = coef * v.vol[t] * elem_psi(v, F, v.mu[t], v.lam[t]);
-    }
-    if (withInertia && owner && gid < v.nV) {
-        double d2 = 0.0;
-#pragma unroll
-        for (int i = 0; i < 3; ++i) {
-            double d = v.x[3 * (size_t)gid + i] - v.xTilde[3 * (size_t)gid + i];
-            d2 += d * d;
-        }
-        e += d2 * v.mass[gid] / 2.0;
-    }
+        e = elem_energy(v, t, ld3(v.x, tv.x), ld3(v.x, tv.y), ld3(v.x, tv.z), ld3(v.x, tv.w), coef);
+    }
+    if (withInertia && owner && gid < v.nV) e += node_inertia(v, gid);
     double r = block_sum(e, sm);
     if (threadIdx.x == 0) partial[blockIdx.x] = r;
 }
@@ -318,16 +325,19 @@
     }
 }
 
+__device__ __forceinline__ bool elem_inverted(const d3& x0, const d3& x1, const d3& x2, const d3& x3)
+{
+    const double e[9] = { x1.x - x0.x, x1.y - x0.y, x1.z - x0.z, x2.x - x0.x, x2.y - x0.y, x2.z - x0.z, x3.x - x0.x,
+        x3.y - x0.y, x3.z - x0.z };
+    return det3(e) < 0.0;
+}
 __global__ __launch_bounds__(BLOCK) void k_check_inversion(ElemView v, int* flag)
 {
     const int t = v.tetBegin + blockIdx.x * BLOCK + threadIdx.x;
     if (t >= v.tetEnd) return;
     if (!(v.mu[t] != 0.0 && v.lam[t] != 0.0)) return;
     const int4 tv = v.tet[t];
-    const d3 x0 = ld3(v.x, tv.x), x1 = ld3(v.x, tv.y), x2 = ld3(v.x, tv.z), x3 = ld3(v.x, tv.w);
-    const double e[9] = { x1.x - x0.x, x1.y - x0.y, x1.z - x0.z, x2.x - x0.x, x2.y - x0.y, x2.z - x0.z, x3.x - x0.x,
-        x3.y - x0.y, x3.z - x0.z };
-    if (det3(e) < 0.0) atomicOr(flag, 1);
+    if (elem_inverted(ld3(v.x, tv.x), ld3(v.x, tv.y), ld3(v.x, tv.z), ld3(v.x, tv.w))) atomicOr(flag, 1);
 }
 
 struct cplx {
@@ -395,6 +405,44 @@
     return t;
 }
 
+__device__ __forceinline__ double elem_inversion_root(const d3& x0, const d3& x1, const d3& x2, const d3& x3, const double* __restrict__ p, const int4& tv,
+    double slackness, double tMax)
+{
+    double res = 1e20;
+    const d3 p0 = ld3(p, tv.x), p1 = ld3(p, tv.y), p2 = ld3(p, tv.z), p3 = ld3(p, tv.w);
+    const double v0[3] = { x1.x - x0.x, x1.y - x0.y, x1.z - x0.z }, v1[3] = { x2.x - x0.x, x2.y - x0.y, x2.z - x0.z },
+                 v2[3] = { x3.x - x0.x, x3.y - x0.y, x3.z - x0.z };
+    const double q0[3] = { p1.x - p0.x, p1.y - p0.y, p1.z - p0.z }, q1[3] = { p2.x - p0.x, p2.y - p0.y, p2.z - p0.z },
+                 q2[3] = { p3.x - p0.x, p3.y - p0.y, p3.z - p0.z };
+    auto cross = [](const double* x, const double* y, double* z) {
+        z[0] = x[1] * y[2] - x[2] * y[1];
+        z[1] = x[2] * y[0] - x[0] * y[2];
+        z[2] = x[0] * y[1] - x[1] * y[0];
+    };
+    auto dot = [](const double* x, const double* y) { return x[0] * y[0] + x[1] * y[1] + x[2] * y[2]; };
+    double pxp[3], vxp[3], pxv[3], vxv[3], mix[3];
+    cross(q0, q1, pxp);
+    cross(v0, q1, vxp);
+    cross(q0, v1, pxv);
+    cross(v0, v1, vxv);
+    for (int c = 0; c < 3; ++c) mix[c] = vxp[c] + pxv[c];
+    const double a = dot(q2, pxp);
+    const double b = dot(v2, pxp) + dot(q2, mix);
+    const double c = dot(q2, vxv) + dot(v2, mix);
+    const double d = (1.0 - slackness) * dot(v2, vxv);
+    const double lower = d + tMax * (fmin(c, 0.0) + tMax * (fmin(b, 0.0) + tMax * fmin(a, 0.0)));
+    if (!(lower > 0.01 * d)) {
+        const double r = cubic_root(a, b, c, d, 1.0e-6);
+        res = (r >= 0) ? r : 1e20;
+    }
+    return res;
+}
+__device__ __forceinline__ void wave_min_to(double res, unsigned long long* __restrict__ outMin)
+{
+#pragma unroll
+    for (int off = 32; off > 0; off >>= 1) res = fmin(res, __shfl_down(res, off, 64));
+    if ((threadIdx.x & 63) == 0 && res < 1e20) atomicMin(outMin, (unsigned long long)__double_as_longlong(res));
+}
 __global__ __launch_bounds__(BLOCK) void k_inversion_step(ElemView v, const double* __restrict__ p, double slackness, double tMax,
     unsigned long long* __restrict__ outMin)
 {
@@ -402,37 +450,75 @@
     double res = 1e20;
     if (t < v.tetEnd) {
         const int4 tv = v.tet[t];
+        res = elem_inversion_root(ld3(v.x, tv.x), ld3(v.x, tv.y), ld3(v.x, tv.z), ld3(v.x, tv.w), p, tv, slackness, tMax);
+    }
+    wave_min_to(res, outMin);
+}
+
+template <bool FILTER>
+__global__ __launch_bounds__(BLOCK) void k_filter_energy(ElemView v, const double* __restrict__ p, double slackness, double tMax,
+    unsigned long long* __restrict__ outMin, double coef, double* __restrict__ partial)
+{
+    __shared__ double sm[BLOCK / 64];
+    const int gid = blockIdx.x * BLOCK + threadIdx.x;
+    const int t = v.tetBegin + gid;
+    double e = 0.0, res = 1e20;
+    if (t < v.tetEnd) {
+        const int4 tv = v.tet[t];
         const d3 x0 = ld3(v.x, tv.x), x1 = ld3(v.x, tv.y), x2 = ld3(v.x, tv.z), x3 = ld3(v.x, tv.w);
-        const d3 p0 = ld3(p, tv.x), p1 = ld3(p, tv.y), p2 = ld3(p, tv.z), p3 = ld3(p, tv.w);
-        const double v0[3] = { x1.x - x0.x, x1.y - x0.y, x1.z - x0.z }, v1[3] = { x2.x - x0.x, x2.y - x0.y, x2.z - x0.z },
-                     v2[3] = { x3.x - x0.x, x3.y - x0.y, x3.z - x0.z };
-        const double q0[3] = { p1.x - p0.x, p1.y - p0.y, p1.z - p0.z }, q1[3] = { p2.x - p0.x, p2.y - p0.y, p2.z - p0.z },
-                     q2[3] = { p3.x - p0.x, p3.y - p0.y, p3.z - p0.z };
-        auto cross = [](const double* x, const double* y, double* z) {
-            z[0] = x[1] * y[2] - x[2] * y[1];
-            z[1] = x[2] * y[0] - x[0] * y[2];
-            z[2] = x[0] * y[1] - x[1] * y[0];
-        };
-        auto dot = [](const double* x, const double* y) { return x[0] * y[0] + x[1] * y[1] + x[2] * y[2]; };
-        double pxp[3], vxp[3], pxv[3], vxv[3], mix[3];
-        cross(q0, q1, pxp);
-        cross(v0, q1, vxp);
-        cross(q0, v1, pxv);
-        cross(v0, v1, vxv);
-        for (int c = 0; c < 3; ++c) mix[c] = vxp[c] + pxv[c];
-        const double a = dot(q2, pxp);
-        const double b = dot(v2, pxp) + dot(q2, mix);
-        const double c = dot(q2, vxv) + dot(v2, mix);
-        const double d = (1.0 - slackness) * dot(v2, vxv);
-        const double lower = d + tMax * (fmin(c, 0.0) + tMax * (fmin(b, 0.0) + tMax * fmin(a, 0.0)));
-        if (!(lower > 0.01 * d)) {
-            const double r = cubic_root(a, b, c, d, 1.0e-6);
-            res = (r >= 0) ? r : 1e20;
-        }
-    }
-#pragma unroll
-    for (int off = 32; off > 0; off >>= 1) res = fmin(res, __shfl_down(res, off, 64));
-    if ((threadIdx.x & 63) == 0 && res < 1e20) atomicMin(outMin, (unsigned long long)__double_as_longlong(res));
+        if (FILTER) res = elem_inversion_root(x0, x1, x2, x3, p, tv, slackness, tMax);
+        e = elem_energy(v, t, x0, x1, x2, x3, coef);
+    }
+    if (gid < v.nV) e += node_inertia(v, gid);
+    if (FILTER) wave_min_to(res, outMin);
+    const double r = block_sum(e, sm);
+    if (threadIdx.x == 0) partial[blockIdx.x] = r;
+}
+template <bool CHECK>
+__global__ __launch_bounds__(BLOCK) void k_check_energy(ElemView v, int* __restrict__ flag, double coef, double* __restrict__ partial)
+{
+    __shared__ double sm[BLOCK / 64];
+    const int gid = blockIdx.x * BLOCK + threadIdx.x;
+    const int t = v.tetBegin + gid;
+    double e = 0.0;
+    if (t < v.tetEnd) {
+        const int4 tv = v.tet[t];
+        const d3 x0 = ld3(v.x, tv.x), x1 = ld3(v.x, tv.y), x2 = ld3(v.x, tv.z), x3 = ld3(v.x, tv.w);
+        if (CHECK && v.mu[t] != 0.0 && v.lam[t] != 0.0 && elem_inverted(x0, x1, x2, x3)) atomicOr(flag, 1);
+        e = elem_energy(v, t, x0, x1, x2, x3, coef);
+    }
+    if (gid < v.nV) e += node_inertia(v, gid);
+    const double r = block_sum(e, sm);
+    if (threadIdx.x == 0) partial[blockIdx.x] = r;
+}
+__global__ __launch_bounds__(BLOCK) void k_tail_publish(const double* __restrict__ partial0, const double* __restrict__ partial1, int n, double* __restrict__ scalar,
+    int* __restrict__ flag, int* __restrict__ hflag, double* __restrict__ hscalar)
+{
+    __shared__ double sm[BLOCK / 64];
+    double x = 0.0;
+    for (int i = threadIdx.x; i < n; i += BLOCK) x += partial0[i];
+    const double e0 = block_sum(x, sm);
+    __syncthreads();
+    x = 0.0;
+    for (int i = threadIdx.x; i < n; i += BLOCK) x += partial1[i];
+    const double e1 = block_sum(x, sm);
+    if (threadIdx.x == 0) {
+        const int f = flag[0];
+        const double s2 = scalar[2], s3 = scalar[3], s4 = scalar[4], s5 = scalar[5], s6 = scalar[6];
+        scalar[0] = e0;
+        scalar[1] = e1;
+        hflag[0] = f;
+        hscalar[0] = e0;
+        hscalar[1] = e1;
+        hscalar[2] = s2;
+        hscalar[3] = s3;
+        hscalar[4] = s4;
+        hscalar[5] = s5;
+        hscalar[6] = s6;
+        scalar[3] = 0.0;
+        scalar[2] = 1e20;
+        flag[0] = 0;
+    }
 }
 
 __global__ void k_step_forward(int n, const double* __restrict__ x0, const double* __restrict__ p, double alpha, double* __restrict__ x)
@@ -856,6 +942,23 @@
 {
     hipLaunchKernelGGL(k_trial_step_fused, dim3(std::max(nblk(n3), 1)), dim3(BLOCK), 0, s, n3, x, x0, p, filterMin, useFilter ? 1 : 0, alphaOut);
 }
+void launch_filter_energy(const ElemView& v, const double* p, double slackness, double tMax, bool filter, double* outMin, double coef, double* partial, hipStream_t s)
+{
+    const int nb = std::max(1, nblk(std::max(v.tetEnd - v.tetBegin, v.nV)));
+    if (filter) hipLaunchKernelGGL(k_filter_energy<true>, dim3(nb), dim3(BLOCK), 0, s, v, p, slackness, tMax, (unsigned long long*)outMin, coef, partial);
+    else hipLaunchKernelGGL(k_filter_energy<false>, dim3(nb), dim3(BLOCK), 0, s, v, p, slackness, tMax, (unsigned long long*)outMin, coef, partial);
+}
+void launch_check_energy(const ElemView& v, bool check, int* flag, double coef, double* partial, hipStream_t s)
+{
+    const int nb = std::max(1, nblk(std::max(v.tetEnd - v.tetBegin, v.nV)));
+    if (check) hipLaunchKernelGGL(k_check_energy<true>, dim3(nb), dim3(BLOCK), 0, s, v, flag, coef, partial);
+    else hipLaunchKernelGGL(k_check_energy<false>, dim3(nb), dim3(BLOCK), 0, s, v, flag, coef, partial);
+}
+void launch_tail_publish(const ElemView& v, const double* partial0, const double* partial1, double* scalar, int* flag, void* hflag, void* hscalar, hipStream_t s)
+{
+    const int nb = std::max(1, nblk(std::max(v.tetEnd - v.tetBegin, v.nV)));
+    hipLaunchKernelGGL(k_tail_publish, dim3(1), dim3(BLOCK), 0, s, partial0, partial1, nb, scalar, flag, (int*)hflag, (double*)hscalar);
+}
 void launch_iter_reset(double* scalar, int* flag, hipStream_t s) { hipLaunchKernelGGL(k_iter_reset, dim3(1), dim3(1), 0, s, scalar, flag); }
 void launch_publish2(const void* a, void* da, int na, const void* b, void* db, int nb, hipStream_t s)
 {
diff --git a/ipc_amd/lib.py b/ipc_amd/lib.py
--- a/ipc_amd/lib.py
+++ b/ipc_amd/lib.py
@@ -349,6 +349,11 @@
     def elastic_hessian_add(self, coef=1.0, projectDBC=True):
         self._chk(self._L.ipcgpu_elastic_hessian_add(self.h, C.c_double(coef), C.c_int(int(projectDBC))))
 
+    def set_nodal_mass(self, mass):
+        mass = _f64(mass)
+        assert mass.size == self.nV
+        self._chk(self._L.ipcgpu_set_mesh_features(self.h, None, None, _dp(mass), None, None))
+
     def filter_step_size(self, p, step=1.0):
         p = _f64(p)
         s = C.c_double(step)
@@ -447,6 +452,13 @@
         x = np.zeros_like(rhs)
         self._chk(self._L.ipcgpu_linsys_solve(self.h, _dp(rhs), _dp(x)))
         return x
+
+    def factorize_solve(self, rhs, negate=False):
+        rhs = _f64(rhs)
+        x = np.zeros_like(rhs)
+        xinf = C.c_double()
+        rc = self._chk(self._L.ipcgpu_linsys_factorize_solve(self.h, _dp(rhs), _dp(x), C.c_int(1 if negate else 0), C.byref(xinf)), allow_not_pd=True)
+        return rc == IPCGPU_OK, x, xinf.value
 
     def precondition_diag(self, v):
         v = _f64(v)
@@ -838,6 +850,13 @@
         return dict(nActive=int(cnt[0]), nPara=int(cnt[1]), nCand=int(cnt[2]), nHalfSpace=int(cnt[3]), nFullCCD=int(cnt[4]),
                     nPatternChanges=int(cnt[5]), ccdPair=(int(pr[0]), int(pr[1])))
 
+    def tail_stats(self):
+        s = np.zeros(7, dtype=np.int64)
+        d = C.c_double()
+        self._chk(self._L.ipcgpu_opt_tail_stats(self.h, s.ctypes.data_as(C.POINTER(C.c_longlong)), C.byref(d)))
+        return dict(fused=int(s[0]), resets=int(s[1]), accepted=int(s[2]), inverted=int(s[3]), uphill=int(s[4]), bad_pivot=int(s[5]), slots_clean=bool(s[6]),
+                    dir_norm=d.value)
+
     def timers(self):
         t = np.zeros(16)
         self._chk(self._L.ipcgpu_opt_get_timers(self.h, _dp(t)))
```

Result: no change. 452.0, median of 6 (+0.7%).
